# floe/backscrub

Hardware: AMD Instinct MI355X
Metric: composited frames/sec at 640×480 (batch), 1/2/4/8 MI355X + mask IoU vs CPU ref (higher is better)
Workload: dtype f32 (network) / u8 (image kernels); 1 GPU; BASELINE configs[1]: batch=256 640x480 frames, segm_lite_v681.tflite; moving scene: ring of 4 batches, a new one every step; 1 step = prep+network+decode+mask+blend, inputs resident in HBM; streams_per_gpu=256, library=bsx 0.1 (HIP gfx950, f32 NHWC)

## Files before the change

backscrub_amd/csrc/bsx_api.hip:

```cpp
#include "debug_switches.hpp"
#include <hip/hip_runtime.h>

#include <algorithm>
#include <cmath>
#include <cstdarg>
#include <cstdio>
#include <cstdlib>
#include <cstring>
#include <map>
#include <memory>
#include <string>
#include <thread>
#include <vector>

#include "../../include/bsx.h"
#include "gen_mid.hpp"
#include "kernels.hpp"
#include "roctx_ranges.hpp"
#include "plan.hpp"
#include "refusal.hpp"
#include "rtc.hpp"
#include "specialised.hpp"
#include "tflite_model.hpp"
#include "vcam_nv12_plan.hpp"
// ... 245 lines not shown
    BSX_HIP(c, hipMemcpy(c->d_geom_classes, rec.data(), G * sizeof(GeomClass), hipMemcpyHostToDevice));
  }
  if (any_edge && !c->d_geom_classes_vg) {
    BSX_HIP(c, hipMalloc(reinterpret_cast<void**>(&c->d_geom_classes_vg), G * sizeof(GeomClass)));
    BSX_HIP(c, hipMemcpy(c->d_geom_classes_vg, rec_vg.data(), G * sizeof(GeomClass), hipMemcpyHostToDevice));
  }
  if (!c->no_uniform_tiles && !c->d_geom_tile_class) {
    BSX_HIP(c, hipMalloc(&c->d_geom_tile_class, tiles + 4));
    BSX_HIP(c, hipMemset(c->d_geom_tile_class, 0, tiles + 4));
  }
  if (!c->h_geo) BSX_HIP(c, hipHostMalloc(reinterpret_cast<void**>(&c->h_geo), bsx_ctx::kIdRing * N * sizeof(GeomDesc), hipHostMallocDefault));
  BSX_HIP(c, hipMalloc(reinterpret_cast<void**>(&c->d_geo), bsx_ctx::kIdRing * N * sizeof(GeomDesc)));
  return BSX_OK;
}

int init_device_state(bsx_ctx* c) {
  BSX_HIP(c, hipStreamCreateWithFlags(&c->own_stream, hipStreamNonBlocking));
  const size_t N = (size_t)c->n_streams;
  BSX_HIP(c, hipMalloc(&c->d_arena, c->plan.arena_floats_per_stream * N * sizeof(float)));
  BSX_HIP(c, hipMalloc(&c->d_net_in, N * c->inW * c->inH * c->inC * sizeof(float)));
  BSX_HIP(c, hipMalloc(&c->d_net_in_u8, N * c->inW * c->inH * sizeof(uint32_t)));
  BSX_HIP(c, hipMalloc(&c->d_net_out, N * c->outW * c->outH * c->outC * sizeof(float)));
  BSX_HIP(c, hipMalloc(&c->d_weights, std::max<size_t>(c->plan.weights.size(), 4) * sizeof(float)));
  BSX_HIP(c, hipMemcpy(c->d_weights, c->plan.weights.data(), c->plan.weights.size() * sizeof(float), hipMemcpyHostToDevice));
  BSX_HIP(c, hipMalloc(&c->d_weights16, std::max<size_t>(c->plan.weights16.size(), 8) * sizeof(uint16_t)));
  BSX_HIP(c, hipMemcpy(c->d_weights16, c->plan.weights16.data(), c->plan.weights16.size() * sizeof(uint16_t), hipMemcpyHostToDevice));
  if (const char* m = getenv("BSX_F16_GEMM")) c->f16_terms = !strcmp(m, "off") ? 0 : (!strcmp(m, "fast") ? 1 : (!strcmp(m, "fast16") ? 17 : 3));
  c->use_program = !c->plan.program.empty() && BSX_DBG_ENV("BSX_NO_FRAME_PROGRAM") == nullptr &&
                   (c->plan.seg.on || c->plan.program_lds_tensors >= c->plan.program_global_tensors || BSX_DBG_ENV("BSX_FORCE_FRAME_PROGRAM") != nullptr);
  hipDeviceProp_t prop;
  const bool have_prop = c->use_program && !BSX_DBG_ENV("BSX_NO_RTC") && hipGetDeviceProperties(&prop, c->device) == hipSuccess;
  const KernelVariant v = kernel_variant(c->plan);
  if (c->use_program) {
    BSX_HIP(c, hipMalloc(&c->d_program, c->plan.program.size() * sizeof(MicroOp)));
    BSX_HIP(c, hipMemcpy(c->d_program, c->plan.program.data(), c->plan.program.size() * sizeof(MicroOp), hipMemcpyHostToDevice));
    BSX_HIP(c, frame_program_prepare(c->plan.program_lds_floats));
    if (c->plan.seg.on) BSX_HIP(c, seg_prepare());
    c->act16 = v.act16;
    if (BSX_DBG_ENV("BSX_NO_RTC")) no_specialised("BSX_NO_RTC", &c->kern);
    else if (!have_prop) no_specialised("no device properties", &c->kern);
    else load_specialised(build_specialised(c->plan, v, prop.gcnArchName), &c->kern);
    if (c->act16 && !c->kern.mid) {
      c->last_error = "BSX_ACT16: the specialised middle kernel is not available (" + c->kern.mid_note + ")";
      return BSX_EDEVICE;
    }
    if (c->act16) c->kern.mid_note += ", 16-bit activation storage";
  } else {
    BSX_HIP(c, nn_prepare());
  }
  if (const char* l = BSX_DBG_ENV("BSX_PIPE_WGS")) c->pipe_wgs = std::min(8, std::max(0, atoi(l)));
  if (const char* l = BSX_DBG_ENV("BSX_LANES")) c->lanes = std::min(4, std::max(1, atoi(l)));
  if (c->lanes > 1) {
    BSX_HIP(c, hipEventCreateWithFlags(&c->ev_fork, hipEventDisableTiming));
    for (int k = 1; k < c->lanes; k++) {
      BSX_HIP(c, hipStreamCreateWithFlags(&c->lane_stream[k], hipStreamNonBlocking));
      BSX_HIP(c, hipEventCreateWithFlags(&c->ev_join[k], hipEventDisableTiming));
    }
  }
  if (BSX_DBG_ENV("BSX_NO_GRAPH")) c->graph_state = -1;
  c->in_u8 = v.u8in && ((c->use_program && c->plan.seg.on) || (!c->use_program && head0_u8_ok(c->plan)));
  BSX_HIP(c, hipMalloc(&c->d_ofinal, N * c->outW * c->outH));
  BSX_HIP(c, hipMalloc(&c->d_masks, c->mask_bytes));
  BSX_HIP(c, hipMemset(c->d_ofinal, 0, N * c->outW * c->outH));
  BSX_HIP(c, hipMemset(c->d_masks, 255, c->mask_bytes));
  {
    const double sigma_color = 100.0, sigma_space = 100.0;
    const double gc = -0.5 / (sigma_color * sigma_color), gs = -0.5 / (sigma_space * sigma_space);
    const int radius = 2;
    std::vector<float> lut(768);
    for (int i = 0; i < 768; i++) lut[i] = (float)std::exp(i * i * gc);
    BSX_HIP(c, hipMalloc(&c->d_color_lut, 768 * sizeof(float)));
    BSX_HIP(c, hipMemcpy(c->d_color_lut, lut.data(), 768 * sizeof(float), hipMemcpyHostToDevice));
    int k = 0;
    for (int i = -radius; i <= radius; i++) for (int j = -radius; j <= radius; j++) {
      double r = std::sqrt((double)i * i + (double)j * j);
      if (r > radius) continue;
      c->bilateral.space_w[k] = (float)std::exp(r * r * gs);
      c->bilateral.off_y[k] = i; c->bilateral.off_x[k] = j;
      k++;
    }
    c->bilateral.color_lut = c->d_color_lut;
    c->bilateral.scale = c->norm_scale; c->bilateral.offset = c->norm_offset;
    if (k != 13 || !bilateral_taps_match(c->bilateral)) { c->last_error = "bilateral tap table does not match the kernel"; return BSX_EDEVICE; }
  }
  int rc = upload_tab(c, make_resize_tab(c->roi.w, c->roi.h, c->in_roi.w, c->in_roi.h), &c->tab_down);
  if (rc) return rc;
  rc = upload_tab(c, make_resize_tab(c->in_roi.w, c->in_roi.h, c->roi.w, c->roi.h), &c->tab_up);
  if (rc) return rc;
  c->tiles_per_frame = (size_t)((c->roi.w + mask_tile_width() - 1) / mask_tile_width()) * (size_t)((c->roi.h + mask_tile_height() - 1) / mask_tile_height());
  if (!c->no_uniform_tiles && c->tab_up.tab.mode == 0 && c->tab_up.tab.tile_ok && c->geoms.size() <= 1) {
    BSX_HIP(c, hipMalloc(&c->d_tile_class, N * c->tiles_per_frame + 4));
    BSX_HIP(c, hipMemset(c->d_tile_class, 0, N * c->tiles_per_frame + 4));
    c->tab_up.tab.tile_class = c->d_tile_class;
  }
  for (size_t g = 0; g < c->geoms.size(); g++) {
    bsx_ctx::Geom& G = c->geoms[g];
    if (g == 0) { G.tab_down = c->tab_down; G.tab_up = c->tab_up; }
    else {
      if ((rc = upload_tab(c, make_resize_tab(G.roi.w, G.roi.h, G.in_roi.w, G.in_roi.h), &G.tab_down))) return rc;
      if ((rc = upload_tab(c, make_resize_tab(G.in_roi.w, G.in_roi.h, G.roi.w, G.roi.h), &G.tab_up))) return rc;
    }
    G.tab_up.tab.tile_class = nullptr;
    G.edge = c->edge_roi && !geom_class_on_grid(G.roi);
    const size_t tile_rows = (size_t)((G.roi.h + mask_tile_height() - 1) / mask_tile_height());
    G.tiles_per_frame = (size_t)geom_tile_cols(G.roi, G.edge) * tile_rows;
    G.vg_tiles_per_frame = (size_t)geom_tile_cols(G.roi, false) * tile_rows;
    G.outside_blocks = geom_outside_blocks(G.width, G.height, G.roi);
    G.fusable = G.edge ? geom_class_edge_fusable(G.width, G.roi, G.tab_up.tab, G.shifted_tiles_fit) : geom_class_fusable(G.width, G.roi, G.tab_up.tab);
    G.xcd = geom_class_xcd(G.width, G.roi);
  }
  if (c->geoms.size() > 1) return geoms_device_state(c);
  return BSX_OK;
}

hipStream_t pick(bsx_ctx*, void* s) { return (hipStream_t)s; }

struct LaunchTimer { std::vector<hipEvent_t> ev; int k = 0; ~LaunchTimer() { for (hipEvent_t e : ev) if (e) (void)hipEventDestroy(e); } };
int timed(bsx_ctx* c, LaunchTimer* t, hipStream_t s) {
  if (t->k + 1 >= (int)t->ev.size()) { c->last_error = "error: bsx_profile_batch: the step made more launches than the profile counts\n"; return BSX_EDEVICE; }
  BSX_HIP(c, hipEventRecord(t->ev[++t->k], s));
  return BSX_OK;
}
#define BSX_LAUNCH(c, t, s, expr) do { BSX_HIP(c, (expr)); if (t) { const int trc_ = timed(c, t, s); if (trc_) return trc_; } } while (0)

int run_prep(bsx_ctx* c, const uint8_t* d_frames, int n, hipStream_t s, bool with_f32 = false, bool yuyv_in = false, LaunchTimer* t = nullptr) {
  bsx_roctx::Range range("bsx:prep");
  float* f32 = (!c->in_u8 || with_f32) ? c->tensor_ptr(c->plan.input) : nullptr;
  uint32_t* u8 = c->in_u8 ? c->d_net_in_u8 : nullptr;
  BSX_LAUNCH(c, t, s, launch_prep_fused(d_frames, c->width, c->height, c->roi, f32, u8, c->inW, c->inH, c->in_roi, c->tab_down.tab, c->bilateral, n, s, yuyv_in));
  return BSX_OK;
}
bool argmax_tail(const bsx_ctx* c) {
  return !c->use_program && !c->keep_logits && c->model_type == BSX_MODEL_DEEPLAB && !c->plan.steps.empty() && c->plan.steps.back().out == c->plan.output &&
         resize_argmax_fusable(c->plan.steps.back());
}
hipError_t launch_program(bsx_ctx* c, int n, hipStream_t s, unsigned long long* timeline = nullptr) {
  long pf = (long)c->plan.arena_floats_per_stream;
  if (c->kern.mid) {
    float* arena = c->d_arena;
    const float* weights = c->d_weights;
    void* args[] = {&arena, &pf, &weights, &timeline};
    return hipModuleLaunchKernel(c->kern.mid, (unsigned)n, 1, 1, (unsigned)c->plan.mid_lanes, 1, 1, 0, s, args, nullptr);
  }
  return launch_frame_program(c->d_program, (int)c->plan.program.size(), c->plan.program_lds_floats, c->d_arena, pf, c->d_net_in, c->d_net_out, c->d_weights, n, s,
                              timeline);
}
int state_write_fence(bsx_ctx* c, hipStream_t s) {
  if (!c->wait_before_state) return BSX_OK;
  hipEvent_t ev = c->wait_before_state;
  c->wait_before_state = nullptr;
  BSX_HIP(c, hipStreamWaitEvent(s, ev, 0));
  return BSX_OK;
}
bool program_op_elided(const bsx_ctx* c, int i) { return c->kern.mid && !BSX_DBG_ENV("BSX_RTC_FINE") && mid_pw_feeds_dw(c->plan, i); }

bool debug_tensor_half(const bsx_ctx* c, int t) {
  const Plan& p = c->plan;
  if (t == p.input || t == p.output) return false;
  if (c->use_program) {
    if (!c->act16) return false;
    if (p.seg.on && std::find(p.seg_stored.begin(), p.seg_stored.end(), t) != p.seg_stored.end()) return true;
    for (size_t i = 0; i < p.program.size() && i < p.program_out_tensor.size(); i++)
      if (p.program_out_tensor[i] == t) return p.program[i].kind != kMicroSe;
    return false;
  }
  const int n = c->last_net_n > 0 ? c->last_net_n : c->n_streams;
  for (int j = 1; j < (int)p.steps.size(); j++)
    if (p.steps[j].out == t) return p.steps[j - 1].fuse_dw == j && ir_out16(p, p.steps[j - 1], n, c->d_weights16, c->f16_terms, BSX_DBG_ENV("BSX_NO_PW_GEMM") != nullptr);
  return false;
}

bool k3_frame_runs(const bsx_ctx* c) { return c->use_program && c->plan.seg.on && c->plan.seg.k3f.on && c->kern.k3_frame != nullptr; }
bool infer_decodes(const bsx_ctx* c) { return (c->use_program && c->plan.seg.on && !c->keep_logits) || argmax_tail(c); }
int run_infer(bsx_ctx* c, int n, hipStream_t s, bool logits = true, int slot = 0, const int* ids = nullptr, LaunchTimer* t = nullptr) {
  bsx_roctx::Range range("bsx:network");
  c->last_net_n = n;
  c->last_net_logits = logits;
  if (c->arena_poison) {
    BSX_HIP(c, hipMemsetAsync(c->d_arena, 0xFF, c->plan.arena_floats_per_stream * (size_t)c->n_streams * sizeof(float), s));
    BSX_HIP(c, hipMemsetAsync(c->d_net_out, 0xFF, (size_t)c->n_streams * c->outW * c->outH * c->outC * sizeof(float), s));
  }
  if (c->use_program && c->plan.seg.on) {
    const SegPlan& sp = c->plan.seg;
    const hipFunction_t* fn = c->kern.seg;
    const long pf = (long)c->plan.arena_floats_per_stream;
    const void* in = c->in_u8 ? (const void*)c->d_net_in_u8 : (const void*)c->d_net_in;
    BSX_LAUNCH(c, t, s, launch_seg_head(fn[0], sp.head, c->d_arena, pf, in, c->d_weights, n, s, c->act16, c->in_u8, c->norm_scale, c->norm_offset));
    BSX_LAUNCH(c, t, s, launch_seg_k2(fn[1], sp.k2, c->d_arena, pf, c->d_weights, n, s, c->act16));
    BSX_LAUNCH(c, t, s, launch_program(c, n, s));
    if (k3_frame_runs(c)) {
      BSX_LAUNCH(c, t, s, launch_seg_k3_frame(c->kern.k3_frame, sp.k3f, c->d_arena, pf, c->d_weights, n, s));
    } else {
      BSX_LAUNCH(c, t, s, launch_seg_k3(fn[2], sp.k3, c->d_arena, pf, c->d_weights, n, s, c->act16));
      if (sp.tail.pre_gate_off >= 0) BSX_LAUNCH(c, t, s, launch_seg_gate(sp.tail.gate, c->d_arena, pf, c->d_weights, sp.tail.pre_gate_off, n, s));
    }
    if (!logits) { const int frc = state_write_fence(c, s); if (frc) return frc; }
    BSX_LAUNCH(c, t, s, launch_seg_tail(fn[3], sp.tail, c->d_arena, pf, c->d_net_out, c->d_ofinal + (size_t)slot * c->outW * c->outH, c->d_weights, logits, n, s,
                                        c->act16, ids));
    return BSX_OK;
  }
  if (c->use_program) {
    BSX_LAUNCH(c, t, s, launch_program(c, n, s));
    return BSX_OK;
  }
  const bool fused_tail = !logits && argmax_tail(c);
  const size_t ns = c->plan.steps.size() - (fused_tail ? 1 : 0);
  for (size_t i = 0; i < ns; i++)
    BSX_LAUNCH(c, t, s, launch_step(c->plan.steps[i], c->plan, c->d_arena, c->d_net_in, c->d_net_out, c->d_weights, n, c->n_streams, s, c->d_weights16, c->f16_terms, c->in_u8 ? c->d_net_in_u8 : nullptr, c->norm_scale, c->norm_offset));
  if (fused_tail) {
    const Step& last = c->plan.steps.back();
    { const int frc = state_write_fence(c, s); if (frc) return frc; }
    BSX_LAUNCH(c, t, s, launch_resize_argmax_iir(last, c->d_arena + (size_t)c->plan.tensor_off[last.in0] * (size_t)c->n_streams,
                                                 c->d_ofinal + (size_t)slot * c->outW * c->outH, n, s, c->tail_generic, ids));
  }
  return BSX_OK;
}
int run_decode(bsx_ctx* c, int n, hipStream_t s, int slot = 0, const int* ids = nullptr, LaunchTimer* t = nullptr) {
  bsx_roctx::Range range("bsx:decode");
  { const int frc = state_write_fence(c, s); if (frc) return frc; }
  BSX_LAUNCH(c, t, s, launch_decode(c->model_type, c->tensor_ptr(c->plan.output), c->d_ofinal + (size_t)slot * c->outW * c->outH, c->outW * c->outH, c->outC, n, s, ids));
  return BSX_OK;
}
ResizeTab tab_up_at(const bsx_ctx* c, int slot) { ResizeTab t = c->tab_up.tab; if (t.tile_class) t.tile_class += (size_t)slot * c->tiles_per_frame; return t; }
int run_mask(bsx_ctx* c, int n, hipStream_t s, int slot = 0, const int* ids = nullptr, LaunchTimer* t = nullptr, uint8_t* masks = nullptr) {
  bsx_roctx::Range range("bsx:mask");
  BSX_LAUNCH(c, t, s, launch_mask_upscale_blur(c->d_ofinal + (size_t)slot * c->outW * c->outH, c->outW, c->outH, c->in_roi, tab_up_at(c, slot),
                                      (masks ? masks : c->d_masks) + (size_t)slot * c->width * c->height, c->width, c->height, c->roi, n, s, ids));
  return BSX_OK;
}
int infer_after_prep(bsx_ctx* c, int n, hipStream_t s, int slot, const int* ids, LaunchTimer* t = nullptr) {
  if (c->onprep && !t) { BSX_HIP(c, hipStreamSynchronize(s)); c->onprep(c->caller_ctx); }
  const bool fused_decode = infer_decodes(c);
  if (const int rc = run_infer(c, n, s, !fused_decode, slot, ids, t)) return rc;
  if (c->oninfer && !t) { BSX_HIP(c, hipStreamSynchronize(s)); c->oninfer(c->caller_ctx); }
  return fused_decode ? BSX_OK : run_decode(c, n, s, slot, ids, t);
}
int enqueue_masks(bsx_ctx* c, const uint8_t* d_frames, int n, hipStream_t s, bool yuyv_in, int slot, const int* ids, LaunchTimer* t = nullptr) {
  if (const int rc = run_prep(c, d_frames, n, s, false, yuyv_in, t)) return rc;
  return infer_after_prep(c, n, s, slot, ids, t);
}
int process_impl(bsx_ctx* c, const uint8_t* d_frames, int n, int slot, hipStream_t s, bool yuyv_in = false, const int* ids = nullptr, uint8_t* masks = nullptr) {
  if (const int rc = enqueue_masks(c, d_frames, n, s, yuyv_in, slot, ids)) return rc;
  if (c->onmask) { BSX_HIP(c, hipStreamSynchronize(s)); c->onmask(c->caller_ctx); }
  return run_mask(c, n, s, slot, ids, nullptr, masks);
}


int refuse(bsx_ctx* c, const char* fn, const char* fmt, ...) {
  char buf[256];
  va_list ap;
  va_start(ap, fmt); vsnprintf(buf, sizeof buf, fmt, ap); va_end(ap);
  c->last_error = std::string("error: ") + fn + ": " + buf + "\n";
  return BSX_EINVAL;
}
}
int bsx::refuse_call(bsx_ctx* c, const char* fn, const char* fmt, ...) {
  char buf[256];
  va_list ap;
  va_start(ap, fmt); vsnprintf(buf, sizeof buf, fmt, ap); va_end(ap);
  g_last_error = std::string("error: ") + fn + ": " + buf + "\n";
  if (c) c->last_error = g_last_error;
  return BSX_EINVAL;
}
namespace {
int refuse_pending(bsx_ctx* c, const char* fn) {
  return c->pend.active ? refuse(c, fn, "a pipelined composite is pending (flush with bsx_step_batch_pipelined(ctx, NULL, ...) first)") : BSX_OK;
}

int refuse_geoms(bsx_ctx* c, const char* fn) {
  return c->geoms.size() > 1 ? refuse(c, fn, "context has %d geometries (only bsx_step_batch_geoms and bsx_step_batch_vcam_geoms step such a context)", (int)c->geoms.size()) : BSX_OK;
}

struct StepReq {
  const uint8_t* frames; const uint8_t* bg; size_t bg_stride; uint8_t* out;
  int out_w, out_h, n;
  unsigned flags; hipStream_t s;
  const int* ids;
  const MixDesc* mix = nullptr;
  const int* mix_pos = nullptr;
  bool mix_bgr = false;
  bool mix_blur_due = false;
  bool yuyv() const { return (flags & BSX_STEP_YUYV) != 0; }
  bool yin() const { return (flags & BSX_STEP_YUYV_IN) != 0; }
  unsigned flip() const { return flags & (BSX_STEP_FLIP_H | BSX_STEP_FLIP_V); }
  int bgblur() const { return (int)((flags >> 8) & 255u); }
  bool resize(const bsx_ctx* c) const { return out_w != c->width || out_h != c->height; }
  size_t out_bytes() const { return (size_t)n * out_w * out_h * (yuyv() ? 2 : 3); }
  bool out_overlaps(const uint8_t* p, size_t bytes) const { return out < p + bytes && p < out + out_bytes(); }
  bool overlap(const bsx_ctx* c) const { return out_overlaps(frames, (size_t)n * c->width * c->height * (yin() ? 2 : 3)); }
};
enum class Entry { Step, Streams, Vcam, Pipelined, Mixed, VcamMixed };

bool tile_fusable(const bsx_ctx* c, const StepReq& r) {
  return !c->onmask && !c->no_mask_blend_fusion && (!r.yuyv() || ((uintptr_t)r.out & 3) == 0) && !(r.overlap(c) && (r.yin() || r.yuyv() || r.flip())) &&
         (!r.yin() || prep_yuyv_fusable(c->width, c->roi, c->tab_down.tab)) &&
         mask_blend_fusable(c->width, c->height, c->roi, r.bg, r.bg_stride, r.frames, r.yuyv() ? r.frames : r.out);
}

int check_step(bsx_ctx* c, const char* fn, const StepReq& r, Entry kind) {
  const bool vcam = kind == Entry::Vcam, pipe = kind == Entry::Pipelined, blur = r.bgblur() != 0;
  if (kind == Entry::Mixed) {
    if (!r.frames || !r.out || r.n <= 0 || r.n > c->n_streams) return refuse(c, fn, "null buffer or batch size out of range");
    if (r.flags & ~(BSX_STEP_YUYV | BSX_STEP_NO_MASK | BSX_STEP_YUYV_IN)) return refuse(c, fn, "flags 0x%x has bits outside yuyv / no-mask / yuyv-in", r.flags);
    if (const int rc = refuse_pending(c, fn)) return rc;
    if (r.yuyv() && (c->width & 1)) return refuse(c, fn, "YUYV output needs an even width");
    if (r.yin() && (c->width & 1)) return refuse(c, fn, "YUYV input needs an even capture width");
    if (r.overlap(c)) return refuse(c, fn, "output overlaps the frames (the mixed step has no in-place form)");
// ... 823 lines not shown
  char line[256];
  snprintf(line, sizeof line, "specialised middle kernel: %zu micro-ops, %zu workgroup barriers per launch (%zu between ops + %zu inside ops)\n", p.program.size(), ob + sy, ob, sy);
  return line;
}
}

extern "C" {

const char* bsx_version(void) { return "bsx 0.1 (HIP gfx950, f32 NHWC)"; }

int bsx_device_count(void) {
  int n = 0;
  if (hipGetDeviceCount(&n) != hipSuccess) return 0;
  return n;
}

const char* bsx_last_error(const bsx_ctx* ctx) { return ctx ? ctx->last_error.c_str() : g_last_error.c_str(); }

static bool capture_rois(const bsx_ctx* c, size_t width, size_t height, Rect4* roi, Rect4* in_roi) {
  float ratio = (float)c->inH / (float)c->inW;
  float frameratio = (float)height / (float)width;
  if (frameratio < ratio) {
    *roi = Rect4{(int)((width - height / ratio) / 2), 0, (int)(height / ratio), (int)height};
    *in_roi = Rect4{0, 0, c->inW, c->inH};
  } else {
    *roi = Rect4{0, 0, (int)width, (int)height};
    *in_roi = Rect4{(int)((c->inW - c->inH / frameratio) / 2), 0, (int)(c->inH / frameratio), c->inH};
  }
  return !(roi->w <= 0 || roi->h <= 0 || roi->x < 0 || roi->x + roi->w > (int)width || in_roi->w <= 0 || in_roi->x < 0 || in_roi->x + in_roi->w > c->inW ||
           in_roi->x + in_roi->w > c->outW || in_roi->h > c->outH);
}

static bsx_ctx* new_ctx(const char* model_path, size_t threads, const bsx_geometry* geoms, int n_geoms, int device, bsx_debug_fn ondebug, bsx_stage_fn onprep,
                        bsx_stage_fn oninfer, bsx_stage_fn onmask, void* caller_ctx, unsigned geom_flags = 0) {
  const size_t width = (size_t)geoms[0].width, height = (size_t)geoms[0].height;
  int n_streams = 0;
  for (int g = 0; g < n_geoms; g++) n_streams += geoms[g].n_streams;
  try {
  std::unique_ptr<bsx_ctx> c(new bsx_ctx);
  c->ondebug = ondebug; c->onprep = onprep; c->oninfer = oninfer; c->onmask = onmask; c->caller_ctx = caller_ctx;
  c->threads = threads; c->width = (int)width; c->height = (int)height; c->n_streams = n_streams; c->device = device;
  c->edge_roi = (geom_flags & BSX_GEOMS_EDGE_ROI) != 0;
  std::string err;
  if (!load_tflite(model_path, &c->graph, &err)) { report(nullptr, ondebug, caller_ctx, "error: %s\n", err.c_str()); return nullptr; }
  c->model_type = model_type_from_name(model_path);
  if (c->model_type == BSX_MODEL_UNKNOWN) { report(nullptr, ondebug, caller_ctx, "error: unknown model type '%s'.\n", model_path); return nullptr; }
  if (c->model_type == BSX_MODEL_DEEPLAB) { c->norm_scale = (float)(1 / 127.5); c->norm_offset = -1.f; }
  else { c->norm_scale = (float)(1 / 255.0); c->norm_offset = 0.f; }
  const TensorInfo& ti = c->graph.tensors[c->graph.input];
  const TensorInfo& to = c->graph.tensors[c->graph.output];
  if (ti.shape.size() != 4 || to.shape.size() != 4 || ti.dims[0] != 1) {
    report(nullptr, ondebug, caller_ctx, "error: model input/output is not a single 4-D float tensor\n");
    return nullptr;
  }
  c->inH = ti.dims[1]; c->inW = ti.dims[2]; c->inC = ti.dims[3];
  c->outH = to.dims[1]; c->outW = to.dims[2]; c->outC = to.dims[3];
  if (c->inC != 3) { report(nullptr, ondebug, caller_ctx, "error: model input must have 3 channels\n"); return nullptr; }
  if ((c->model_type == BSX_MODEL_MEET && c->outC != 2) || (c->model_type == BSX_MODEL_DEEPLAB && c->outC < 16)) {
    report(nullptr, ondebug, caller_ctx, "error: model output has %d channels, unexpected for this model type\n", c->outC);
    return nullptr;
  }
  bool no_reuse = BSX_DBG_ENV("BSX_ARENA_NO_REUSE") != nullptr;
  const bool segments = BSX_DBG_ENV("BSX_NO_SEGMENTS") == nullptr && BSX_DBG_ENV("BSX_NO_FRAME_PROGRAM") == nullptr;
  if (!build_plan(c->graph, &c->plan, &err, !no_reuse, segments)) { report(nullptr, ondebug, caller_ctx, "error: unable to build GPU plan: %s\n", err.c_str()); return nullptr; }
  if (!capture_rois(c.get(), width, height, &c->roi, &c->in_roi)) {
    report(nullptr, ondebug, caller_ctx, "error: frame/model geometry yields an empty or out-of-range ROI\n");
    return nullptr;
  }
  c->no_mask_tile = BSX_DBG_ENV("BSX_NO_MASK_TILE") != nullptr;
  for (int g = 0; g < n_geoms; g++) {
    bsx_ctx::Geom G;
    G.width = geoms[g].width; G.height = geoms[g].height; G.n_streams = geoms[g].n_streams;
    G.first = g ? c->geoms[g - 1].first + c->geoms[g - 1].n_streams : 0;
    G.mask_offset = c->mask_bytes;
    c->mask_bytes += (size_t)G.n_streams * G.width * G.height;
    if (!capture_rois(c.get(), (size_t)G.width, (size_t)G.height, &G.roi, &G.in_roi)) {
      report(nullptr, ondebug, caller_ctx, "error: bsx_new_geoms: geoms[%d] (%d x %d): frame/model geometry yields an empty or out-of-range ROI\n", g, G.width, G.height);
      return nullptr;
    }
    if (c->edge_roi) {
      const HostResizeTab up = make_resize_tab(G.in_roi.w, G.in_roi.h, G.roi.w, G.roi.h);
      G.shifted_tiles_fit = up.mode == 0 && mask_tile_fits(up.xofs.data(), up.yofs.data(), up.sw, up.sh, up.dw, up.dh, geom_edge_shift(G.roi));
      const bool tiles = up.mode == 0 && !c->no_mask_tile && G.roi.w >= 8 && G.shifted_tiles_fit && mask_tile_fits(up.xofs.data(), up.yofs.data(), up.sw, up.sh, up.dw, up.dh);
      if (G.width & 3) {
        report(nullptr, ondebug, caller_ctx, "error: bsx_new_geoms_ex: geoms[%d] (%d x %d): width %d is not a multiple of 4 (the edge-ROI flag frees roi.x and roi.w; a row "
               "must still be whole dwords)\n", g, G.width, G.height, G.width);
        return nullptr;
      }
      if (!tiles) {
        report(nullptr, ondebug, caller_ctx, "error: bsx_new_geoms_ex: geoms[%d] (%d x %d) is off the fused tile route: the mask up-scale %d x %d -> %d x %d must be a tiled "
               "linear one\n", g, G.width, G.height, G.in_roi.w, G.in_roi.h, G.roi.w, G.roi.h);
        return nullptr;
      }
    } else if (n_geoms > 1) {
      const HostResizeTab up = make_resize_tab(G.in_roi.w, G.in_roi.h, G.roi.w, G.roi.h);
      const bool tiles = up.mode == 0 && !c->no_mask_tile && mask_tile_fits(up.xofs.data(), up.yofs.data(), up.sw, up.sh, up.dw, up.dh);
      if ((G.width & 3) || (G.roi.x & 3) || (G.roi.w & 3) || !tiles) {
        report(nullptr, ondebug, caller_ctx, "error: bsx_new_geoms: geoms[%d] (%d x %d) is off the fused tile route: width %d, roi.x %d and roi.w %d must be multiples of 4 and "
               "the mask up-scale %d x %d -> %d x %d a tiled linear one\n", g, G.width, G.height, G.width, G.roi.x, G.roi.w, G.in_roi.w, G.in_roi.h, G.roi.w, G.roi.h);
        return nullptr;
      }
    }
    c->geoms.push_back(G);
  }
  c->no_mask_blend_fusion = BSX_DBG_ENV("BSX_NO_MASK_BLEND_FUSION") != nullptr;
  c->no_bgblur_fusion = BSX_DBG_ENV("BSX_NO_BGBLUR_FUSION") != nullptr;
  c->vcam_direct = BSX_DBG_ENV("BSX_VCAM_DIRECT") != nullptr;
  c->no_uniform_tiles = getenv("BSX_NO_UNIFORM_TILES") != nullptr;
  c->tail_generic = BSX_DBG_ENV("BSX_TAIL_GENERIC") != nullptr;
  c->keep_logits = BSX_DBG_ENV("BSX_KEEP_LOGITS") != nullptr;
  c->arena_poison = BSX_DBG_ENV("BSX_ARENA_POISON") != nullptr;
  int ndev = 0;
  if (hipGetDeviceCount(&ndev) != hipSuccess || device < 0 || device >= ndev) {
    report(nullptr, ondebug, caller_ctx, "error: HIP device %d not available (%d visible)\n", device, ndev); return nullptr; }
  DeviceGuard guard(device);
  if (init_device_state(c.get()) != BSX_OK) { bsx_ctx* raw = c.release(); bsx_delete(raw); return nullptr; }
  c->plan_text = c->plan.describe();
  {
    char line[256];
    for (size_t i = 0; i < c->plan.steps.size(); i++) {
      if (c->use_program || !c->d_weights16 || !ir_out16_planned(c->plan, c->plan.steps[i], c->f16_terms)) continue;
      const Step& dd = c->plan.steps[c->plan.steps[i].fuse_dw];
      snprintf(line, sizeof line, "f16 storage: steps %zu and %d (expand + depthwise) store t%d (%dx%dx%d per frame) as f16 at %ld pixels and more, step %d reads it as f16\n", i,
               c->plan.steps[i].fuse_dw, dd.out, dd.OH, dd.OW, dd.Cout, kOut16MinRows, c->plan.steps[i].fuse_dw + 1);
      c->plan_text += line;
    }
    snprintf(line, sizeof line, "frame program: %s, %zu micro-ops, LDS %d floats (%.1f KiB), %d tensors in LDS, %d in HBM\n",
             c->use_program ? "ON" : "off", c->plan.program.size(), c->plan.program_lds_floats, c->plan.program_lds_floats / 256.0,
             c->plan.program_lds_tensors, c->plan.program_global_tensors);
    c->plan_text += line;
    if (no_reuse) c->plan_text += "arena: every tensor in a slot of its own (debug switch)\n";
    if (c->arena_poison) c->plan_text += "arena: filled with NaN bytes in front of every network stage (debug switch)\n";
    if (c->use_program) c->plan_text += "program execution: " + c->kern.mid_note + "\n";
    if (c->use_program && c->plan.seg.on) {
      std::string seg = c->plan.seg_text;
      if (c->act16)
        for (size_t at = seg.find(" stores t"); at != std::string::npos; at = seg.find(" stores t", at)) {
          for (at += 7; at + 2 < seg.size() && seg[at] == ' ' && seg[at + 1] == 't' && isdigit((unsigned char)seg[at + 2]); ) {
            for (at += 2; at < seg.size() && isdigit((unsigned char)seg[at]); at++) {}
            seg.insert(at, ":f16");
            at += 4;
          }
        }
      c->plan_text += seg;
    }
    if (c->use_program && c->plan.seg.on) c->plan_text += "segment execution: " + c->kern.seg_note + "\n";
    if (c->use_program && c->plan.seg.on && c->plan.seg.k3f.on && !c->kern.k3_frame)
      c->plan_text += "segment k3 execution: tiles and the gate launch (the per-frame form is part of the specialised module only)\n";
    if (c->use_program && c->kern.mid) c->plan_text += mid_barrier_line(c->plan, c->act16);
    for (size_t i = 0; i < c->plan.program_labels.size(); i++) {
      c->plan_text += "P" + std::to_string(i) + " " + c->plan.program_labels[i];
      if (i < c->plan.program_out_tensor.size()) {
        const int sp = c->plan.program[i].out.space;
        c->plan_text += " -> t" + std::to_string(c->plan.program_out_tensor[i]) + (sp == kLocLds ? " lds" : (program_op_elided(c.get(), (int)i) ? " elided" : (sp == kLocOutput ? " output" : " hbm")));
        if (sp == kLocGlobal && !program_op_elided(c.get(), (int)i) && debug_tensor_half(c.get(), c->plan.program_out_tensor[i])) c->plan_text += " f16";
      }
      c->plan_text += "\n";
    }
  }
  return c.release();
  } catch (const std::exception& e) {
    report(nullptr, ondebug, caller_ctx, "error: %s while creating the context\n", e.what());
    return nullptr;
  } catch (...) {
    report(nullptr, ondebug, caller_ctx, "error: unknown exception while creating the context\n");
    return nullptr;
  }
}

bsx_ctx* bsx_new(const char* model_path, size_t threads, size_t width, size_t height, int n_streams, int device, bsx_debug_fn ondebug,
                 bsx_stage_fn onprep, bsx_stage_fn oninfer, bsx_stage_fn onmask, void* caller_ctx) {
  if (!model_path || !width || !height || width > 0x7fffffffu || height > 0x7fffffffu || n_streams <= 0 || n_streams > 65535) {
    report(nullptr, ondebug, caller_ctx, "error: bad arguments to bsx_new\n"); return nullptr; }
  const bsx_geometry one{(int)width, (int)height, n_streams};
  return new_ctx(model_path, threads, &one, 1, device, ondebug, onprep, oninfer, onmask, caller_ctx);
}

static bsx_ctx* new_geoms_checked(const char* fn, const char* model_path, size_t threads, const bsx_geometry* geoms, int n_geoms, int device, unsigned geom_flags,
                                  bsx_debug_fn ondebug, bsx_stage_fn onprep, bsx_stage_fn oninfer, bsx_stage_fn onmask, void* caller_ctx) {
  if (!model_path || !geoms) { report(nullptr, ondebug, caller_ctx, "%s model_path or geoms is NULL\n", fn); return nullptr; }
  if (n_geoms < 1 || n_geoms > BSX_MAX_GEOMS) { report(nullptr, ondebug, caller_ctx, "%s n_geoms = %d is outside [1, %d]\n", fn, n_geoms, BSX_MAX_GEOMS); return nullptr; }
  long total = 0;
  for (int g = 0; g < n_geoms; g++) {
    if (geoms[g].width <= 0 || geoms[g].height <= 0) { report(nullptr, ondebug, caller_ctx, "%s geoms[%d]: size %d x %d is not positive\n", fn, g, geoms[g].width, geoms[g].height); return nullptr; }
    if (geoms[g].n_streams <= 0) { report(nullptr, ondebug, caller_ctx, "%s geoms[%d] (%d x %d): n_streams = %d is not positive\n", fn, g, geoms[g].width, geoms[g].height, geoms[g].n_streams); return nullptr; }
    for (int k = 0; k < g; k++)
      if (geoms[k].width == geoms[g].width && geoms[k].height == geoms[g].height) {
        report(nullptr, ondebug, caller_ctx, "%s geoms[%d] (%d x %d) repeats the size of geoms[%d]\n", fn, g, geoms[g].width, geoms[g].height, k); return nullptr; }
    total += geoms[g].n_streams;
    if (total > 65535) { report(nullptr, ondebug, caller_ctx, "%s geoms[%d] (%d x %d) brings the total to %ld streams, above 65535\n", fn, g, geoms[g].width, geoms[g].height, total); return nullptr; }
  }
  if (n_geoms > 1 && onmask) { report(nullptr, ondebug, caller_ctx, "%s an onmask callback needs a context of one geometry (%d given)\n", fn, n_geoms); return nullptr; }
  return new_ctx(model_path, threads, geoms, n_geoms, device, ondebug, onprep, oninfer, onmask, caller_ctx, geom_flags);
}

bsx_ctx* bsx_new_geoms(const char* model_path, size_t threads, const bsx_geometry* geoms, int n_geoms, int device, bsx_debug_fn ondebug, bsx_stage_fn onprep,
                       bsx_stage_fn oninfer, bsx_stage_fn onmask, void* caller_ctx) {
  return new_geoms_checked("error: bsx_new_geoms:", model_path, threads, geoms, n_geoms, device, 0, ondebug, onprep, oninfer, onmask, caller_ctx);
}

bsx_ctx* bsx_new_geoms_ex(const char* model_path, size_t threads, const bsx_geometry* geoms, int n_geoms, int device, unsigned flags, bsx_debug_fn ondebug,
                          bsx_stage_fn onprep, bsx_stage_fn oninfer, bsx_stage_fn onmask, void* caller_ctx) {
  if (flags == 0) return bsx_new_geoms(model_path, threads, geoms, n_geoms, device, ondebug, onprep, oninfer, onmask, caller_ctx);
  if (const unsigned unknown = flags & ~BSX_GEOMS_EDGE_ROI) {
    report(nullptr, ondebug, caller_ctx, "error: bsx_new_geoms_ex: flags 0x%x has the unknown bit 0x%x (known: 0x%x, the edge-ROI flag)\n", flags, unknown & (0u - unknown),
           BSX_GEOMS_EDGE_ROI);
    return nullptr;
  }
  return new_geoms_checked("error: bsx_new_geoms_ex:", model_path, threads, geoms, n_geoms, device, flags, ondebug, onprep, oninfer, onmask, caller_ctx);
}

void bsx_delete(bsx_ctx* c) {
  if (!c) return;
  DeviceGuard guard(c->device);
  if (c->own_stream) (void)hipStreamSynchronize(c->own_stream);
  for (auto& kv : c->host_graphs) if (kv.second) (void)hipGraphExecDestroy(kv.second);
  unload_specialised(&c->kern);
  void* ptrs[] = {c->d_arena, c->d_net_in, c->d_net_in_u8, c->d_net_out, c->d_weights, c->d_ofinal, c->d_masks, c->d_host_frame, c->d_bgr_scratch, c->d_bgr_scratch2, c->d_mask_scratch, c->d_bgblur_scratch, c->d_bgr_in_scratch, c->d_color_lut, c->tab_down.mem, c->tab_up.mem, c->d_program, c->d_weights16, c->d_tile_class};
  for (void* p : ptrs) if (p) (void)hipFree(p);
  for (auto& kv : c->bg_tabs) if (kv.second.mem) (void)hipFree(kv.second.mem);
  for (auto& kv : c->vcam_tabs) if (kv.second.d.mem) (void)hipFree(kv.second.d.mem);
  for (auto& kv : c->vg_geoms) { for (void* m : kv.second.mem) if (m) (void)hipFree(m); if (kv.second.d_rec) (void)hipFree(kv.second.d_rec); }
  if (c->own_stream) (void)hipStreamDestroy(c->own_stream);
  for (int k = 1; k < 4; k++) { if (c->lane_stream[k]) (void)hipStreamDestroy(c->lane_stream[k]); if (c->ev_join[k]) (void)hipEventDestroy(c->ev_join[k]); }
  if (c->ev_fork) (void)hipEventDestroy(c->ev_fork);
  if (c->comp_stream) { (void)hipStreamSynchronize(c->comp_stream); (void)hipStreamDestroy(c->comp_stream); }
  if (c->ev_pdone) (void)hipEventDestroy(c->ev_pdone);
  if (c->ev_pcomp) (void)hipEventDestroy(c->ev_pcomp);
  for (hipEvent_t& e : c->ev_ids) if (e) (void)hipEventDestroy(e);
  if (c->d_ids) (void)hipFree(c->d_ids);
  if (c->h_ids) (void)hipHostFree(c->h_ids);
  if (c->d_mix) (void)hipFree(c->d_mix);
  if (c->h_mix) (void)hipHostFree(c->h_mix);
  if (c->d_rsz) (void)hipFree(c->d_rsz);
  if (c->h_rsz) (void)hipHostFree(c->h_rsz);
  if (c->d_blur) (void)hipFree(c->d_blur);
  if (c->h_blur) (void)hipHostFree(c->h_blur);
  if (c->d_blur_coef) (void)hipFree(c->d_blur_coef);
  for (size_t g = 1; g < c->geoms.size(); g++) { if (c->geoms[g].tab_down.mem) (void)hipFree(c->geoms[g].tab_down.mem); if (c->geoms[g].tab_up.mem) (void)hipFree(c->geoms[g].tab_up.mem); }
  if (c->d_geom_classes) (void)hipFree(c->d_geom_classes);
  if (c->d_geom_classes_vg) (void)hipFree(c->d_geom_classes_vg);
  if (c->d_geom_tile_class) (void)hipFree(c->d_geom_tile_class);
  if (c->d_geo) (void)hipFree(c->d_geo);
  if (c->d_vo) (void)hipFree(c->d_vo);
  if (c->h_vo) (void)hipHostFree(c->h_vo);
  if (c->h_geo) (void)hipHostFree(c->h_geo);
  delete c;
}

int bsx_get_info(const bsx_ctx* c, bsx_info* o) {
  if (!c || !o) return BSX_EINVAL;
  memset(o, 0, sizeof *o);
  o->model_type = c->model_type; o->width = c->width; o->height = c->height; o->n_streams = c->n_streams;
  o->in_w = c->inW; o->in_h = c->inH; o->in_c = c->inC; o->out_w = c->outW; o->out_h = c->outH; o->out_c = c->outC;
  int r[4] = {c->roi.x, c->roi.y, c->roi.w, c->roi.h}, q[4] = {c->in_roi.x, c->in_roi.y, c->in_roi.w, c->in_roi.h};
  memcpy(o->roi, r, sizeof r); memcpy(o->in_roi, q, sizeof q);
  o->n_ops = c->graph.n_file_ops; o->n_steps = c->use_program ? (c->plan.seg.on ? 5 : 1) : (int)c->plan.steps.size(); o->device = c->device;
  o->norm_scale = c->norm_scale; o->norm_offset = c->norm_offset;
  o->nn_flops_per_frame = 2.0 * c->plan.macs_per_frame;
  o->act_bytes_per_stream = c->plan.arena_floats_per_stream * sizeof(float);
  return BSX_OK;
}

int bsx_reset(bsx_ctx* c, void* stream) {
  if (!c) return BSX_EINVAL;
  DeviceGuard guard(c->device);
  hipStream_t s = pick(c, stream);
  const size_t N = (size_t)c->n_streams;
  c->pend.active = false;
  BSX_HIP(c, hipMemsetAsync(c->d_ofinal, 0, N * c->outW * c->outH, s));
  BSX_HIP(c, hipMemsetAsync(c->d_masks, 255, c->mask_bytes, s));
  return BSX_OK;
}

uint8_t* bsx_masks_device(bsx_ctx* c) { return c ? c->d_masks : nullptr; }

int bsx_process_batch(bsx_ctx* c, const uint8_t* d_frames, int n, uint8_t* d_masks, void* stream) {
  if (!c || !d_frames || n <= 0 || n > c->n_streams) return BSX_EINVAL;
  if (const int rc = refuse_geoms(c, "bsx_process_batch")) return rc;
  if (const int rc = refuse_pending(c, "bsx_process_batch")) return rc;
  DeviceGuard guard(c->device);
  hipStream_t s = pick(c, stream);
  if (const int rc = process_impl(c, d_frames, n, 0, s)) return rc;
  if (d_masks) BSX_HIP(c, hipMemcpyAsync(d_masks, c->d_masks, (size_t)n * c->width * c->height, hipMemcpyDeviceToDevice, s));
  return BSX_OK;
}

int bsx_process_host(bsx_ctx* c, int stream_idx, const uint8_t* h_bgr, size_t bgr_stride, uint8_t* h_mask, size_t mask_stride) {
  if (!c || !h_bgr || !h_mask || stream_idx < 0 || stream_idx >= c->n_streams) return BSX_EINVAL;
  if (const int rc = refuse_geoms(c, "bsx_process_host")) return rc;
  if (bgr_stride < (size_t)c->width * 3 || mask_stride < (size_t)c->width) return BSX_ESIZE;
  if (const int rc = refuse_pending(c, "bsx_process_host")) return rc;
  DeviceGuard guard(c->device);
  hipStream_t s = c->own_stream;
  const size_t fbytes = (size_t)c->width * c->height * 3;
  if (!c->d_host_frame) BSX_HIP(c, hipMalloc(&c->d_host_frame, fbytes));
  BSX_HIP(c, hipMemcpy2DAsync(c->d_host_frame, (size_t)c->width * 3, h_bgr, bgr_stride, (size_t)c->width * 3, c->height, hipMemcpyHostToDevice, s));
  int rc = BSX_OK;
  hipGraphExec_t exec = nullptr;
  if (c->graph_state >= 0 && !c->onprep && !c->oninfer && !c->onmask) {
    auto it = c->host_graphs.find(stream_idx);
    if (it != c->host_graphs.end()) exec = it->second;
    else if (c->host_graphs.size() < 64) {
      hipGraph_t g = nullptr;
      bool ok = hipStreamBeginCapture(s, hipStreamCaptureModeThreadLocal) == hipSuccess;
      if (ok) {
        rc = process_impl(c, c->d_host_frame, 1, stream_idx, s);
// ... 327 lines not shown
  DeviceGuard guard(c->device);
  hipStream_t s = pick(c, stream);
  const bool seg = c->use_program && c->plan.seg.on;
  const bool fused_decode = infer_decodes(c);
  const bool atail = argmax_tail(c);
  const int n_net = c->use_program ? (seg ? (c->plan.seg.tail.pre_gate_off >= 0 && !k3_frame_runs(c) ? 6 : 5) : 1) : (int)c->plan.steps.size();
  const bool fuse_tail = tile_fusable(c, StepReq{d_frames, d_bg, bg_stride, d_out, c->width, c->height, n, 0u, s, nullptr});
  const int L = 1 + n_net + (fused_decode ? 0 : 1) + (fuse_tail ? 1 : 2) + (fuse_tail ? 1 : 0);
  if (cap < L) return BSX_EINVAL;
  LaunchTimer t{std::vector<hipEvent_t>((size_t)L + 1, nullptr)};
  for (auto& e : t.ev) BSX_HIP(c, hipEventCreate(&e));
  std::vector<double> sum(L, 0.0);
  const double N = n, px = (double)c->width * c->height;
  for (int it = 0; it < iters; it++) {
    t.k = 0;
    BSX_HIP(c, hipEventRecord(t.ev[0], s));
    if (const int rc = enqueue_masks(c, d_frames, n, s, false, 0, nullptr, &t)) return rc;
    if (fuse_tail) {
      BSX_LAUNCH(c, &t, s, launch_mask_blend(c->d_ofinal, c->outW, c->outH, c->in_roi, c->tab_up.tab, c->d_masks, c->width, c->height, c->roi, d_bg, bg_stride,
                                             d_frames, d_out, n, s));
    } else if (const int rc = run_mask(c, n, s, 0, nullptr, &t)) return rc;
    BSX_LAUNCH(c, &t, s, launch_blend(d_bg, bg_stride, d_frames, c->d_masks, d_out, (size_t)c->width * c->height, n, s));
    BSX_HIP(c, hipStreamSynchronize(s));
    if (t.k != L) { c->last_error = "error: bsx_profile_batch: the step made fewer launches than the profile counts\n"; return BSX_EDEVICE; }
    for (int j = 0; j < L; j++) { float ms = 0; BSX_HIP(c, hipEventElapsedTime(&ms, t.ev[j], t.ev[j + 1])); sum[j] += ms; }
  }
  auto put = [&](int j, const std::string& name, double bytes, double flops) {
    memset(&out[j], 0, sizeof out[j]);
    snprintf(out[j].name, sizeof out[j].name, "%s", name.c_str());
    out[j].avg_ms = sum[j] / iters; out[j].bytes = bytes; out[j].flops = flops;
  };
  int j = 0;
  const double canvas = (double)c->inW * c->inH;
  const double touched = (double)std::min(c->roi.w, 2 * c->in_roi.w) * (double)std::min(c->roi.h, 2 * c->in_roi.h);
  put(j++, "prep", N * (3.0 * touched + (c->in_u8 ? 4.0 : 12.0) * canvas), 0);
  if (seg) {
    const std::vector<Step>& S = c->plan.steps;
    const int NS = (int)S.size();
    auto macs = [&](int a, int b) { double m = 0; for (int i = a; i <= b; i++) m += S[i].macs; return m; };
    const SegPlan& sp = c->plan.seg;
    const double eA = 16.0 * sp.head.H1 * sp.head.W1, eb0 = 16.0 * sp.head.H2 * sp.head.W2, ec0 = (double)sp.k2.dw.C * sp.k2.H3 * sp.k2.W3;
    const double elo2 = 16.0 * sp.k3.HL * sp.k3.WL, elo = 16.0 * sp.k3.H2 * sp.k3.W2;
    const double ein = (double)c->inW * c->inH * c->inC, eout = (double)c->outW * c->outH * c->outC;
    put(j++, "seg_head", N * ((c->in_u8 ? 4.0 * c->inW * c->inH : 4.0 * ein) + 4.0 * (eA + eb0)), N * 2.0 * macs(0, 2));
    put(j++, "seg_k2", N * 4.0 * (eb0 + eb0 + ec0), N * 2.0 * macs(3, 8));
    put(j++, "frame_program", N * 4.0 * (ec0 + elo2) + 4.0 * c->plan.weights.size(), N * 2.0 * macs(9, NS - 11));
    const double egate = 16.0 * (sp.tail.gate.part[0].n + sp.tail.gate.part[1].n) + 16.0, fgate = 2.0 * macs(NS - 5, NS - 4);
    if (k3_frame_runs(c)) put(j++, "seg_k3", N * 4.0 * (eb0 + elo2 + elo + egate), N * (2.0 * macs(NS - 10, NS - 8) + fgate));
    else {
      put(j++, "seg_k3", N * 4.0 * (eb0 + elo2 + elo), N * 2.0 * macs(NS - 10, NS - 8));
      if (sp.tail.pre_gate_off >= 0) put(j++, "seg_gate", N * 4.0 * egate, 0);
    }
    put(j++, fused_decode ? "seg_tail+decode" : "seg_tail", N * (4.0 * (eA + elo) + (fused_decode ? 2.0 * c->outW * c->outH : 4.0 * eout)), N * 2.0 * macs(NS - 7, NS - 1));
  } else if (c->use_program) {
    double io = (double)c->inW * c->inH * c->inC + (double)c->outW * c->outH * c->outC;
    put(j++, "frame_program", N * io * 4.0 + 4.0 * c->plan.weights.size(), N * 2.0 * c->plan.macs_per_frame);
  } else
  for (const Step& st : c->plan.steps) {
    double in = (double)st.H * st.W * st.Cin, o = (double)st.OH * st.OW * st.Cout, b = 0;
    switch (st.kind) {
      case StepKind::Eltwise: b = in + o + (st.elt == kEltUnary ? 0 : (st.bcast1 ? st.Cin : in)) + (st.elt == kEltMulAdd ? in : 0); break;
      case StepKind::Concat: b = 2 * o; break;
      case StepKind::Gap: b = in + st.Cin; break;
      default: b = in + o + (st.residual >= 0 ? o : 0) + (st.in_scale >= 0 ? st.Cin : 0); break;
    }
    const bool is_tail = atail && &st == &c->plan.steps.back();
    const bool ir_on = c->d_weights16 && c->f16_terms > 0;
    const bool h0 = c->plan.steps[0].fuse_head0;
    const bool h0_member = h0 && (&st == &c->plan.steps[1] || &st == &c->plan.steps[2]);
    if (h0_member || (st.fused_away && !(h0 && &st <= &c->plan.steps[2]) && ir_on)) { put(j++, st.label + " (inside the launch before)", 0, 0); continue; }
    if (st.chain_mid >= 0 && chain3_on(c->plan, st.chain_mid, n, c->d_weights16, c->f16_terms)) { put(j++, st.label + " (inside the chained launch)", 0, 0); continue; }
    if (st.chain_first >= 0 && chain3_on(c->plan, (int)(&st - c->plan.steps.data()), n, c->d_weights16, c->f16_terms)) {
      const Step& ca = c->plan.steps[st.chain_first];
      const Step& cc = c->plan.steps[st.chain_last];
      put(j++, ca.label + "+" + st.label + "+" + cc.label, N * 4.0 * ((double)ca.H * ca.W * ca.Cin + (double)cc.OH * cc.OW * cc.Cout), N * 2.0 * (ca.macs + st.macs + cc.macs));
      continue;
    }
    if (st.fuse_head0 && h0) {
      const Step& d1 = c->plan.steps[1];
      const Step& p2 = c->plan.steps[2];
      put(j++, st.label + "+" + d1.label + "+" + p2.label, N * ((c->in_u8 ? 4.0 * st.H * st.W : 4.0 * in) + 4.0 * (double)p2.OH * p2.OW * p2.Cout), N * 2.0 * (st.macs + d1.macs + p2.macs));
      continue;
    }
    if (st.fuse_dw >= 0 && ir_on) {
      const Step& dd = c->plan.steps[st.fuse_dw];
      put(j++, st.label + "+" + dd.label, N * 4.0 * (in + (double)dd.OH * dd.OW * dd.Cout), N * 2.0 * (st.macs + dd.macs));
      continue;
    }
    put(j++, is_tail ? st.label + "+argmax" : st.label, is_tail ? N * (4.0 * in + 2.0 * st.OH * st.OW) : N * b * 4.0, N * 2.0 * st.macs);
  }
  if (!fused_decode) put(j++, "decode_iir", N * ((double)c->outW * c->outH * c->outC * 4.0 + 2.0 * c->outW * c->outH), 0);
  if (fuse_tail) {
    put(j++, "mask_blend", N * ((double)c->in_roi.w * c->in_roi.h + 10.0 * px), 0);
    put(j++, "blend(standalone)", N * 10.0 * px, 0);
  } else {
    put(j++, "mask_upscale_blur", N * ((double)c->in_roi.w * c->in_roi.h + (double)c->roi.w * c->roi.h), 0);
    put(j++, "blend", N * 10.0 * px, 0);
  }
  return j;
}

int bsx_debug_mask_tile_stats(bsx_ctx* c, int n, long* out4) {
  if (!c || !out4 || n <= 0 || n > c->n_streams) return BSX_EINVAL;
  if (const int rc = refuse_geoms(c, "bsx_debug_mask_tile_stats")) return rc;
  DeviceGuard guard(c->device);
  out4[0] = (long)c->tiles_per_frame * n; out4[1] = out4[2] = 0; out4[3] = out4[0];
  if (!c->d_tile_class) return BSX_OK;
  BSX_HIP(c, launch_tile_class(c->d_ofinal, c->outW, c->outH, c->in_roi, c->tab_up.tab, c->roi, n, nullptr));
  std::vector<uint8_t> cls((size_t)out4[0]);
  if (hipDeviceSynchronize() != hipSuccess || hipMemcpy(cls.data(), c->d_tile_class, cls.size(), hipMemcpyDeviceToHost) != hipSuccess) return BSX_EDEVICE;
  out4[3] = 0;
  for (uint8_t v : cls) out4[v == 1 ? 1 : (v == 2 ? 2 : 3)]++;
  return BSX_OK;
}

int bsx_debug_gauss_coeffs(int ksize, int shift, uint32_t* c4, uint32_t* c2) {
  return (c4 && c2 && gauss_coeff_words(ksize, shift, c4, c2)) ? BSX_OK : BSX_EINVAL;
}

int bsx_debug_program_timeline(bsx_ctx* c, int n, unsigned long long* ticks, int cap, void* stream) {
  if (!c || !ticks || n <= 0 || n > c->n_streams) return BSX_EINVAL;
  DeviceGuard guard(c->device);
  if (!c->use_program) return 0;
  const int L = (int)c->plan.program.size();
  if (cap < L + 1 || L + 1 > 256) return BSX_EINVAL;
  unsigned long long* d = nullptr;
  const size_t kTl = 1024 + 64 * 16 * 4;
  BSX_HIP(c, hipMalloc(&d, kTl * sizeof(unsigned long long)));
  BSX_HIP(c, hipMemset(d, 0, kTl * sizeof(unsigned long long)));
  hipStream_t s = pick(c, stream);
  BSX_HIP(c, launch_program(c, n, s, d));
  BSX_HIP(c, hipStreamSynchronize(s));
  BSX_HIP(c, hipMemcpy(ticks, d, std::min((size_t)cap, kTl) * sizeof(unsigned long long), hipMemcpyDeviceToHost));
  (void)hipFree(d);
  return L;
}

int bsx_model_describe(const char* model_path, char* buf, size_t cap) {
  if (!model_path || !buf || !cap) return BSX_EINVAL;
  std::string err, out;
  int rc = BSX_OK;
  try {
  Graph g; Plan p;
  if (!load_tflite(model_path, &g, &err) || !build_plan(g, &p, &err)) { out = err; rc = BSX_EMODEL; }
  else {
    char head[256];
    snprintf(head, sizeof head, "ops=%d nodes=%d steps=%d macs=%.0f arena_floats=%zu\n", g.n_file_ops, (int)g.nodes.size(), (int)p.steps.size(),
             p.macs_per_frame, p.arena_floats_per_stream);
    out = head + p.describe();
    snprintf(head, sizeof head, "program micro-ops=%zu lds_floats=%d lds_tensors=%d hbm_tensors=%d arena_bytes_per_frame=%ld placement_policy=%u lds_blocks=%zu lds_check=%s\n", p.program.size(),
             p.program_lds_floats, p.program_lds_tensors, p.program_global_tensors, p.program_arena_bytes, p.program_policy, p.program_blocks.size(), p.program_check.c_str());
    out += head;
    for (size_t i = 0; i < p.program_labels.size(); i++)
      out += "P" + std::to_string(i) + " " + p.program_labels[i] + (i < p.program_out_tensor.size() ? " -> t" + std::to_string(p.program_out_tensor[i]) : std::string()) + "\n";
    if (p.seg.on) out += p.seg_text;
    if (!p.program.empty()) out += mid_barrier_line(p, false);
    if (BSX_DBG_ENV("BSX_PLAN_BLOCKS"))
      for (const auto& b : p.program_blocks) { snprintf(head, sizeof head, "block off=%d len=%d steps=[%d,%d] %s\n", b.off, b.len, b.from, b.until, b.what.c_str()); out += head; }
  }
  } catch (const std::exception& e) { out = std::string("exception while reading the model: ") + e.what(); rc = BSX_EMODEL; }
  catch (...) { out = "unknown exception while reading the model"; rc = BSX_EMODEL; }
  snprintf(buf, cap, "%s", out.c_str());
  return rc;
}

long bsx_model_kernel_source(const char* model_path, char* buf, size_t cap) {
  if (!model_path || !buf || !cap) return BSX_EINVAL;
  try {
    Graph g; Plan p;
    std::string err;
    if (!load_tflite(model_path, &g, &err) || !build_plan(g, &p, &err)) { snprintf(buf, cap, "%s", err.c_str()); return BSX_EMODEL; }
    if (p.program.empty()) { snprintf(buf, cap, "no program"); return 0; }
    const SpecialisedCode m = build_specialised(p, kernel_variant(p), "gfx950", kBuildMid).mid;
    snprintf(buf, cap, "%s", (m.source.empty() ? m.why : m.source).c_str());
    return (long)m.source.size();
  } catch (...) { snprintf(buf, cap, "exception while reading the model"); return BSX_EMODEL; }
}

long bsx_model_seg_source(const char* model_path, char* buf, size_t cap) {
  if (!model_path || !buf || !cap) return BSX_EINVAL;
  try {
    Graph g; Plan p;
    std::string err;
    if (!load_tflite(model_path, &g, &err) || !build_plan(g, &p, &err)) { snprintf(buf, cap, "%s", err.c_str()); return BSX_EMODEL; }
    const SpecialisedCode sc = build_specialised(p, kernel_variant(p), "gfx950", kBuildSeg).seg;
    snprintf(buf, cap, "%s", (sc.source.empty() ? sc.why : sc.source).c_str());
    return (long)sc.source.size();
  } catch (...) { snprintf(buf, cap, "exception while reading the model"); return BSX_EMODEL; }
}

int bsx_model_precompile(const char* model_path, const char* arch, char* msg, size_t cap) {
  if (!model_path || !msg || !cap) return BSX_EINVAL;
  try {
    Graph g; Plan p;
    std::string err;
    if (!load_tflite(model_path, &g, &err) || !build_plan(g, &p, &err)) { snprintf(msg, cap, "%s", err.c_str()); return BSX_EMODEL; }
    if (p.program.empty()) { snprintf(msg, cap, "interpreted (no program)"); return BSX_OK; }
    const SpecialisedBuild b = build_specialised(p, kernel_variant(p), arch ? arch : "gfx950");
    const std::string& e = b.mid.fallback;
    if (b.mid.code.empty()) { snprintf(msg, cap, "%s", e.c_str()); return e.compare(0, 19, "interpreted (hipRTC") == 0 ? BSX_EMODEL : BSX_OK; }
    std::string seg_msg;
    if (p.seg.on) {
      if (!b.seg.code.empty()) {
        long worst = 0;
        for (const char* k : {"bsx_seg_head", "bsx_seg_k2", "bsx_seg_k3", "bsx_seg_tail"}) worst = std::max(worst, code_object_scratch_bytes(b.seg.code, k));
        if (b.seg_k3_frame) worst = std::max(worst, code_object_scratch_bytes(b.seg.code, "bsx_seg_k3f"));
        char sm[256];
        snprintf(sm, sizeof sm, "; segment kernels %s (%zu bytes of source, %zu bytes of code object, %ld B of scratch)", b.seg.cached ? "cached" : "compiled", b.seg.source.size(),
                 b.seg.code.size(), worst);
        seg_msg = sm;
      } else {
        seg_msg = "; segment kernels: " + b.seg.fallback;
        if (b.seg.fallback.find("hipRTC:") != std::string::npos) { snprintf(msg, cap, "%s", seg_msg.c_str()); return BSX_EMODEL; }
      }
    }
    snprintf(msg, cap, "%s (%zu bytes of source, %zu bytes of code object, %ld B of scratch%s, cache %s)%s", b.mid.cached ? "cached" : "compiled", b.mid.source.size(),
             b.mid.code.size(), b.scratch, b.opaque_tid ? ", lane indices re-derived per op" : "", rtc_cache_dir().c_str(), seg_msg.c_str());
    return BSX_OK;
  } catch (...) { snprintf(msg, cap, "exception while reading the model"); return BSX_EMODEL; }
}

const char* bsx_plan_describe(bsx_ctx* c) { return c ? c->plan_text.c_str() : ""; }

static const char* debug_tensor_unstored(const bsx_ctx* c, int t) {
  const Plan& p = c->plan;
  if (t == p.input) return nullptr;
  if (t == p.output) return c->last_net_logits ? nullptr : "the last network stage decoded inside its final kernel and wrote no logits";
  if (c->use_program) {
    if (p.seg.on && std::find(p.seg_stored.begin(), p.seg_stored.end(), t) != p.seg_stored.end()) return nullptr;
    if (p.seg.on && std::find(p.seg_partials.begin(), p.seg_partials.end(), t) != p.seg_partials.end()) return nullptr;
    for (size_t i = 0; i < p.program.size() && i < p.program_out_tensor.size(); i++) {
      if (p.program_out_tensor[i] != t) continue;
      if (p.program[i].out.space == kLocLds) return "the frame program keeps it in LDS";
      if (p.program[i].out.space != kLocGlobal) return "the frame program writes it to a buffer of its own";
      if (program_op_elided(c, (int)i)) return "the specialised middle kernel computes it chunk by chunk inside the depthwise that reads it";
      return nullptr;
    }
    return p.seg.on ? "it lives inside a segment kernel or a fused micro-op (LDS / registers only)" : "it lives inside a fused micro-op (LDS / registers only)";
  }
  const int NS = (int)p.steps.size();
  const int n = c->last_net_n > 0 ? c->last_net_n : c->n_streams;
  const bool ir_on = c->d_weights16 && c->f16_terms > 0;
  for (int j = 0; j < NS; j++) {
    const Step& st = p.steps[j];
    if (st.out != t) continue;
    if (p.steps[0].fuse_head0 && j < 2) return "the fused head kernel (stem + depthwise + 1x1) keeps it in LDS";
    if (st.fuse_dw >= 0 && ir_on) return "the fused expand + depthwise kernel keeps it in LDS";
    if (st.chain_first >= 0 && chain3_on(p, j, n, c->d_weights16, c->f16_terms)) return "the chained 1x1 kernel keeps it in registers";
    if (st.chain_mid >= 0 && j < st.chain_mid && chain3_on(p, st.chain_mid, n, c->d_weights16, c->f16_terms)) return "the chained 1x1 kernel keeps it in registers";
    return nullptr;
  }
  return "no step of this plan writes it";
}

static long debug_tensor_at(bsx_ctx* c, int t, int stream_idx, float* h_out, long cap) {
  if (!c) return BSX_EINVAL;
  if (t < 0 || t >= (int)c->plan.tensor_off.size() || t >= (int)c->plan.tensor_elems.size() || stream_idx < 0 || stream_idx >= c->n_streams || (h_out && cap < 0)) { c->last_error = "bsx_debug_tensor: tensor or stream index out of range"; return BSX_EINVAL; }
  if (c->plan.tensor_off[t] < 0) { c->last_error = "bsx_debug_tensor: tensor " + std::to_string(t) + " has no place in the arena (a constant, or fused away by the planner)"; return BSX_EINVAL; }
  if (const char* why = debug_tensor_unstored(c, t)) { c->last_error = "bsx_debug_tensor: tensor " + std::to_string(t) + " is never written to the arena on this path: " + why; return BSX_EINVAL; }
  DeviceGuard guard(c->device);
  const long n = c->plan.tensor_elems[t];
  if (!h_out) return n;
  const float* p = (t == c->plan.input || t == c->plan.output || !c->use_program) ? c->tensor_ptr(t) + (size_t)stream_idx * (size_t)n
                                                                                 : c->tensor_ptr(t) + (size_t)stream_idx * c->plan.arena_floats_per_stream;
  if (hipDeviceSynchronize() != hipSuccess) return BSX_EDEVICE;
  const size_t take = (size_t)std::min(n, cap);
  if (debug_tensor_half(c, t)) {
    const bool batch_major = !c->use_program;
    const _Float16* ph = reinterpret_cast<const _Float16*>(batch_major ? c->tensor_ptr(t) : p) + (batch_major ? (size_t)stream_idx * (size_t)n : 0);
    std::vector<_Float16> h(take);
    if (take && hipMemcpy(h.data(), ph, sizeof(_Float16) * take, hipMemcpyDeviceToHost) != hipSuccess) return BSX_EDEVICE;
    for (size_t i = 0; i < take; i++) h_out[i] = (float)h[i];
    return n;
  }
  if (hipMemcpy(h_out, p, sizeof(float) * take, hipMemcpyDeviceToHost) != hipSuccess) return BSX_EDEVICE;
  return n;
}

long bsx_debug_tensor_of(bsx_ctx* c, int t, int stream_idx, float* h_out, long cap) { return debug_tensor_at(c, t, stream_idx, h_out, cap); }
long bsx_debug_tensor(bsx_ctx* c, int t, float* h_out, long cap) { return debug_tensor_at(c, t, 0, h_out, cap); }

}
```

backscrub_amd/csrc/gen_mid.cpp:

```cpp
#include "debug_switches.hpp"
#include "gen_mid.hpp"

#include <algorithm>
#include <cstdarg>
#include <cstdio>
#include <cstdlib>
#include <utility>
#include <vector>

namespace bsx {
namespace {

const char kPrelude[] =
#include "mid_prelude_str.inc"
    ;

struct Out {
  std::string s;
  void f(const char* fmt, ...) __attribute__((format(printf, 2, 3))) {
    char buf[2048];
    va_list ap, ap2;
    va_start(ap, fmt);
    va_copy(ap2, ap);
    const int need = vsnprintf(buf, sizeof buf, fmt, ap);
    va_end(ap);
    if (need >= 0 && (size_t)need < sizeof buf) s.append(buf, (size_t)need);
    else if (need >= 0) { std::string big((size_t)need + 1, '\0'); vsnprintf(&big[0], big.size(), fmt, ap2); big.resize((size_t)need); s += big; }
    va_end(ap2);
  }
};

std::string comment_safe(const std::string& in) {
  std::string o;
  for (char ch : in.substr(0, 200)) o += (ch == '\n' || ch == '\r' || ch == '\\' || (unsigned char)ch < 32) ? ' ' : ch;
  return o;
}

int sp_of(const Loc& l) { return l.space == kLocNone ? 0 : (l.space == kLocLds ? 1 : 2); }
bool plain(const Loc& l) { return l.space == kLocNone || l.space == kLocLds || l.space == kLocGlobal; }


}


static bool dw_geom_ok(const MicroOp& d) { return d.strip && d.dh == 1 && d.dw == 1 && d.kh == d.kw && (d.kh == 3 || d.kh == 5) && d.sh == d.sw && (d.sh == 1 || d.sh == 2) && d.Cin % 4 == 0; }
bool mid_dw_chunked(const MicroOp& d) {
  return d.kind == (int)StepKind::DwConv && dw_geom_ok(d) && d.in0.space == kLocGlobal && d.band_rows > 0 && (d.Cin % d.band_rows) % 8 == 0 && d.res.space == kLocNone &&
         !BSX_DBG_ENV("BSX_RTC_NO_DW_STAGE");
}
bool mid_pw_feeds_dw(const Plan& plan, int j) {
  const std::vector<MicroOp>& P = plan.program;
  const int n = (int)P.size();
  auto disjoint = [](long a0, long a1, long b0, long b1) { return a1 <= b0 || b1 <= a0; };
  if (BSX_DBG_ENV("BSX_RTC_NO_PWDW") || j < 0 || j + 1 >= n) return false;
  const MicroOp& a = P[j];
  const MicroOp& d = P[j + 1];
  if (!(a.kind == (int)StepKind::PwConv && a.mfma && !a.gemv && a.stage_floats > 0 && a.out.space == kLocGlobal && a.res.space == kLocNone) || !mid_dw_chunked(d)) return false;
  if (d.in0.off != a.out.off || d.Cin != a.Cout || d.band_rows % 16 || a.cout_pad < a.Cout) return false;
  for (long e : plan.program_ext_offs) if (e == a.out.off) return false;
  for (int q = j + 2; q < n; q++) {
    for (const Loc* l : {&P[q].in0, &P[q].in1, &P[q].in2, &P[q].res, &P[q].scale}) if (l->space == kLocGlobal && l->off == a.out.off) return false;
    for (int c = 0; c < P[q].n_cat; c++) if (P[q].cat[c].space == kLocGlobal && P[q].cat[c].off == a.out.off) return false;
    if (P[q].out.space == kLocGlobal && P[q].out.off == a.out.off) break;
  }
  const long pin = (long)a.H * a.W, ws0 = d.ws_off, ws1 = ws0 + (long)d.H * d.W * (d.band_rows + 4);
  std::vector<std::pair<long, long>> keep, placed;
  keep.push_back({a.w_lds, a.w_lds + a.stage_floats});
  if (a.in0.space == kLocLds) keep.push_back({a.in0.off, a.in0.off + pin * a.in0.stride});
  if (a.in2.space == kLocLds) keep.push_back({a.in2.off, a.in2.off + pin * a.in2.stride});
  if (a.scale.space == kLocLds) keep.push_back({a.scale.off, a.scale.off + a.Cin});
  placed.push_back({ws0, ws1});
  if (d.stage_floats > 0) placed.push_back({d.w_lds, d.w_lds + d.stage_floats});
  if (d.out.space == kLocLds) placed.push_back({d.out.off, d.out.off + (long)d.OH * d.OW * d.out.stride});
  for (auto& kq : keep) for (auto& pq : placed) if (!disjoint(kq.first, kq.second, pq.first, pq.second)) return false;
  return true;
}

std::string generate_mid_source(const Plan& plan, std::string* why, bool act16, bool opaque_tid) {
  auto asp = [&](const Loc& l) { const int sp = sp_of(l); return (sp == 2 && act16) ? 3 : sp; };
  auto loc = [&](Out& o, const char* p, const Loc& l) { o.f("  static constexpr int %s_SP = %d, %s_OFF = %d, %s_ST = %d;\n", p, asp(l), p, l.off, p, l.stride); };
  auto fail = [&](const std::string& m) { if (why) *why = m; return std::string(); };
  const std::vector<MicroOp>& P = plan.program;
  if (P.empty()) return fail("no program");
  const bool fine = BSX_DBG_ENV("BSX_RTC_FINE") != nullptr;
  Out o;
  o.s.reserve(sizeof kPrelude + 64 * 1024);
  if (BSX_DBG_ENV("BSX_RTC_EXP_MFMA")) o.s += "#define BSXM_EXP_MFMA_QUARTER 1   // timing experiment: WRONG RESULTS (mid_prelude.hip op_pw)\n";
  o.f("#define BSXM_LANES %d\n#define BSXM_ZERO_OFF %d\n", plan.mid_lanes, plan.lds_zero_off());
  if (opaque_tid) o.s += "#define BSXM_OPAQUE_TID 1\n";
  o.s += kPrelude;
  o.f("\nnamespace bsxm {\n");
  std::string body;
  Out k;
  const int n = (int)P.size();
  auto stage_of = [&](int i, Out& dst) {
    const MicroOp& m = P[i];
    if (m.stage_floats > 0) dst.f("  stage<%d>(W + %lld, L + %d);\n", m.stage_floats, m.w_off, m.w_lds);
    else {
      if (m.fc_stage[0] > 0) dst.f("  stage<%d>(W + %lld, L + %d);\n", m.fc_stage[0], m.b_off, m.fc_lds[0]);
      if (m.fc_stage[1] > 0) dst.f("  stage<%d>(W + %lld, L + %d);\n", m.fc_stage[1], m.b3_off, m.fc_lds[1]);
    }
  };
  stage_of(0, k);
  auto dw_chunked = [&](const MicroOp& d) { return mid_dw_chunked(d); };
  (void)dw_chunked;
  auto pw_feeds_dw = [&](int j) { return !fine && mid_pw_feeds_dw(plan, j); };
  for (int i = 0; i < n; i++) {
    const MicroOp& m = P[i];
    for (const Loc* l : {&m.in0, &m.in1, &m.in2, &m.res, &m.scale, &m.out}) if (!plain(*l)) return fail("operand in the network input / output buffer");
    if (fine && i > 0 && i <= 64) k.f("  FINE_END(%d);\n", i - 1);
    if (fine) k.f("  f_a = __builtin_readcyclecounter();\n");
    k.f("  op_barrier();\n  if (tl && blockIdx.x == 0 && threadIdx.x == 0) tl[%d] = __builtin_amdgcn_s_memrealtime();\n", i);
    k.f("  // ---- P%d %s\n", i, i < (int)plan.program_labels.size() ? comment_safe(plan.program_labels[i]).c_str() : "");
    if (fine) k.f("  f_b = __builtin_readcyclecounter();\n");
    const bool fed_by_prev = i > 0 && pw_feeds_dw(i - 1);
    if (i + 1 < n && !fed_by_prev) stage_of(i + 1, k);
    auto fc_loads = [&](int j) {
      const MicroOp& q = P[j];
      auto fcl = [&](int which, int cin, int cout, int stage, int lds, long long w2, long long b) {
        k.f("  FcRegs<%d, %d> fc%d_%d;\n", cin, cout, j, which);
        if (stage > 0) k.f("  fc_load<%d, %d, SP_LDS, %d, %d>(L, W, fc%d_%d);\n", cin, cout, lds + (int)(w2 - b), lds, j, which);
        else k.f("  fc_load<%d, %d, SP_GLB, %lld, %lld>(L, W, fc%d_%d);\n", cin, cout, w2, b, j, which);
      };
      fcl(1, q.Cin, q.C1, q.fc_stage[0], q.fc_lds[0], q.w2_off, q.b_off);
      if (q.n_fc == 2) fcl(2, q.C1, q.C2, q.fc_stage[1], q.fc_lds[1], q.w3_off, q.b3_off);
    };
    auto early = [&](int j) {
      if (j <= 0 || j >= n || P[j].kind != kMicroSe || P[j].fc_stage[0] > 0 || P[j].fc_stage[1] > 0) return false;
      if (BSX_DBG_ENV("BSX_RTC_NO_EARLY_FC")) return false;
      const MicroOp& pv = P[j - 1];
      if (pv.kind == (int)StepKind::PwConv && pv.mfma && !pv.gemv) return true;
      if (pv.kind != (int)StepKind::DwConv || pv.in0.space != kLocLds) return false;
      const int K = pv.kh, S = pv.sh, V = K == 5 ? 2 : 4, TX = (S == 1 && !(pv.OW % 5 != 0 && pv.OW % 4 == 0)) ? 5 : 4, NIN = (TX - 1) * S + K;
      return K * (NIN + K) * V <= 144;
    };
    if (early(i + 1)) fc_loads(i + 1);
    if (m.kind == (int)StepKind::PwConv && m.mfma && !m.gemv) {
      if (m.Cin % 4 || m.Cout % 4 || m.cout_pad % 16 || m.stage_floats <= 0) return fail("pw: channel counts / unstaged weights");
      if (m.scale.space != kLocNone && m.scale.space != kLocLds) return fail("pw: scale vector outside LDS");
      o.f("struct Op%d {\n  static constexpr int P = %d, CIN = %d, COUT = %d, CPAD = %d, ACT = %d;\n", i, m.OH * m.OW, m.Cin, m.Cout, m.cout_pad, m.act);
      loc(o, "X", m.in0); loc(o, "Y", m.out); loc(o, "R", m.res); loc(o, "D", m.in2);
      o.f("  static constexpr int S_OFF = %d, W_LDS = %d, B_LDS = %d;\n", m.scale.space == kLocLds ? m.scale.off : -1, m.w_lds, m.w_lds + (int)(m.b_off - m.w_off));
      o.f("  static constexpr int N0 = 0, NCOLS = %d, YSUB = 0;\n", m.cout_pad);
      o.f("  static constexpr bool NFAST = %s;\n};\n", ((m.out.space == kLocGlobal && !BSX_DBG_ENV("BSX_RTC_NO_NFAST")) || (m.in0.space == kLocGlobal && m.cout_pad > 16 && !BSX_DBG_ENV("BSX_RTC_NO_NFAST_IN"))) ? "true" : "false");
      if (pw_feeds_dw(i)) k.f("  // (computed chunk by chunk inside P%d: the tensor between them is never written)\n", i + 1);
      else k.f("  op_pw<Op%d>(L, A);\n", i);
    } else if (m.kind == (int)StepKind::DwConv) {
      const bool ok = m.strip && m.dh == 1 && m.dw == 1 && m.kh == m.kw && (m.kh == 3 || m.kh == 5) && m.sh == m.sw && (m.sh == 1 || m.sh == 2) && m.Cin % 4 == 0;
      if (!ok) return fail("dw: geometry outside the strip form");
      const int K = m.kh, S = m.sh, V = K == 5 ? 2 : 4;
      int TX = S == 1 ? 5 : 4;
      if (S == 1 && m.OW % 5 != 0 && m.OW % 4 == 0) TX = 4;
      const bool staged = m.stage_floats > 0;
      if (!staged && (m.w_off > 0x7fffffffll || m.b_off > 0x7fffffffll)) return fail("dw: weight offset");
      const bool chunked = mid_dw_chunked(m);
      const int CK = chunked ? m.band_rows : m.Cin, nch = (m.Cin + CK - 1) / CK;
      for (int c = 0; c < nch; c++) {
        const int CKc = std::min(CK, m.Cin - c * CK);
        char name[32];
        if (chunked) snprintf(name, sizeof name, "Op%d_%d", i, c); else snprintf(name, sizeof name, "Op%d", i);
        o.f("struct %s {\n  static constexpr int K = %d, S = %d, H = %d, W = %d, OH = %d, OW = %d, PT = %d, PL = %d, C = %d, CW = %d, YC0 = %d, ACT = %d, V = %d, TX = %d;\n", name, K, S,
            m.H, m.W, m.OH, m.OW, m.pt, m.pl, CKc, m.Cin, c * CK, m.act, V, TX);
        o.f("  static constexpr bool ZC = %s;\n", ((chunked && BSX_DBG_ENV("BSX_RTC_NO_ZC_CHUNK")) || BSX_DBG_ENV("BSX_RTC_NO_ZERO_CELL")) ? "false" : "true");
        if (chunked) o.f("  static constexpr int X_SP = 1, X_OFF = %d, X_ST = %d;\n", m.ws_off, CK + 4); else loc(o, "X", m.in0);
        loc(o, "Y", m.out); loc(o, "R", m.res);
        if (staged) o.f("  static constexpr int W_SP = SP_LDS, W_OFF = %d, B_OFF = %d;\n};\n", m.w_lds + c * CK, m.w_lds + (int)(m.b_off - m.w_off) + c * CK);
        else o.f("  static constexpr int W_SP = SP_GLB, W_OFF = %lld, B_OFF = %lld;\n};\n", m.w_off + c * CK, m.b_off + c * CK);
        if (chunked) {
          if (c > 0) k.f("  __syncthreads();\n");
          if (fed_by_prev) {
            const MicroOp& a = P[i - 1];
            o.f("struct Op%d_%d {\n  static constexpr int P = %d, CIN = %d, COUT = %d, CPAD = %d, ACT = %d;\n", i - 1, c, a.OH * a.OW, a.Cin, a.Cout, a.cout_pad, a.act);
            loc(o, "X", a.in0); loc(o, "R", a.res); loc(o, "D", a.in2);
            o.f("  static constexpr int Y_SP = 1, Y_OFF = %d, Y_ST = %d;\n", m.ws_off, CK + 4);
            o.f("  static constexpr int S_OFF = %d, W_LDS = %d, B_LDS = %d;\n", a.scale.space == kLocLds ? a.scale.off : -1, a.w_lds, a.w_lds + (int)(a.b_off - a.w_off));
            o.f("  static constexpr int N0 = %d, NCOLS = %d, YSUB = %d;\n  static constexpr bool NFAST = true;\n};\n", c * CK, (CKc + 15) / 16 * 16, c * CK);
            k.f("  op_pw<Op%d_%d>(L, A);\n  __syncthreads();\n", i - 1, c);
            if (c == nch - 1 && i + 1 < n) stage_of(i + 1, k);
          } else
            k.f("  load_chunk<%d, %d, %d, %d, %d, %d, %d, %d>(L, A);\n  __syncthreads();\n", asp(m.in0), m.in0.off, m.H * m.W, m.in0.stride, CKc, c * CK, m.ws_off, CK + 4);
        }
        k.f("  op_dw<%s>(L, A, W);\n", name);
      }
    } else if (m.kind == kMicroSe) {
      if (m.in1.space != kLocLds || (m.n_fc == 2 && m.in2.space != kLocLds) || m.Cin % 4 || m.C1 % 1) return fail("se: mean / hidden vectors outside LDS");
      if (m.w2_off > 0x7fffffffll || m.w3_off > 0x7fffffffll) return fail("se: weight offset");
      if (!early(i)) fc_loads(i);
      const int mean = m.in1.off;
      auto part = [&](const Loc& l, int rows, int C, int hw, int coff, bool accum, bool partials) {
        const int st = partials ? C : l.stride;
        k.f("  gap_part<%d, %d, %d, %d, %d, %d, %d, %s, %d>(L, A);\n", partials ? 2 : asp(l), l.off, st, rows, C, hw, coff, accum ? "true" : "false", mean);
      };
      if (m.n_cat == 0) part(m.in0, m.H * m.W, m.Cin, m.H * m.W, 0, false, false);
      else {
        int coff = 0;
        for (int c = 0; c < m.n_cat; c++) {
          if (!plain(m.cat[c]) || m.cat_c[c] % 4) return fail("se: pooled part");
          const bool partials = m.cat_parts[c] > 0;
          if (partials && m.cat[c].space != kLocGlobal) return fail("se: partial sums outside the arena");
          part(m.cat[c], partials ? m.cat_parts[c] : m.cat_hw[c], m.cat_c[c], m.cat_hw[c], coff, m.gap_sum && c > 0, partials);
          if (!m.gap_sum) coff += m.cat_c[c];
        }
      }
      k.f("  __syncthreads();\n");
      const Loc& y1 = m.n_fc == 1 ? m.out : m.in2;
      k.f("  fc_apply<%d, %d, %d, %d, %d, %d>(L, A, fc%d_1);\n", m.Cin, m.C1, m.act, mean, sp_of(y1), y1.off, i);
      if (m.n_fc == 2) {
        k.f("  __syncthreads();\n");
        k.f("  fc_apply<%d, %d, %d, %d, %d, %d>(L, A, fc%d_2);\n", m.C1, m.C2, m.act2, m.in2.off, sp_of(m.out), m.out.off, i);
      }
    } else if (m.kind == (int)StepKind::Resize) {
      if (m.Cin % 4) return fail("resize: channels");
      o.f("struct Op%d {\n  static constexpr int H = %d, W = %d, OH = %d, OW = %d, C = %d;\n  static constexpr bool HALF_PIXEL = %s, ALIGN = %s;\n", i, m.H, m.W, m.OH, m.OW, m.Cin,
          m.half_pixel ? "true" : "false", m.align_corners ? "true" : "false");
      loc(o, "X", m.in0); loc(o, "Y", m.out);
      o.f("};\n");
      k.f("  op_resize<Op%d>(L, A);\n", i);
    } else {
      return fail("micro-op kind " + std::to_string(m.kind) + " has no specialised body");
    }
  }
  o.f("}  // namespace bsxm\n\nusing namespace bsxm;\n");
  const bool two_per_cu = plan.mid_lanes <= 512 && plan.lds_total_floats <= kLdsTotalFloats / 2;
  o.f("extern \"C\" __global__ void __launch_bounds__(%d)%s bsx_mid(float* __restrict__ arena, long per_frame, const float* __restrict__ weights, unsigned long long* tl) {\n", plan.mid_lanes,
      two_per_cu ? " __attribute__((amdgpu_waves_per_eu(4, 4)))" : "");
  if (plan.program_lds_floats > plan.lds_zero_off()) return fail("LDS plan reaches into the zero cell");
  o.f("  static_assert(kZeroOff == %d && kThreads == %d, \"geometry macros\");\n", plan.lds_zero_off(), plan.mid_lanes);
  o.f("  __shared__ __attribute__((aligned(16))) float smem[%d];\n", plan.lds_total_floats);
  o.f("  lds_f* L = (lds_f*)smem;\n  glb_f* A = (glb_f*)(arena + (size_t)blockIdx.x * (size_t)per_frame);\n  const glb_f* W = (const glb_f*)weights;\n");
  o.f("  if (threadIdx.x < %d) L[kZeroOff + threadIdx.x] = 0.f;      // visible to every wave behind the first op's barrier\n", kLdsZeroFloats);
  if (fine) o.f("  unsigned long long f_a = 0, f_b = 0;\n"
                "#define FINE_END(i) do { const unsigned long long f_d = __builtin_readcyclecounter(); if (tl && blockIdx.x == 0 && (threadIdx.x & 63) == 0) { "
                "unsigned long long* f4 = tl + 1024 + ((i) * 16 + (threadIdx.x >> 6)) * 4; f4[0] = f_b - f_a; f4[1] = 0; f4[2] = f_d - f_b; f4[3] = f_a; } } while (0)\n");
  o.s += k.s;
  if (fine && n <= 64) o.f("  FINE_END(%d);\n", n - 1);
  o.f("  op_barrier();\n  if (tl && blockIdx.x == 0 && threadIdx.x == 0) tl[%d] = __builtin_amdgcn_s_memrealtime();\n}\n", n);
  return o.s;
}

}
```

backscrub_amd/csrc/gen_mid.hpp:

```cpp
#pragma once
#include <string>

#include "plan.hpp"

namespace bsx {

std::string generate_mid_source(const Plan& plan, std::string* why, bool act16 = false, bool opaque_tid = false);

bool mid_dw_chunked(const MicroOp& d);
bool mid_pw_feeds_dw(const Plan& plan, int j);

}
```

backscrub_amd/csrc/mid_prelude.hip:

```cpp
#if !defined(__HIPCC_RTC__)
#include <hip/hip_runtime.h>
#endif

namespace bsxm {

enum { SP_NONE = 0, SP_LDS = 1, SP_GLB = 2, SP_GLB16 = 3 };
enum { ACT_NONE = 0, ACT_RELU = 1, ACT_RELU6 = 3, ACT_HSWISH = 100, ACT_SIGMOID = 101 };
#ifndef BSXM_LANES
#define BSXM_LANES 1024
#endif
#ifndef BSXM_ZERO_OFF
#define BSXM_ZERO_OFF (160 * 256 - 4)
#endif
constexpr int kThreads = BSXM_LANES, kWaves = kThreads / 64;
constexpr int kZeroOff = BSXM_ZERO_OFF;

typedef __attribute__((address_space(3))) float lds_f;
typedef __attribute__((address_space(1))) float glb_f;
typedef float f4v __attribute__((ext_vector_type(4)));
typedef float f2v __attribute__((ext_vector_type(2)));
typedef __attribute__((address_space(3))) f4v lds_v4;
typedef __attribute__((address_space(1))) f4v glb_v4;
typedef __attribute__((address_space(3))) f2v lds_v2;
typedef __attribute__((address_space(1))) f2v glb_v2;
// ... 123 lines not shown
      if constexpr (TM > 0) {
#pragma unroll
        for (int r = 0; r < TM; r++) ta[r] = __fmul_rn(ta[r], L[T::S_OFF + 16 * NJ + TM * g + r]);
      }
    }
    if constexpr (T::D_SP != SP_NONE) {
#pragma unroll
      for (int j = 0; j < NJ; j++) { const f4v dv = ld4<T::D_SP>(L + T::D_OFF, A + T::D_OFF, arow * T::D_ST + 16 * j + 4 * g); a[j].x = __fadd_rn(a[j].x, dv.x); a[j].y = __fadd_rn(a[j].y, dv.y); a[j].z = __fadd_rn(a[j].z, dv.z); a[j].w = __fadd_rn(a[j].w, dv.w); }
      if constexpr (TM > 0) {
#pragma unroll
        for (int r = 0; r < TM; r++) ta[r] = __fadd_rn(ta[r], ld1<T::D_SP>(L + T::D_OFF, A + T::D_OFF, arow * T::D_ST + 16 * NJ + TM * g + r));
      }
    }
    f4v acc0 = {0.f, 0.f, 0.f, 0.f}, acc1 = {0.f, 0.f, 0.f, 0.f};
#if defined(BSXM_EXP_MFMA_QUARTER)
#pragma unroll
    for (int j = 0; j < NJ; j += 2) {
      acc0 = __builtin_amdgcn_mfma_f32_16x16x4f32(b[j][0] + b[j][1] + b[j][2] + b[j][3], a[j].x + a[j].y + a[j].z + a[j].w, acc0, 0, 0, 0);
      if (j + 1 < NJ) acc1 = __builtin_amdgcn_mfma_f32_16x16x4f32(b[j + 1 < NJ ? j + 1 : j][0] + b[j + 1 < NJ ? j + 1 : j][1] + b[j + 1 < NJ ? j + 1 : j][2] + b[j + 1 < NJ ? j + 1 : j][3],
                                                                  a[j + 1 < NJ ? j + 1 : j].x + a[j + 1 < NJ ? j + 1 : j].y + a[j + 1 < NJ ? j + 1 : j].z + a[j + 1 < NJ ? j + 1 : j].w, acc1, 0, 0, 0);
    }
#else
#pragma unroll
    for (int j = 0; j < NJ; j += 2) {
      acc0 = __builtin_amdgcn_mfma_f32_16x16x4f32(b[j][0], a[j].x, acc0, 0, 0, 0);
      if (j + 1 < NJ) acc1 = __builtin_amdgcn_mfma_f32_16x16x4f32(b[j + 1 < NJ ? j + 1 : j][0], a[j + 1 < NJ ? j + 1 : j].x, acc1, 0, 0, 0);
      acc0 = __builtin_amdgcn_mfma_f32_16x16x4f32(b[j][1], a[j].y, acc0, 0, 0, 0);
      if (j + 1 < NJ) acc1 = __builtin_amdgcn_mfma_f32_16x16x4f32(b[j + 1 < NJ ? j + 1 : j][1], a[j + 1 < NJ ? j + 1 : j].y, acc1, 0, 0, 0);
      acc0 = __builtin_amdgcn_mfma_f32_16x16x4f32(b[j][2], a[j].z, acc0, 0, 0, 0);
      if (j + 1 < NJ) acc1 = __builtin_amdgcn_mfma_f32_16x16x4f32(b[j + 1 < NJ ? j + 1 : j][2], a[j + 1 < NJ ? j + 1 : j].z, acc1, 0, 0, 0);
      acc0 = __builtin_amdgcn_mfma_f32_16x16x4f32(b[j][3], a[j].w, acc0, 0, 0, 0);
      if (j + 1 < NJ) acc1 = __builtin_amdgcn_mfma_f32_16x16x4f32(b[j + 1 < NJ ? j + 1 : j][3], a[j + 1 < NJ ? j + 1 : j].w, acc1, 0, 0, 0);
    }
#endif
    if constexpr (TM > 0) {
#pragma unroll
      for (int r = 0; r < TM; r++) acc1 = __builtin_amdgcn_mfma_f32_16x16x4f32(tb[r], ta[r], acc1, 0, 0, 0);
    }
    const f4v acc = acc0 + acc1;
    const int c0 = n0 + 4 * g, pix = m0 + li;
    f4v v = acc;
    if ((T::COUT % 16 == 0 || c0 < T::COUT) && (P % 16 == 0 || pix < P)) {
      v = act4<T::ACT>(v + *(const lds_v4*)(bl + c0));
      if constexpr (T::R_SP != SP_NONE) v += ld4<T::R_SP>(L + T::R_OFF, A + T::R_OFF, pix * T::R_ST + c0);
      st4<T::Y_SP>(L + T::Y_OFF, A + T::Y_OFF, pix * T::Y_ST + c0 - T::YSUB, v);
    }
  }
}

template <int SP, int X_OFF, int P, int CFULL, int CK, int C0, int WS, int WST = CK + 4>
__device__ __forceinline__ void load_chunk(lds_f* L, const glb_f* A) {
  constexpr int Q = CK / 4, TOTAL = P * Q, IT = (TOTAL + kThreads - 1) / kThreads;
  f4v v[IT];
#pragma unroll
  for (int it = 0; it < IT; it++) {
    const int i = min(tid_now() + it * kThreads, TOTAL - 1), px = i / Q, q = i - px * Q;
    v[it] = ld4<SP>(L, A + X_OFF, px * CFULL + C0 + 4 * q);
  }
#pragma unroll
  for (int it = 0; it < IT; it++) {
    const int i = tid_now() + it * kThreads, px = i / Q, q = i - px * Q;
    if (i < TOTAL) *(lds_v4*)(L + WS + px * WST + 4 * q) = v[it];
  }
}

template <class T> __device__ __forceinline__ void op_dw(lds_f* L, glb_f* A, const glb_f* Wg) {
  constexpr int K = T::K, S = T::S, TX = T::TX, V = T::V, C = T::C, CV = C / V, NIN = (TX - 1) * S + K;
  constexpr int NSTRIPS = (T::OW + TX - 1) / TX, TOTAL = CV * NSTRIPS * T::OH;
  typedef float vec_t __attribute__((ext_vector_type(V)));
  constexpr bool ZC = T::ZC && T::X_SP == SP_LDS;
  auto ldx = [&](int off) -> vec_t { if constexpr (V == 4) return ld4<T::X_SP>(L + T::X_OFF, A + T::X_OFF, off); else return ld2<T::X_SP>(L + T::X_OFF, A + T::X_OFF, off); };
  auto ldw = [&](int off) -> vec_t { if constexpr (V == 4) return ld4<T::W_SP>(L, Wg, off); else return ld2<T::W_SP>(L, Wg, off); };
#pragma unroll
  for (int it = 0; it < (TOTAL + kThreads - 1) / kThreads; it++) {
    const int item = tid_now() + it * kThreads;
    if (item >= TOTAL) break;
    const int t = item / CV, cq = item - t * CV, oy = t / NSTRIPS, sx = t - oy * NSTRIPS;
    const int ch = cq * V, ox0 = sx * TX, ix0 = ox0 * S - T::PL;
    vec_t acc[TX];
#pragma unroll
    for (int k = 0; k < TX; k++) acc[k] = (vec_t)(0.f);
    auto load_row = [&](int fy, vec_t (&xin)[NIN], vec_t (&wv)[K]) {
      const int iy = oy * S - T::PT + fy;
      const bool vy = iy >= 0 && iy < T::H;
      if constexpr (ZC) {
        const int rowo = (iy * T::W + ix0) * T::X_ST + ch;
#pragma unroll
        for (int j = 0; j < NIN; j++) { const int ix = ix0 + j; xin[j] = ldx(((vy && ix >= 0 && ix < T::W) ? rowo : kZeroOff - T::X_OFF - j * T::X_ST) + j * T::X_ST); }
#pragma unroll
        for (int fx = 0; fx < K; fx++) wv[fx] = ldw(T::W_OFF + (fy * K + fx) * T::CW + ch);
      } else {
        const int rowo = min(max(iy, 0), T::H - 1) * T::W * T::X_ST + ch;
#pragma unroll
        for (int j = 0; j < NIN; j++) xin[j] = ldx(rowo + min(max(ix0 + j, 0), T::W - 1) * T::X_ST);
#pragma unroll
        for (int fx = 0; fx < K; fx++) { wv[fx] = ldw(T::W_OFF + (fy * K + fx) * T::CW + ch); if (!vy) wv[fx] = (vec_t)(0.f); }
      }
    };
    auto fma_row = [&](vec_t (&xin)[NIN], const vec_t (&wv)[K]) {
      if constexpr (!ZC) {
#pragma unroll
        for (int j = 0; j < NIN; j++) { const int ix = ix0 + j; if (ix < 0 || ix >= T::W) xin[j] = (vec_t)(0.f); }
      }
#pragma unroll
      for (int k = 0; k < TX; k++) {
#pragma unroll
        for (int fx = 0; fx < K; fx++) acc[k] = __builtin_elementwise_fma(xin[k * S + fx], wv[fx], acc[k]);
      }
    };
    if constexpr (T::X_SP == SP_GLB || T::X_SP == SP_GLB16) {
      vec_t xa[NIN], wa[K];
      load_row(0, xa, wa);
#pragma unroll 1
      for (int fy = 0; fy < K; fy++) {
        vec_t xb[NIN], wb[K];
        load_row(fy + 1 < K ? fy + 1 : fy, xb, wb);
        fma_row(xa, wa);
#pragma unroll
        for (int j = 0; j < NIN; j++) xa[j] = xb[j];
#pragma unroll
        for (int fx = 0; fx < K; fx++) wa[fx] = wb[fx];
      }
    } else if constexpr (K * (NIN + K) * V <= 144) {
#pragma unroll
      for (int fy = 0; fy < K; fy++) { vec_t xin[NIN], wv[K]; load_row(fy, xin, wv); fma_row(xin, wv); }
    } else {
      vec_t x0[NIN], w0[K], x1[NIN], w1[K];
      static_assert(K % 2 == 1, "op_dw: odd filter sizes");
      load_row(0, x0, w0);
#pragma unroll 1
      for (int fy = 0; fy + 1 < K; fy += 2) {
        load_row(fy + 1, x1, w1);
        fma_row(x0, w0);
        load_row(fy + 2, x0, w0);
        fma_row(x1, w1);
      }
      fma_row(x0, w0);
    }
    const vec_t bq = ldw(T::B_OFF + ch);
#pragma unroll
    for (int k = 0; k < TX; k++) {
      const int ox = ox0 + k;
      if (T::OW % TX == 0 || ox < T::OW) {
        const int pix = oy * T::OW + ox, cho = ch + T::YC0;
        vec_t v = acc[k] + bq;
        if constexpr (V == 4) v = act4<T::ACT>(v); else v = act2<T::ACT>(v);
        if constexpr (T::R_SP != SP_NONE) { if constexpr (V == 4) v += ld4<T::R_SP>(L + T::R_OFF, A + T::R_OFF, pix * T::R_ST + ch); else v += ld2<T::R_SP>(L + T::R_OFF, A + T::R_OFF, pix * T::R_ST + ch); }
        if constexpr (V == 4) st4<T::Y_SP>(L + T::Y_OFF, A + T::Y_OFF, pix * T::Y_ST + cho, v); else st2<T::Y_SP>(L + T::Y_OFF, A + T::Y_OFF, pix * T::Y_ST + cho, v);
      }
    }
  }
}

template <int SP, int OFF, int ST, int ROWS, int C, int HW, int COFF, bool ACCUM, int MEAN_OFF>
__device__ __forceinline__ void gap_part(lds_f* L, glb_f* A) {
  constexpr int C4 = C / 4;
  const int lane = tid_now() & 63, wave = wave_id();
#pragma unroll
  for (int it = 0; it < (C4 + kWaves - 1) / kWaves; it++) {
    const int cq = wave + it * kWaves;
    if (cq >= C4) break;
    f4v a0 = {0.f, 0.f, 0.f, 0.f}, a1 = a0;
#pragma unroll
    for (int r0 = 0; r0 < ROWS; r0 += 128) {
      const int r = r0 + lane;
      if (r < ROWS) a0 += ld4<SP>(L + OFF, A + OFF, r * ST + cq * 4);
      if (r0 + 64 < ROWS && r + 64 < ROWS) a1 += ld4<SP>(L + OFF, A + OFF, (r + 64) * ST + cq * 4);
    }
    a0 += a1;
    float t = wave_total_scatter(a0, lane);
    if (lane < 4) {
      t /= (float)HW;
      if (ACCUM) t += L[MEAN_OFF + COFF + cq * 4 + lane];
      L[MEAN_OFF + COFF + cq * 4 + lane] = t;
    }
  }
}

template <int CIN, int COUT> struct FcGeom {
  static constexpr int K8 = 4 * ((CIN + 31) / 32);
  static constexpr bool EIGHT = CIN % K8 == 0;
  static constexpr int LK = EIGHT ? 8 : ((CIN % 16 == 0) ? 4 : ((CIN % 8 == 0) ? 2 : 1)), KLEN = EIGHT ? K8 : CIN / LK, NSUB = CIN / KLEN;
  static constexpr int PER = kThreads / LK, IT = (COUT + PER - 1) / PER, Q = KLEN / 4;
};
template <int CIN, int COUT> struct FcRegs { f4v w[FcGeom<CIN, COUT>::IT][FcGeom<CIN, COUT>::Q]; float b[FcGeom<CIN, COUT>::IT]; };
template <int CIN, int COUT, int W_SP, int W_OFF, int B_OFF>
__device__ __forceinline__ void fc_load(const lds_f* L, const glb_f* Wg, FcRegs<CIN, COUT>& r) {
  typedef FcGeom<CIN, COUT> G;
  const int sub = tid_now() & (G::LK - 1), co0 = tid_now() / G::LK;
  asm volatile("" : "+s"(Wg));
#pragma unroll
  for (int it = 0; it < G::IT; it++) {
    const int co = min(co0 + it * G::PER, COUT - 1);
    const int ks = min(sub, G::NSUB - 1) * G::KLEN;
#pragma unroll
    for (int q = 0; q < G::Q; q++) r.w[it][q] = ld4<W_SP>(L, Wg, W_OFF + co * CIN + ks + 4 * q);
    r.b[it] = ld1<W_SP>(L, Wg, B_OFF + co);
  }
}
template <int CIN, int COUT, int ACT, int X_OFF, int Y_SP, int Y_OFF>
__device__ __forceinline__ void fc_apply(lds_f* L, glb_f* A, const FcRegs<CIN, COUT>& r) {
  typedef FcGeom<CIN, COUT> G;
  const int sub = tid_now() & (G::LK - 1), co0 = tid_now() / G::LK;
  f4v xv[G::Q];
#pragma unroll
  for (int q = 0; q < G::Q; q++) {
    xv[q] = *(const lds_v4*)(L + X_OFF + min(sub, G::NSUB - 1) * G::KLEN + 4 * q);
    if (G::NSUB < G::LK && sub >= G::NSUB) xv[q] = (f4v)(0.f);
  }
#pragma unroll
  for (int it = 0; it < G::IT; it++) {
    const int co = co0 + it * G::PER;
    float a0 = 0.f, a1 = 0.f;
#pragma unroll
    for (int q = 0; q < G::Q; q++) {
      a0 = fmaf(xv[q].x, r.w[it][q].x, a0); a1 = fmaf(xv[q].y, r.w[it][q].y, a1); a0 = fmaf(xv[q].z, r.w[it][q].z, a0); a1 = fmaf(xv[q].w, r.w[it][q].w, a1);
    }
    float acc = a0 + a1;
    if constexpr (G::LK >= 2) acc += dpp<kQuadXor1>(acc);
    if constexpr (G::LK >= 4) acc += dpp<kQuadXor2>(acc);
    if constexpr (G::LK >= 8) acc += dpp<kHalfMirror>(acc);
    if (sub == 0 && co < COUT) st1<Y_SP>(L + Y_OFF, A + Y_OFF, co, act1<ACT>(acc + r.b[it]));
  }
}

__device__ __forceinline__ void interp(int o, float scale, bool half_pixel, int in_size, float* frac, int* lo, int* hi) {
  const float v = half_pixel ? __fadd_rn(__fmul_rn((float)o + 0.5f, scale), -0.5f) : __fmul_rn((float)o, scale);
  const float fl = __builtin_floorf(v);
  *lo = max((int)fl, 0);
  *hi = min((int)__builtin_ceilf(v), in_size - 1);
  *frac = v - (float)*lo;
}
__device__ __forceinline__ float bilerp(float x00, float x10, float x01, float x11, float dy, float dx) {
  const float a = __fmul_rn(__fmul_rn(x00, 1.f - dy), 1.f - dx), b = __fmul_rn(__fmul_rn(x10, dy), 1.f - dx);
  const float c = __fmul_rn(__fmul_rn(x01, 1.f - dy), dx), d = __fmul_rn(__fmul_rn(x11, dy), dx);
  return __fadd_rn(__fadd_rn(__fadd_rn(a, b), c), d);
}
template <class T> __device__ __forceinline__ void op_resize(lds_f* L, glb_f* A) {
  constexpr int CV = T::C / 4, TOTAL = T::OH * T::OW * CV;
  const float hs = (T::ALIGN && T::OH > 1) ? (float)(T::H - 1) / (float)(T::OH - 1) : (float)T::H / (float)T::OH;
  const float ws = (T::ALIGN && T::OW > 1) ? (float)(T::W - 1) / (float)(T::OW - 1) : (float)T::W / (float)T::OW;
#pragma unroll
  for (int it = 0; it < (TOTAL + kThreads - 1) / kThreads; it++) {
    const int item = tid_now() + it * kThreads;
    if (item >= TOTAL) break;
    const int p = item / CV, ch = (item - p * CV) * 4, oy = p / T::OW, ox = p - oy * T::OW;
    float dy, dx; int y0, y1, x0, x1;
    interp(oy, hs, T::HALF_PIXEL, T::H, &dy, &y0, &y1);
    interp(ox, ws, T::HALF_PIXEL, T::W, &dx, &x0, &x1);
    const f4v a = ld4<T::X_SP>(L + T::X_OFF, A + T::X_OFF, (y0 * T::W + x0) * T::X_ST + ch), b = ld4<T::X_SP>(L + T::X_OFF, A + T::X_OFF, (y1 * T::W + x0) * T::X_ST + ch);
    const f4v c = ld4<T::X_SP>(L + T::X_OFF, A + T::X_OFF, (y0 * T::W + x1) * T::X_ST + ch), d = ld4<T::X_SP>(L + T::X_OFF, A + T::X_OFF, (y1 * T::W + x1) * T::X_ST + ch);
    const f4v v = {bilerp(a.x, b.x, c.x, d.x, dy, dx), bilerp(a.y, b.y, c.y, d.y, dy, dx), bilerp(a.z, b.z, c.z, d.z, dy, dx), bilerp(a.w, b.w, c.w, d.w, dy, dx)};
    st4<T::Y_SP>(L + T::Y_OFF, A + T::Y_OFF, p * T::Y_ST + ch, v);
  }
}

}
```

backscrub_amd/csrc/plan.cpp:

```cpp
#include "debug_switches.hpp"
#include "plan.hpp"
#include "gen_seg.hpp"
#include "gen_mid.hpp"

#include <algorithm>
#include <cmath>
#include <cstdio>
#include <cstdlib>
#include <cstring>
#include <map>

namespace bsx {
namespace {

void conv_geometry(int in, int k, int s, int d, bool same, int* out, int* pad) {
  int eff = (k - 1) * d + 1;
  *out = same ? (in + s - 1) / s : (in + s - eff) / s;
  int total = (*out - 1) * s + eff - in;
  *pad = total > 0 ? total / 2 : 0;
}

uint16_t f32_to_f16_rn(float f) {
  uint32_t x; memcpy(&x, &f, 4);
  const uint32_t sign = (x >> 16) & 0x8000u;
  x &= 0x7fffffffu;
  if (x >= 0x7f800000u) return (uint16_t)(sign | 0x7c00u | ((x > 0x7f800000u) ? 0x200u : 0));
  if (x >= 0x477ff000u) return (uint16_t)(sign | 0x7bffu);
  if (x < 0x33000001u) return (uint16_t)sign;
  if (x < 0x38800000u) {
    const int e = (int)(x >> 23);
    const uint32_t m = (x & 0x7fffffu) | 0x800000u;
    const int shift = 126 - e;
    uint32_t h = m >> shift;
    const uint32_t rem = m & ((1u << shift) - 1), half = 1u << (shift - 1);
    if (rem > half || (rem == half && (h & 1))) h++;
    return (uint16_t)(sign | h);
  }
  uint32_t h = ((x - 0x38000000u) >> 13);
  const uint32_t rem = x & 0x1fffu;
  if (rem > 0x1000u || (rem == 0x1000u && (h & 1))) h++;
  return (uint16_t)(sign | h);
}
float f16_to_f32(uint16_t h) {
  const uint32_t sign = (uint32_t)(h & 0x8000u) << 16, e = (h >> 10) & 31, m = h & 1023;
  uint32_t bits;
  if (e == 31) bits = sign | 0x7f800000u | (m << 13);
  else if (e) bits = sign | ((e + 112) << 23) | (m << 13);
  else if (!m) bits = sign;
  else { int sh = 0; uint32_t mm = m; while (!(mm & 1024)) { mm <<= 1; sh++; } bits = sign | ((uint32_t)(113 - sh) << 23) | ((mm & 1023) << 13); }
  float f; memcpy(&f, &bits, 4); return f;
}

bool is_unary(OpType t) { return t == OpType::Relu || t == OpType::Relu6 || t == OpType::HardSwish || t == OpType::Logistic; }
int unary_act(OpType t) {
  switch (t) {
    case OpType::Relu: return kActRelu;
    case OpType::Relu6: return kActRelu6;
    case OpType::HardSwish: return kActHswish;
    case OpType::Logistic: return kActSigmoid;
    default: return kActNone;
  }
}
const char* act_name(int a) {
  switch (a) { case kActRelu: return "relu"; case kActRelu6: return "relu6"; case kActHswish: return "hswish"; case kActSigmoid: return "sigmoid"; default: return "-"; }
}
bool same_dims(const TensorInfo& a, const TensorInfo& b) { for (int i = 0; i < 4; i++) if (a.dims[i] != b.dims[i]) return false; return true; }
bool is_chan_vec(const TensorInfo& v, const TensorInfo& full) { return v.dims[1] == 1 && v.dims[2] == 1 && v.dims[3] == full.dims[3] && (full.dims[1] * full.dims[2] > 1); }

int round_up(int v, int m) { return (v + m - 1) / m * m; }

}

std::string Plan::describe() const {
  static const char* kn[] = {"conv", "pwconv", "dwconv", "gap", "eltwise", "resize", "concat", "tconv"};
  std::string s;
  char line[512];
  int i = 0;
  for (const Step& st : steps) {
    snprintf(line, sizeof line, "%3d %-7s %-26s in %dx%dx%d -> out %dx%dx%d k%dx%d s%d d%d act=%s res=%d scale=%d macs=%.0f t%d->t%d\n", i++,
             kn[(int)st.kind], st.label.c_str(), st.H, st.W, st.Cin, st.OH, st.OW, st.Cout, st.kh, st.kw, st.sh, st.dh, act_name(st.act),
             st.residual, st.in_scale, st.macs, st.in0, st.out);
    s += line;
    if (st.fuse_head0) { s += "      ^ fused with steps 1 and 2 (stem + depthwise + 1x1 in one tiled kernel)\n"; }
    if (st.chain_first >= 0) {
      snprintf(line, sizeof line, "      ^ chained with steps %d and %d at 8192 pixels and more (three 1x1 convolutions in one kernel: the tensors between them stay in registers)\n", st.chain_first, st.chain_last);
      s += line;
    }
    if (st.fuse_dw >= 0) {
      const Step& dd = steps[st.fuse_dw];
      const IrGeom ig = ir_geometry(st.OH, st.OW, st.Cout, dd.OH, dd.sh, dd.dh);
      snprintf(line, sizeof line, "      ^ fused with step %d (expand + depthwise in one kernel: %d channels x %d rows per workgroup, %d band(s))\n", st.fuse_dw, ig.CH, ig.BH, ig.nbands);
      s.insert(s.size() - 1, "");
      s += line;
    }
  }
  return s;
}

static void lower_frame_program(const Graph& g, Plan* plan, const std::vector<Step>& steps, const std::vector<int>& ext, const std::map<int, int>& part_n,
                                const std::map<int, int>& part_hw, const int scratch, const unsigned policy = 0) {
  const bool long_to_hbm = (policy & 1u) != 0, elide_expand = (policy & 2u) != 0, small_top = (policy & 4u) != 0;
  const int kLdsTotal = plan->lds_total_floats, kLdsZero = plan->lds_zero_off();
  plan->program.clear();
  plan->program_scratch_floats = scratch;
  plan->program_labels.clear();
  plan->program_out_tensor.clear();
  plan->program_blocks.clear();
  plan->program_check.clear();
  plan->program_ext_offs.clear();
  for (int t : ext) if (t >= 0 && plan->tensor_off[t] >= 0) plan->program_ext_offs.push_back(plan->tensor_off[t]);
  const int NS = (int)steps.size();
  const int NT = (int)g.tensors.size();
  std::vector<int> last(NT, -1);
  for (int s = 0; s < NS; s++) {
    const Step& st = steps[s];
    if ((st.kind == StepKind::PwConv || st.kind == StepKind::Eltwise || st.kind == StepKind::DwConv || st.kind == StepKind::Gap ||
         st.kind == StepKind::TConv) && (st.Cin % 4)) return;
    if (st.out_bias >= 0) return;
    for (int t : {st.in0, st.in1, st.in2, st.residual, st.in_scale, st.out}) if (t >= 0) last[t] = s;
    for (int t : st.concat_in) last[t] = s;
  }
  last[g.output] = NS + 1;
  for (int t : ext) if (t >= 0) last[t] = NS + 1;
  auto padded = [&](int t) { const TensorInfo& ti = g.tensors[t]; const int C = ti.dims[3], P = ti.dims[1] * ti.dims[2]; return (P * (C + (((C / 4) % 2 == 0) ? 4 : 8)) + 3) / 4 * 4; };
  std::vector<char> elide(NS, 0);
  if (elide_expand)
    for (int s = 0; s + 1 < NS; s++) {
      const Step& a = steps[s];
      const Step& d = steps[s + 1];
      if (!(a.kind == StepKind::PwConv && a.residual < 0 && a.out >= 0 && last[a.out] == s + 1 && d.kind == StepKind::DwConv && d.in0 == a.out && d.residual < 0 && d.dh == 1 && d.dw == 1)) continue;
      if (a.out == g.output || std::find(ext.begin(), ext.end(), a.out) != ext.end() || g.tensors[a.out].dims[3] % 8 || a.cout_pad < (g.tensors[a.out].dims[3] + 15) / 16 * 16) continue;
      const int P = g.tensors[a.out].dims[1] * g.tensors[a.out].dims[2], need = padded(a.out), need_o = padded(d.out), ws = (P * 20 + 3) / 4 * 4 , room = kLdsTotal - scratch - 2 * kLdsMaxStageFloats;
      if (need + need_o > room && (need_o > room ? ws : need_o + ws) <= room) {
        elide[s] = 1;
        for (int t : {a.in0, a.in2, a.in_scale}) if (t >= 0) last[t] = std::max(last[t], s + 1);
      }
    }
  const bool no_lds = BSX_DBG_ENV("BSX_PROGRAM_NO_LDS") != nullptr;
  std::vector<Loc> loc(NT);
  struct Blk { int off, len, until; };
  std::vector<Blk> live;
  std::map<int, int> reserved_at;
  int reserved = 0;
  std::vector<int> firstdef(NT, -1);
  for (int s = 0; s < NS; s++) if (steps[s].out >= 0 && firstdef[steps[s].out] < 0) firstdef[steps[s].out] = s;
  if (!BSX_DBG_ENV("BSX_PLAN_NO_TOPDOWN")) {
    for (int t = 0; t < NT; t++) {
      if (firstdef[t] < 0 || last[t] - firstdef[t] <= 8 || t == g.input || t == g.output) continue;
      if (std::find(ext.begin(), ext.end(), t) != ext.end()) continue;
      const TensorInfo& ti = g.tensors[t];
      const int C = ti.dims[3], P = ti.dims[1] * ti.dims[2];
      if (C % 4 || P <= 1) continue;
      const int pad = ((C / 4) % 2 == 0) ? 4 : 8, need = (P * (C + pad) + 3) / 4 * 4;
      if (reserved + need > kLdsTotal / 4) continue;
      reserved += need;
      reserved_at[t] = kLdsZero - reserved;
    }
  }
  const int cap = kLdsZero - reserved;
  int high = scratch;
  auto place = [&](int t, int s) {
    if (t < 0 || loc[t].space != kLocNone) return;
    const TensorInfo& ti = g.tensors[t];
    int C = ti.dims[3], P = ti.dims[1] * ti.dims[2];
    Loc l;
    l.elems = (int)ti.elems();
    bool lds_ok = (C % 4 == 0) && t != g.input && t != g.output && !no_lds;
    int pad = ((C / 4) % 2 == 0) ? 4 : 8;
    int stride = P > 1 ? C + pad : C;
    int need = (P * stride + 3) / 4 * 4;
    if (need > kLdsTotal - scratch - 2 * kLdsMaxStageFloats && !BSX_DBG_ENV("BSX_PLAN_NO_SLOT_RESERVE")) lds_ok = false;
    if (long_to_hbm && lds_ok && reserved_at.find(t) == reserved_at.end() && firstdef[t] >= 0 && last[t] - firstdef[t] > 8 && P > 1 &&
        std::find(ext.begin(), ext.end(), t) == ext.end()) lds_ok = false;
    if (lds_ok && s >= 0 && s < NS && elide[s] && steps[s].out == t) lds_ok = false;
    if (lds_ok) {
      live.erase(std::remove_if(live.begin(), live.end(), [&](const Blk& b) { return b.until < s; }), live.end());
      std::sort(live.begin(), live.end(), [](const Blk& a, const Blk& b) { return a.off < b.off; });
      int pos = scratch;
      auto rz = reserved_at.find(t);
      if (rz != reserved_at.end()) pos = rz->second;
      else if (small_top && need <= kLdsTotal / 6) {
        pos = cap + 1;
        int hi = cap;
        for (int k = (int)live.size() - 1; k >= -1; k--) {
          const int lo = k >= 0 ? live[k].off + live[k].len : scratch;
          if (hi - lo >= need) { pos = hi - need; break; }
          if (k >= 0) hi = std::min(hi, live[k].off);
        }
      } else
      for (const Blk& b : live) { if (pos + need <= b.off) break; pos = std::max(pos, b.off + b.len); }
      if (rz != reserved_at.end() || pos + need <= cap) {
        l.space = kLocLds; l.off = pos; l.stride = stride;
        if (rz == reserved_at.end()) live.push_back({pos, need, last[t]});
        plan->program_blocks.push_back({pos, need, s, last[t], "tensor " + std::to_string(t)});
        high = std::max(high, pos + need);
        plan->program_lds_tensors++;
        loc[t] = l;
        return;
      }
    }
    l.space = t == g.input ? kLocInput : (t == g.output ? kLocOutput : kLocGlobal);
    l.off = (int)plan->tensor_off[t]; l.stride = C;
    plan->program_global_tensors++;
    loc[t] = l;
  };
  plan->program_lds_tensors = plan->program_global_tensors = 0;
  place(g.input, -1);
  for (int t : ext) {
    if (t < 0 || loc[t].space != kLocNone) continue;
    const TensorInfo& ti = g.tensors[t];
    Loc l;
    l.elems = (int)ti.elems(); l.space = kLocGlobal; l.off = (int)plan->tensor_off[t]; l.stride = ti.dims[3];
    loc[t] = l;
    plan->program_global_tensors++;
  }
  auto gemv_form = [&](const Step& st) { return st.kind == StepKind::PwConv && st.in2 < 0 && st.OH * st.OW <= 4 && st.OH * st.OW * st.Cout * 16 <= kLdsScratchFloats; };
  std::vector<int> stage(NS, 0), slot(NS, 0);
  std::vector<std::vector<int>> slots_from(NS);
  for (int s = 0; s < NS; s++) {
    const Step& st = steps[s];
    long nb = st.kind == StepKind::DwConv ? st.Cout : (st.kind == StepKind::TConv ? st.Cout : st.cout_pad);
    long range = ((long)st.b_off - (long)st.w_off) + ((nb + 3) / 4) * 4;
    if (st.kind == StepKind::PwConv && st.OH * st.OW == 1 && st.w2_off > st.b_off && !BSX_DBG_ENV("BSX_NO_FC_STAGE")) {
      auto fc1px = [&](int k) { const Step& f = steps[k]; return f.kind == StepKind::PwConv && f.OH * f.OW == 1; };
      int q0 = s;
      while (q0 > 0 && fc1px(q0 - 1)) q0--;
      const long frange = ((long)st.w2_off - (long)st.b_off) + (long)st.Cout * st.Cin;
      if (q0 > 0 && s - q0 <= 1 && steps[q0 - 1].kind == StepKind::Gap && frange <= kLdsMaxStageFloats) {
        stage[s] = (int)((frange + 3) / 4 * 4);
        slots_from[std::max(q0 - 2, 0)].push_back(s);
      }
      continue;
    }
    bool uses = (st.kind == StepKind::PwConv && !gemv_form(st)) || st.kind == StepKind::Conv || st.kind == StepKind::DwConv || st.kind == StepKind::TConv;
    if (st.kind == StepKind::PwConv && st.cout_pad % 16 != 0) uses = false;
    if (!(uses && st.b_off > st.w_off && range <= kLdsMaxStageFloats)) continue;
    stage[s] = (int)range;
    int q = s > 0 ? s - 1 : 0;
    auto fc_like = [&](int k) { const Step& f = steps[k]; return f.kind == StepKind::PwConv && f.OH * f.OW == 1; };
    if (s > 0 && fc_like(q)) {
      while (q > 0 && fc_like(q - 1)) q--;
      if (q > 0 && steps[q - 1].kind == StepKind::Gap) q--;
    }
    if (s > 2 && steps[s - 1].kind == StepKind::TConv && steps[s - 2].kind == StepKind::DwConv) q = std::min(q, s - 3);
    slots_from[q].push_back(s);
  }
  std::vector<MicroOp> prog;
  std::vector<std::string> labels;
  std::vector<int> out_t;
  std::vector<int> tail_ws(NS, -1), tail_rows(NS, 0);
  auto tail_pattern = [&](int s) {
    if (s + 2 >= NS || BSX_DBG_ENV("BSX_PROGRAM_NO_TAIL")) return false;
    const Step& a = steps[s];
    const Step& b = steps[s + 1];
    const Step& c2 = steps[s + 2];
    return a.kind == StepKind::PwConv && a.residual < 0 && a.Cin == 16 && a.cout_pad == 16 && a.Cout == 16 &&
           a.OH * a.OW > 1024 && last[a.out] == s + 1 &&
           b.kind == StepKind::DwConv && b.in0 == a.out && b.residual == a.out && b.kh == 3 && b.kw == 3 && b.sh == 1 && b.sw == 1 && b.dh == 1 &&
           b.dw == 1 && b.pad_t == 1 && b.pad_l == 1 && last[b.out] == s + 2 &&
           c2.kind == StepKind::TConv && c2.in0 == b.out && c2.kh == 2 && c2.kw == 2 && c2.Cout <= 4 &&
           c2.OH == 2 * c2.H && c2.OW == 2 * c2.W;
  };
  for (int s = 0; s < NS; s++) {
    const Step& st = steps[s];
    for (int s2 : slots_from[s]) {
      const int need = (stage[s2] + 3) / 4 * 4;
      live.erase(std::remove_if(live.begin(), live.end(), [&](const Blk& b) { return b.until < s; }), live.end());
      std::sort(live.begin(), live.end(), [](const Blk& a, const Blk& b) { return a.off < b.off; });
      int pos = -1, hi = cap;
      if (!BSX_DBG_ENV("BSX_PLAN_NO_TOPDOWN")) {
        for (int k = (int)live.size() - 1; k >= -1; k--) {
          const int lo = k >= 0 ? live[k].off + live[k].len : scratch;
          if (hi - lo >= need) { pos = hi - need; break; }
          if (k >= 0) hi = std::min(hi, live[k].off);
        }
        if (pos < 0) pos = cap;
      } else {
        pos = scratch;
        for (const Blk& b : live) { if (pos + need <= b.off) break; pos = std::max(pos, b.off + b.len); }
      }
      if (pos + need <= cap) {
        const int until = elide[s2] ? s2 + 1 : s2;
        slot[s2] = pos; live.push_back({pos, need, until}); high = std::max(high, pos + need);
        plan->program_blocks.push_back({pos, need, s, until, "weights of step " + std::to_string(s2)});
      }
      else stage[s2] = 0;
    }
    if (tail_pattern(s)) {
      auto need_for = [&](int r) { return (r + 2) * st.W * (st.Cout + 4); };
      live.erase(std::remove_if(live.begin(), live.end(), [&](const Blk& b) { return b.until < s; }), live.end());
      std::sort(live.begin(), live.end(), [](const Blk& a, const Blk& b) { return a.off < b.off; });
      const int rmax = BSX_DBG_ENV("BSX_TAIL_ROWS") ? atoi(BSX_DBG_ENV("BSX_TAIL_ROWS")) : 16;
      for (int R = rmax; R >= 1 && tail_ws[s] < 0; R = R > 4 ? R - 2 : R - 1) {
        const int need = need_for(R);
        if ((R + 2) * st.W > 64 * 16 * 4) continue;
        int pos = scratch;
        for (const Blk& b : live) { if (pos + need <= b.off) break; pos = std::max(pos, b.off + b.len); }
        if (pos + need <= cap) {
          tail_ws[s] = pos; tail_rows[s] = R; live.push_back({pos, need, s + 2}); high = std::max(high, pos + need);
          plan->program_blocks.push_back({pos, need, s, s + 2, "tail band of step " + std::to_string(s)});
        }
      }
    }
    place(st.out, s);
    MicroOp m;
    m.kind = (int)st.kind;
    m.H = st.H; m.W = st.W; m.Cin = st.Cin; m.OH = st.OH; m.OW = st.OW; m.Cout = st.Cout;
    m.kh = st.kh; m.kw = st.kw; m.sh = st.sh; m.sw = st.sw; m.dh = st.dh; m.dw = st.dw; m.pt = st.pad_t; m.pl = st.pad_l;
    m.act = st.act; m.elt = st.elt; m.bcast1 = st.bcast1; m.align_corners = st.align_corners; m.half_pixel = st.half_pixel;
    m.cout_pad = st.cout_pad; m.cout_tile = st.cout_tile;
    m.w_off = (long long)st.w_off; m.b_off = (long long)st.b_off; m.w2_off = (long long)st.w2_off;
    m.gemv = gemv_form(st) ? 1 : 0;
    m.strip = (st.kind == StepKind::DwConv && !BSX_DBG_ENV("BSX_NO_DW_STRIP")) ? 1 : 0;
    auto L = [&](int t) { return t >= 0 ? loc[t] : Loc(); };
    m.in0 = L(st.in0); m.in1 = L(st.in1); m.in2 = L(st.in2); m.res = L(st.residual); m.scale = L(st.in_scale); m.out = L(st.out);
    if (st.concat_in.size() > 4) return;
    m.n_cat = (int)st.concat_in.size();
    m.gap_sum = st.gap_sum ? 1 : 0;
    for (int k = 0; k < m.n_cat; k++) {
      const int ct = st.concat_in[k];
      m.cat[k] = L(ct); m.cat_c[k] = st.concat_c[k];
      m.cat_hw[k] = g.tensors[ct].dims[1] * g.tensors[ct].dims[2];
      auto pn = part_n.find(ct);
      if (pn != part_n.end()) { m.cat_parts[k] = pn->second; m.cat_hw[k] = part_hw.at(ct); }
    }
    if (st.kind == StepKind::DwConv && !((st.kh == 3 && st.kw == 3) || (st.kh == 5 && st.kw == 5))) return;
    m.stage_floats = stage[s]; m.w_lds = slot[s];
    if (st.kind == StepKind::PwConv && st.OH * st.OW == 1 && st.w2_off > st.b_off) {
      m.fc_stage[0] = stage[s]; m.fc_lds[0] = slot[s]; m.stage_floats = 0; m.w_lds = 0;
    }
    if (st.kind == StepKind::PwConv && !m.gemv) {
      m.cout_tile = 16;
      m.mfma = (st.cout_pad % 16 == 0 && m.stage_floats > 0) ? 1 : 0;
      if (!m.mfma) m.stage_floats = 0;
    }
    if (st.kind == StepKind::Conv && m.stage_floats > 0 && st.cout_pad % 16 == 0 && m.in0.space != kLocLds && st.residual < 0 &&
        st.dh == 1 && st.dw == 1 && st.kh * st.kw * st.Cin <= 256) {
      const int rowf = st.W * st.Cin;
      int band = 16;
      auto need_for = [&](int b) { return ((b - 1) * st.sh + st.kh) * rowf + 3 * (((st.kh * st.kw * st.Cin + 3) / 4) * 4) + 8; };
      auto band_floats = [&](int b) { return ((b - 1) * st.sh + st.kh) * rowf; };
      while (band > 1 && band_floats(band) > 8192) band /= 2;
      const int need = (need_for(band) + 3) / 4 * 4;
      live.erase(std::remove_if(live.begin(), live.end(), [&](const Blk& b) { return b.until < s; }), live.end());
      std::sort(live.begin(), live.end(), [](const Blk& a, const Blk& b) { return a.off < b.off; });
      int pos = scratch;
      for (const Blk& b : live) { if (pos + need <= b.off) break; pos = std::max(pos, b.off + b.len); }
      if (pos + need <= cap && band_floats(band) <= 8192) {
        m.mfma = 1; m.ws_off = pos; m.band_rows = band;
        live.push_back({pos, need, s});
        plan->program_blocks.push_back({pos, need, s, s, "stem band of step " + std::to_string(s)});
        high = std::max(high, pos + need);
      }
    }
    if (st.kind == StepKind::DwConv && m.strip && m.in0.space == kLocGlobal && st.dh == 1 && st.dw == 1 && st.residual < 0 && !BSX_DBG_ENV("BSX_PLAN_NO_DW_STAGE")) {
      live.erase(std::remove_if(live.begin(), live.end(), [&](const Blk& b) { return b.until < s; }), live.end());
      std::sort(live.begin(), live.end(), [](const Blk& a, const Blk& b) { return a.off < b.off; });
      for (int CK : {32, 16}) {
        if (m.band_rows || (st.Cin % CK) % 8) continue;
        const int need = (st.H * st.W * (CK + 4) + 3) / 4 * 4;
        int pos = scratch;
        for (const Blk& b : live) { if (pos + need <= b.off) break; pos = std::max(pos, b.off + b.len); }
        if (pos + need <= cap) {
          m.ws_off = pos; m.band_rows = CK;
          live.push_back({pos, need, s});
          plan->program_blocks.push_back({pos, need, s, s, "depthwise input chunk of step " + std::to_string(s)});
          high = std::max(high, pos + need);
        }
      }
    }
    if (m.scale.space != kLocNone && m.scale.space != kLocLds) return;
    if (BSX_DBG_ENV("BSX_PROGRAM_NOP")) m.kind = 99;
    if (const char* only = BSX_DBG_ENV("BSX_PROGRAM_ONLY")) { if (atoi(only) != s) m.kind = 99; }
    prog.push_back(m);
    out_t.push_back(st.out);
    {
      char buf[200];
      snprintf(buf, sizeof buf, "%-12s %dx%dx%d->%dx%dx%d%s%s in:%s out:%s", st.label.c_str(), st.H, st.W, st.Cin, st.OH, st.OW, st.Cout,
               m.mfma ? " mfma" : "", m.gemv ? " gemv" : "", m.in0.space == kLocLds ? "lds" : "hbm", m.out.space == kLocLds ? "lds" : "hbm");
      labels.push_back(buf);
    }
  }
  if (!BSX_DBG_ENV("BSX_PROGRAM_NO_SE")) {
    std::vector<MicroOp> fusedp;
    std::vector<std::string> flabels;
    std::vector<int> fout;
    for (size_t i = 0; i < prog.size(); i++) {
      const MicroOp& g0 = prog[i];
      auto is_fc = [&](size_t k, const Loc& in) {
        if (k >= prog.size()) return false;
        const MicroOp& f = prog[k];
        const Step& st = steps[k];
        return f.kind == (int)StepKind::PwConv && f.OH * f.OW == 1 && st.w2_off != 0 && f.res.space == kLocNone && f.scale.space == kLocNone &&
               f.in0.space == kLocLds && f.in0.off == in.off && (f.out.space == kLocLds || f.out.space == kLocGlobal) && f.Cin % 4 == 0;
      };
      auto single_use = [&](size_t k) { const Step& st = steps[k]; return last[st.out] == (int)k + 1; };
      if (tail_ws[i] >= 0 && prog[i].mfma && prog[i].out.space == kLocGlobal && prog[i].scale.space != kLocGlobal) {
        MicroOp m = prog[i];
        const MicroOp& d = prog[i + 1];
        const MicroOp& t = prog[i + 2];
        m.kind = kMicroTail; m.mfma = 0; m.stage_floats = 0;
        m.w3_off = d.w_off; m.b3_off = d.b_off; m.act2 = d.act;
        m.w4_off = t.w_off; m.b4_off = t.b_off; m.act3 = t.act; m.C2 = t.Cout;
        m.OH = t.OH; m.OW = t.OW; m.out = t.out;
        m.ws_off = tail_ws[i]; m.band_rows = tail_rows[i];
        m.magic_w = (unsigned)((0x100000000ull + (unsigned long long)m.W - 1) / (unsigned long long)m.W);
        fusedp.push_back(m);
        flabels.push_back("tail[pw+dw+tconv] " + labels[i]);
        fout.push_back(out_t[i + 2]);
        i += 2;
        continue;
      }
      if (g0.kind == (int)StepKind::Gap && g0.out.space == kLocLds && is_fc(i + 1, g0.out) && single_use(i)) {
        MicroOp m = g0;
        const MicroOp& f1 = prog[i + 1];
        m.kind = kMicroSe; m.in1 = g0.out; m.in2 = f1.out; m.n_fc = 1;
        m.w2_off = (long long)steps[i + 1].w2_off; m.b_off = f1.b_off; m.act = f1.act; m.C1 = f1.Cout; m.out = f1.out;
        m.fc_stage[0] = f1.fc_stage[0]; m.fc_lds[0] = f1.fc_lds[0]; m.fc_stage[1] = 0;
        size_t used = 2;
        if (is_fc(i + 2, f1.out) && single_use(i + 1)) {
          const MicroOp& f2 = prog[i + 2];
          m.n_fc = 2; m.w3_off = (long long)steps[i + 2].w2_off; m.b3_off = f2.b_off; m.act2 = f2.act; m.C2 = f2.Cout; m.out = f2.out;
          m.fc_stage[1] = f2.fc_stage[0]; m.fc_lds[1] = f2.fc_lds[0];
          used = 3;
        }
        fusedp.push_back(m);
        flabels.push_back("se[" + std::to_string(m.n_fc) + "fc" + (m.fc_stage[0] ? "+w1" : "") + (m.fc_stage[1] ? "+w2" : "") + "] " + labels[i]);
        fout.push_back(out_t[i + used - 1]);
        i += used - 1;
      } else {
        fusedp.push_back(g0);
        flabels.push_back(labels[i]);
        fout.push_back(out_t[i]);
      }
    }
    prog.swap(fusedp);
    labels.swap(flabels);
    out_t.swap(fout);
  }
  plan->program = std::move(prog);
  plan->program_labels = std::move(labels);
  plan->program_out_tensor = std::move(out_t);
  plan->program_lds_floats = high;
  if (BSX_DBG_ENV("BSX_PLAN_DEBUG"))
    for (const auto& b : plan->program_blocks) fprintf(stderr, "lds block [%6d, %6d) steps [%2d, %2d] %s\n", b.off, b.off + b.len, b.from, b.until, b.what.c_str());
  plan->program_check = verify_program_lds(*plan);
  if (plan->program_check != "ok") plan->program.clear();
}

static long program_arena_bytes(const Plan& plan) {
  long b = 0;
  const int n = (int)plan.program.size();
  for (int i = 0; i < n; i++) {
    const MicroOp& m = plan.program[i];
    const bool out_elided = mid_pw_feeds_dw(plan, i), in_elided = i > 0 && mid_pw_feeds_dw(plan, i - 1);
    const long reps = out_elided ? (plan.program[i + 1].Cin + plan.program[i + 1].band_rows - 1) / plan.program[i + 1].band_rows : 1;
    for (const Loc* l : {&m.in0, &m.in1, &m.in2, &m.res, &m.out}) {
      if (l->space != kLocGlobal || (l == &m.out && out_elided) || (l == &m.in0 && in_elided)) continue;
      b += 4L * l->elems * (l == &m.out ? 1 : reps);
    }
    for (int c = 0; c < m.n_cat; c++) if (m.cat[c].space == kLocGlobal && m.cat_parts[c] == 0) b += 4L * m.cat[c].elems;
  }
  return b;
}
static void build_frame_program(const Graph& g, Plan* plan, const std::vector<Step>& steps, const std::vector<int>& ext = {},
                                const std::map<int, int>& part_n = {}, const std::map<int, int>& part_hw = {}) {
  auto lower = [&](unsigned policy) {
    lower_frame_program(g, plan, steps, ext, part_n, part_hw, kLdsScratchFloats, policy);
    if (plan->program.empty() || BSX_DBG_ENV("BSX_PLAN_FULL_SCRATCH")) return;
    for (const MicroOp& m : plan->program)
      if ((m.kind == (int)StepKind::PwConv && m.gemv) || m.kind == kMicroTail || m.kind == (int)StepKind::Conv) return;
    lower_frame_program(g, plan, steps, ext, part_n, part_hw, 64, policy);
    if (plan->program.empty()) lower_frame_program(g, plan, steps, ext, part_n, part_hw, kLdsScratchFloats, policy);
  };
  if (const char* force = BSX_DBG_ENV("BSX_PLAN_POLICY")) { plan->program_policy = (unsigned)atoi(force) & 7u; lower(plan->program_policy); plan->program_arena_bytes = program_arena_bytes(*plan); return; }
  unsigned best = 0;
  long best_b = -1;
  for (unsigned pol = 0; pol < 8; pol++) {
    lower(pol);
    if (plan->program.empty()) continue;
    const long b = program_arena_bytes(*plan);
    if (best_b < 0 || b < best_b) { best_b = b; best = pol; }
  }
  lower(best);
  plan->program_policy = best;
  plan->program_arena_bytes = program_arena_bytes(*plan);
}

std::string verify_program_lds(const Plan& plan) {
  const auto& b = plan.program_blocks;
  for (size_t i = 0; i < b.size(); i++) {
    if (b[i].off < plan.program_scratch_floats || b[i].off + b[i].len > plan.lds_zero_off() || b[i].len <= 0 || b[i].from > b[i].until)
      return "block out of range: " + b[i].what;
    for (size_t j = i + 1; j < b.size(); j++) {
      const bool time = b[i].from <= b[j].until && b[j].from <= b[i].until;
      const bool mem = b[i].off < b[j].off + b[j].len && b[j].off < b[i].off + b[i].len;
      if (time && mem) return "overlap: " + b[i].what + " [" + std::to_string(b[i].from) + "," + std::to_string(b[i].until) + "] and " + b[j].what + " [" +
                              std::to_string(b[j].from) + "," + std::to_string(b[j].until) + "]";
    }
  }
  for (const MicroOp& m : plan.program) {
    for (const Loc* l : {&m.in0, &m.in1, &m.in2, &m.res, &m.scale, &m.out})
      if (l->space == kLocLds && (l->off < plan.program_scratch_floats || l->off >= plan.program_lds_floats)) return "operand outside the LDS block area";
    if (m.stage_floats > 0 && (m.w_lds < plan.program_scratch_floats || m.w_lds + m.stage_floats > plan.program_lds_floats)) return "weight slot outside the LDS block area";
  }
  return "ok";
}


namespace {

bool resize_weights_uniform(int in, int out, bool align, bool half_pixel) {
  std::vector<double> wsum(in, 0.0);
  const float scale = (align && out > 1) ? (float)(in - 1) / (float)(out - 1) : (float)in / (float)out;
  for (int o = 0; o < out; o++) {
    const float v = half_pixel ? ((float)o + 0.5f) * scale - 0.5f : (float)o * scale;
    const float fl = std::floor(v);
    const int lo = std::max((int)fl, 0), hi = std::min((int)std::ceil(v), in - 1);
    const float frac = v - (float)lo;
    wsum[lo] += 1.0 - frac; wsum[hi] += frac;
  }
  const double want = (double)out / (double)in;
  for (double x : wsum) if (std::fabs(x - want) > 1e-5) return false;
  return true;
}

SegConvW conv_w(const Step& st) { SegConvW c; c.w_off = (long long)st.w_off; c.b_off = (long long)st.b_off; c.Cin = st.kh * st.kw * st.Cin; c.Cout = st.Cout; c.cout_pad = st.cout_pad; c.act = st.act; return c; }
SegDwW dw_w(const Step& st) { SegDwW c; c.w_off = (long long)st.w_off; c.b_off = (long long)st.b_off; c.C = st.Cout; c.act = st.act; return c; }
SegFc fc_w(const Step& st) { SegFc c; c.w_off = (long long)st.w2_off; c.b_off = (long long)st.b_off; c.Cin = st.Cin; c.Cout = st.Cout; c.act = st.act; return c; }

bool is_pw16(const Step& st) { return st.kind == StepKind::PwConv && st.Cin == 16 && st.Cout == 16 && st.cout_pad == 16 && st.OH * st.OW > 4; }
bool is_fc_step(const Step& st) { return st.kind == StepKind::PwConv && st.OH * st.OW == 1 && st.w2_off != 0 && st.residual < 0 && st.in_scale < 0 && st.in2 < 0 && st.Cin <= 32 && st.Cin % 8 == 0 && st.Cout <= 32; }
bool is_dw3(const Step& st, int stride) {
  return st.kind == StepKind::DwConv && st.kh == 3 && st.kw == 3 && st.sh == stride && st.sw == stride && st.dh == 1 && st.dw == 1;
}
int tiles_for(int extent, int target) { return (extent + target - 1) / target; }

}

static bool seg_fail(int where) { if (BSX_DBG_ENV("BSX_SEG_DEBUG")) fprintf(stderr, "segmentation: check %d failed\n", where); return false; }
static bool build_segments(Graph& g, Plan* plan) {
  const std::vector<Step>& S = plan->steps;
  const int NS = (int)S.size();
  if (NS < 9 + 15) return seg_fail(1);
  auto uses_of = [&](int t) {
    int n = 0;
    for (const Step& q : S) {
      for (int u : {q.concat_in.empty() ? q.in0 : -1, q.in1, q.in2, q.residual, q.in_scale}) n += (u == t);
      for (int u : q.concat_in) n += (u == t);
    }
    return n + (t == g.output);
  };
  auto dims = [&](int t, int k) { return g.tensors[t].dims[k]; };

  const Step &stem = S[0], &hpw = S[1], &hdw = S[2];
  if (!(stem.kind == StepKind::Conv && stem.in0 == g.input && stem.kh == 3 && stem.kw == 3 && stem.sh == 2 && stem.sw == 2 && stem.dh == 1 && stem.dw == 1 &&
        stem.Cin == 3 && stem.Cout == 16 && stem.cout_pad == 16 && stem.residual < 0)) return seg_fail(2);
  const int A = stem.out;
  if (!(is_pw16(hpw) && hpw.in0 == A && hpw.residual < 0 && hpw.in_scale < 0 && hpw.in2 < 0 && uses_of(hpw.out) == 1)) return seg_fail(3);
  if (!(is_dw3(hdw, 2) && hdw.in0 == hpw.out && hdw.Cout == 16 && hdw.residual < 0)) return seg_fail(4);
  const int b0 = hdw.out;
  const Step &g1 = S[3], &f1a = S[4], &f1b = S[5], &pwa = S[6], &pwb = S[7], &kdw = S[8];
  if (!(g1.kind == StepKind::Gap && g1.concat_in.empty() && g1.in0 == b0 && is_fc_step(f1a) && f1a.in0 == g1.out && is_fc_step(f1b) && f1b.in0 == f1a.out &&
        f1a.Cin == 16 && f1b.Cout == 16 && uses_of(b0) == 2)) return seg_fail(5);
  if (!(is_pw16(pwa) && pwa.in0 == b0 && pwa.in_scale == f1b.out && pwa.residual < 0 && pwa.in2 < 0 && uses_of(f1b.out) == 1)) return seg_fail(6);
  const int B = pwa.out;
  if (!(pwb.kind == StepKind::PwConv && pwb.in0 == B && pwb.Cin == 16 && pwb.cout_pad % 16 == 0 && pwb.residual < 0 && pwb.in_scale < 0 && pwb.in2 < 0 &&
        uses_of(pwb.out) == 1 && pwb.Cout % 4 == 0)) return seg_fail(7);
  if (!(is_dw3(kdw, 2) && kdw.in0 == pwb.out && kdw.residual < 0)) return seg_fail(8);
  const int c0 = kdw.out;
  const Step &tr = S[NS - 7], &tg = S[NS - 6], &tf1 = S[NS - 5], &tf2 = S[NS - 4], &tpw = S[NS - 3], &tdw = S[NS - 2], &ttc = S[NS - 1];
  if (!(tr.kind == StepKind::Resize && tr.Cin == 16 && tr.OH == dims(A, 1) && tr.OW == dims(A, 2))) return seg_fail(9);
  const int lo = tr.in0, up = tr.out;
  auto pools = [](const Step& q, int a, int b) { return q.kind == StepKind::Gap && q.concat_in.size() == 2 && ((q.concat_in[0] == a && q.concat_in[1] == b) || (q.gap_sum && q.concat_in[0] == b && q.concat_in[1] == a)); };
  if (!(pools(tg, A, up) && is_fc_step(tf1) && tf1.in0 == tg.out &&
        is_fc_step(tf2) && tf2.in0 == tf1.out && tf2.Cout == 16)) return seg_fail(10);
  if (!(is_pw16(tpw) && tpw.in0 == A && tpw.in_scale == tf2.out && tpw.in2 == up && tpw.residual < 0)) return seg_fail(11);
  if (!(is_dw3(tdw, 1) && tdw.in0 == tpw.out && tdw.residual == tpw.out && tdw.Cout == 16 && tdw.pad_t == 1 && tdw.pad_l == 1)) return seg_fail(12);
  if (!(ttc.kind == StepKind::TConv && ttc.in0 == tdw.out && ttc.kh == 2 && ttc.kw == 2 && ttc.Cin == 16 && (ttc.Cout == 1 || ttc.Cout == 2) && ttc.out == g.output)) return seg_fail(13);
  if (uses_of(A) != 3 || uses_of(up) != 2 || uses_of(tpw.out) != 2 || uses_of(tdw.out) != 1 || uses_of(tf2.out) != 1) return seg_fail(14);
  if (!resize_weights_uniform(tr.H, tr.OH, tr.align_corners, tr.half_pixel) || !resize_weights_uniform(tr.W, tr.OW, tr.align_corners, tr.half_pixel)) return seg_fail(15);
  const Step &kr = S[NS - 14], &kg = S[NS - 13], &kf1 = S[NS - 12], &kf2 = S[NS - 11], &kp1 = S[NS - 10], &kd = S[NS - 9], &kp2 = S[NS - 8];
  if (!(kr.kind == StepKind::Resize && kr.Cin == 16 && kr.OH == dims(B, 1) && kr.OW == dims(B, 2))) return seg_fail(16);
  const int lo2 = kr.in0, up2 = kr.out;
  if (!(pools(kg, B, up2) && is_fc_step(kf1) && kf1.in0 == kg.out &&
        is_fc_step(kf2) && kf2.in0 == kf1.out && kf2.Cout == 16)) return seg_fail(17);
  if (!(is_pw16(kp1) && kp1.in0 == B && kp1.in_scale == kf2.out && kp1.in2 == up2 && kp1.residual < 0)) return seg_fail(18);
  if (!(is_dw3(kd, 1) && kd.in0 == kp1.out && kd.residual == kp1.out && kd.Cout == 16 && kd.pad_t == 1 && kd.pad_l == 1)) return seg_fail(19);
  if (!(is_pw16(kp2) && kp2.in0 == kd.out && kp2.out == lo && kp2.residual < 0 && kp2.in_scale < 0 && kp2.in2 < 0)) return seg_fail(20);
  if (uses_of(B) != 3 || uses_of(up2) != 2 || uses_of(kp1.out) != 2 || uses_of(kd.out) != 1 || uses_of(kf2.out) != 1 || uses_of(lo) != 1 || uses_of(lo2) != 1) return seg_fail(21);
  if (!resize_weights_uniform(kr.H, kr.OH, kr.align_corners, kr.half_pixel) || !resize_weights_uniform(kr.W, kr.OW, kr.align_corners, kr.half_pixel)) return seg_fail(22);
  if (uses_of(c0) != 1) return seg_fail(23);
  auto clampish = [](int a) { return a == kActNone || a == kActRelu || a == kActRelu6; };
  if (!(clampish(stem.act) || stem.act == kActHswish) || !(ttc.act == kActNone || ttc.act == kActSigmoid) || (ttc.act == kActSigmoid && ttc.Cout != 1)) return seg_fail(34);
  for (const Step* q : {&hpw, &hdw, &pwa, &pwb, &kdw, &kp1, &kd, &kp2, &tpw, &tdw}) if (!clampish(q->act)) return seg_fail(35);

  size_t top = plan->arena_floats_per_stream;
  auto reserve = [&](size_t floats) { size_t at = top; top += (floats + 63) / 64 * 64; return (long long)at; };
  auto synth = [&](const char* name, int n, int C) {
    TensorInfo t; t.dims[0] = 1; t.dims[1] = n; t.dims[2] = 1; t.dims[3] = C; t.shape = {1, n, 1, C}; t.name = name;
    g.tensors.push_back(t);
    plan->tensor_off.push_back(-1);
    return (int)g.tensors.size() - 1;
  };
  SegPlan sp;
  int tgt[8] = {4, 14, 4, 7, 16, 14, 18, 14};
  if (const char* e = BSX_DBG_ENV("BSX_SEG_TILES")) sscanf(e, "%d,%d,%d,%d,%d,%d,%d,%d", &tgt[0], &tgt[1], &tgt[2], &tgt[3], &tgt[4], &tgt[5], &tgt[6], &tgt[7]);
  auto split = [&](int extent, int target, int* tile, int* n) { *n = tiles_for(extent, std::max(1, target)); *tile = (extent + *n - 1) / *n; };

  SegHead& h = sp.head;
  h.H0 = stem.H; h.W0 = stem.W; h.H1 = stem.OH; h.W1 = stem.OW; h.H2 = hdw.OH; h.W2 = hdw.OW;
  h.stem_pt = stem.pad_t; h.stem_pl = stem.pad_l; h.dw_pt = hdw.pad_t; h.dw_pl = hdw.pad_l;
  h.stem = conv_w(stem); h.pw = conv_w(hpw); h.dw = dw_w(hdw);
  split(h.H2, tgt[0], &h.TR, &h.tiles_y); split(h.W2, tgt[1], &h.TC, &h.tiles_x);
  h.lds_floats = seg_head_lds_floats(h);
  h.rw = seg_row_width(2 * h.TC + 1); h.m_ct = (65536u + (unsigned)(h.rw / 16) - 1) / (unsigned)(h.rw / 16);
  if (h.TR > 4 || h.TC > 15 || (4 * h.TC + 3) * 3 > 192) return seg_fail(30);
  SegK2& k2 = sp.k2;
  k2.H2 = hdw.OH; k2.W2 = hdw.OW; k2.H3 = kdw.OH; k2.W3 = kdw.OW; k2.dw_pt = kdw.pad_t; k2.dw_pl = kdw.pad_l;
  k2.pw_a = conv_w(pwa); k2.pw_b = conv_w(pwb); k2.dw = dw_w(kdw);
  split(k2.H3, tgt[2], &k2.TR, &k2.tiles_y); split(k2.W3, tgt[3], &k2.TC, &k2.tiles_x);
  k2.lds_floats = seg_k2_lds_floats(k2);
  k2.wst = seg_k2_stage(k2, k2.lds_floats, dbg_env_int(BSX_DBG_ENV("BSX_K2_LDS_CAP"), 160 * 1024), BSX_DBG_ENV("BSX_K2_GLOBAL_W") ? 0 : 2);
  k2.lds_floats += k2.wst.floats;
  k2.rw = seg_row_width(2 * k2.TC + 1); k2.m_ct = (65536u + (unsigned)(k2.rw / 16) - 1) / (unsigned)(k2.rw / 16);
  if (k2.TC > 15 || ((2 * k2.TR + 1) * (k2.rw / 16) + 3) / 4 > 6) return seg_fail(31);
// ... 640 lines not shown
```

backscrub_amd/csrc/plan.hpp:

```cpp
#pragma once
#include "debug_switches.hpp"
#include <cstdio>
#include <cstdlib>
#include <cstddef>
#include <string>
#include <vector>

#include "frame_program.hpp"
#include "segments.hpp"
#include "tflite_model.hpp"

namespace bsx {

enum class StepKind : int { Conv = 0, PwConv, DwConv, Gap, Eltwise, Resize, Concat, TConv };
enum EltOp : int { kEltAdd = 0, kEltMul = 1, kEltUnary = 2, kEltMulAdd = 3 };

struct Step {
  StepKind kind = StepKind::Conv;
  std::string label;
  int in0 = -1, in1 = -1, in2 = -1;
  int out = -1;
  int residual = -1;
  int in_scale = -1;
  int out_bias = -1;
  int H = 1, W = 1, Cin = 1, OH = 1, OW = 1, Cout = 1;
  int kh = 1, kw = 1, sh = 1, sw = 1, dh = 1, dw = 1, pad_t = 0, pad_l = 0;
  int act = kActNone;
  int elt = kEltAdd;
  bool bcast1 = false;
  bool align_corners = false, half_pixel = false;
  int cout_pad = 0;
  int cout_tile = 16;
  size_t w_off = 0, b_off = 0;
  size_t w2_off = 0;
  size_t w16_off = 0;
  int k16_pad = 0;
  std::vector<int> concat_in;
  std::vector<int> concat_c;
  bool gap_sum = false;
  double macs = 0;
  int last_node = -1;
  int fuse_dw = -1;
  bool in_from_fused_dw = false;
  bool fused_away = false;
  bool fuse_head0 = false;
  int chain_first = -1, chain_last = -1;
  int chain_mid = -1;
  size_t chain_w16_off = 0;
};
constexpr int kChainS0 = 5, kChainP1 = 8, kChainP2 = 8;
inline size_t chain3_stream_halves() { return (size_t)(kChainS0 * 4 * kChainP1 + kChainP2 * (4 * kChainP1 + 4)) * 512; }

struct IrGeom { int CH = 0, BH = 0, nbands = 0, rows = 0; };
inline long ir_stage_floats(int CH) { return CH == 32 ? 8 * 512 : 0; }
inline long ir_lds_bytes(int rows, int W, int CH) { return ((long)rows * W * CH + 10 * CH + 4 + ir_stage_floats(CH)) * 4; }
inline IrGeom ir_geometry(int H, int W, int Cexp, int OH, int S, int d) {
  if (const char* e = BSX_DBG_ENV("BSX_IR_GEOM")) {
    int w = 0, ch = 0, bh = 0;
    if (sscanf(e, "%d:%d,%d", &w, &ch, &bh) == 3 && w == W && ch > 0 && Cexp % ch == 0 && bh > 0) {
      IrGeom g; g.CH = ch; g.BH = bh < OH ? bh : OH; g.nbands = (OH + g.BH - 1) / g.BH;
      const int r = S * (g.BH - 1) + 2 * d + 1; g.rows = r < H ? r : H;
      if (ir_lds_bytes(g.rows, W, ch) <= 160 * 1024) return g;
    }
  }
  auto rows_for = [&](int bh) { const int r = S * (bh - 1) + 2 * d + 1; return r < H ? r : H; };
  for (int CH : {32, 24, 16}) {
    if (Cexp % CH) continue;
    if (ir_lds_bytes(rows_for(OH), W, CH) <= 160 * 1024) { IrGeom g; g.CH = CH; g.BH = OH; g.nbands = 1; g.rows = rows_for(OH); return g; }
  }
  IrGeom best;
  double best_score = 0;
  for (int CH : {32, 24, 16}) {
    if (Cexp % CH) continue;
    int BH = OH;
    while (BH > 1 && ir_lds_bytes(rows_for(BH), W, CH) > 80 * 1024) BH--;
    if (ir_lds_bytes(rows_for(BH), W, CH) > 80 * 1024 || BH < 2) continue;
    const int nb = (OH + BH - 1) / BH;
    BH = (OH + nb - 1) / nb;
    const double score = (double)(S * BH) / rows_for(BH) * CH / ((CH + 15) / 16 * 16);
    if (score > best_score) { best_score = score; best.CH = CH; best.BH = BH; best.nbands = nb; best.rows = rows_for(BH); }
  }
  return best;
}

inline long head0_lds_floats(int W0, int W1, int bh) {
  const long in_t = (((2l * (bh + 2) + 1) * (W0 + 2) * 3 + 3) & ~3l), dband = (long)bh * W1 * 16;
  return (in_t > dband ? in_t : dband) + (long)(bh + 2) * W1 * 16 + 1024;
}
inline int head0_band_rows(int W0, int W1) {
  if (const char* e = BSX_DBG_ENV("BSX_H0_BH")) { const int bh = atoi(e); if (bh >= 1 && bh <= 8 && head0_lds_floats(W0, W1, bh) * 4 <= 156 * 1024) return bh; }
  for (int bh = 8; bh >= 2; bh--)
    if (head0_lds_floats(W0, W1, bh) * 4 <= 80 * 1024) return bh;
  for (int bh = 8; bh >= 2; bh--)
    if (head0_lds_floats(W0, W1, bh) * 4 <= 156 * 1024) return bh;
  return 0;
}

struct Plan {
  std::vector<Step> steps;
  std::vector<float> weights;
  std::vector<uint16_t> weights16;
  std::vector<long> tensor_off;
  std::vector<long> tensor_elems;
  size_t arena_floats_per_stream = 0;
  int input = -1, output = -1;
  double macs_per_frame = 0;
  std::vector<MicroOp> program;
  std::vector<std::string> program_labels;
  std::vector<int> program_out_tensor;
  int mid_lanes = kFrameThreads;
  int lds_total_floats = kLdsTotalFloats;
  int lds_zero_off() const { return lds_total_floats - kLdsZeroFloats; }
  int program_lds_floats = 0;
  int program_scratch_floats = 0;
  int program_lds_tensors = 0, program_global_tensors = 0;
  std::vector<long> program_ext_offs;
  struct LdsBlock { int off, len, from, until; std::string what; };
  std::vector<LdsBlock> program_blocks;
  std::string program_check;
  SegPlan seg;
  unsigned program_policy = 0;
  long program_arena_bytes = 0;
  std::string seg_text;
  std::vector<int> seg_stored;
  std::vector<int> seg_partials;
  std::string describe() const;
};

struct MidGeometry { int lanes, lds_floats; };
MidGeometry mid_geometry_default();

std::string verify_program_lds(const Plan& plan);

bool build_plan(const Graph& g, Plan* plan, std::string* err, bool reuse_arena = true, bool segments = true);

}
```

backscrub_amd/csrc/specialised.cpp:

```cpp
#include "specialised.hpp"

#include "debug_switches.hpp"

#include <algorithm>
#include <cstdio>
#include <cstdlib>

#include "gen_mid.hpp"
#include "gen_seg.hpp"
#include "rtc.hpp"

namespace bsx {

KernelVariant kernel_variant(const Plan& plan) {
  const char* a16 = getenv("BSX_ACT16");
  KernelVariant v;
  v.act16 = a16 && atoi(a16) != 0 && plan.seg.on;
  v.u8in = BSX_DBG_ENV("BSX_F32_INPUT") == nullptr;
  return v;
}

namespace {

bool compile(SpecialisedCode* part, const std::string& arch, const char* what, size_t cut) {
  std::string log;
  if (rtc_build(part->source, arch, &part->code, &log, &part->cached)) return true;
  if (BSX_DBG_ENV("BSX_RTC_DEBUG")) fprintf(stderr, "%s\n", log.c_str());
  part->code.clear();
  part->fallback = std::string(what) + " (hipRTC: " + log.substr(0, cut) + ")";
  return false;
}

void build_mid(const Plan& plan, bool act16, const std::string& arch, SpecialisedBuild* b) {
  int force = -1;
  if (const char* e = BSX_DBG_ENV("BSX_RTC_TID")) force = atoi(e) != 0;
  auto form = [&](bool opaque, SpecialisedCode* m, long* scratch) {
    m->source = generate_mid_source(plan, &m->why, act16, opaque);
    if (m->source.empty()) { m->fallback = "interpreted (" + m->why + ")"; return false; }
    if (!compile(m, arch, "interpreted", 400)) return false;
    *scratch = code_object_scratch_bytes(m->code, "bsx_mid");
    return true;
  };
  if (!form(force == 1, &b->mid, &b->scratch)) return;
  b->opaque_tid = force == 1;
  if (force >= 0 || b->scratch <= 0) return;
  SpecialisedCode alt;
  long alt_scratch = -1;
  if (form(true, &alt, &alt_scratch) && alt_scratch >= 0 && alt_scratch < b->scratch) { b->mid = std::move(alt); b->scratch = alt_scratch; b->opaque_tid = true; }
}

void build_seg(const Plan& plan, KernelVariant v, const std::string& arch, SpecialisedCode* s) {
  s->source = generate_seg_source(plan, v.act16, v.u8in, &s->why);
  if (BSX_DBG_ENV("BSX_NO_SEG_RTC")) s->fallback = "ahead-of-time kernels (BSX_NO_SEG_RTC)";
  else if (s->source.empty()) s->fallback = "ahead-of-time kernels (" + s->why + ")";
  else compile(s, arch, "ahead-of-time kernels", 600);
}

bool load_module(const std::vector<char>& code, const char* const* names, int n, hipModule_t* mod, hipFunction_t* fn) {
  hipModule_t m = nullptr;
  if (hipModuleLoadData(&m, code.data()) != hipSuccess) { (void)hipGetLastError(); return false; }
  hipFunction_t f[5] = {};
  for (int i = 0; i < n; i++) {
    if (hipModuleGetFunction(&f[i], m, names[i]) != hipSuccess) { (void)hipModuleUnload(m); (void)hipGetLastError(); return false; }
  }
  *mod = m;
  std::copy(f, f + n, fn);
  return true;
}

}

SpecialisedBuild build_specialised(const Plan& plan, KernelVariant v, const std::string& arch, unsigned parts) {
  SpecialisedBuild b;
  if (parts & kBuildMid) build_mid(plan, v.act16, arch, &b);
  if (parts & kBuildSeg) build_seg(plan, v, arch, &b.seg);
  b.seg_k3_frame = plan.seg.on && plan.seg.k3f.on;
  return b;
}

void no_specialised(const char* why, SpecialisedKernels* k) {
  k->mid_note = std::string("interpreted (") + why + ")";
  k->seg_note = std::string("ahead-of-time kernels (") + why + ")";
}

void load_specialised(const SpecialisedBuild& b, SpecialisedKernels* k) {
  static const char* const kMid[] = {"bsx_mid"};
  static const char* const kSeg[] = {"bsx_seg_head", "bsx_seg_k2", "bsx_seg_k3", "bsx_seg_tail", "bsx_seg_k3f"};
  k->mid_note = b.mid.fallback;
  if (!b.mid.code.empty()) {
    if (!load_module(b.mid.code, kMid, 1, &k->mid_mod, &k->mid)) k->mid_note = "interpreted (code object did not load)";
    else k->mid_note = std::string("specialised kernel (hipRTC") + (b.mid.cached ? ", from the cache" : ", compiled now") + (b.opaque_tid ? ", lane indices re-derived per op" : "") +
                       (b.scratch > 0 ? ", " + std::to_string(b.scratch) + " B of scratch" : "") + ")";
  }
  k->seg_note = b.seg.fallback;
  if (!b.seg.code.empty()) {
    hipFunction_t fn[5] = {};
    if (!load_module(b.seg.code, kSeg, b.seg_k3_frame ? 5 : 4, &k->seg_mod, fn)) k->seg_note = "ahead-of-time kernels (code object did not load)";
    else {
      std::copy(fn, fn + 4, k->seg);
      k->k3_frame = fn[4];
    }
    if (k->seg_mod) k->seg_note = std::string("specialised kernels (hipRTC") + (b.seg.cached ? ", from the cache)" : ", compiled now)");
  }
}

void unload_specialised(SpecialisedKernels* k) {
  if (k->mid_mod) (void)hipModuleUnload(k->mid_mod);
  if (k->seg_mod) (void)hipModuleUnload(k->seg_mod);
  *k = SpecialisedKernels{};
}

}
```

backscrub_amd/csrc/specialised.hpp:

```cpp
#pragma once
#include <hip/hip_runtime.h>

#include <string>
#include <vector>

#include "plan.hpp"

namespace bsx {

struct KernelVariant {
  bool act16 = false;
  bool u8in = false;
};
KernelVariant kernel_variant(const Plan& plan);

struct SpecialisedCode {
  std::string source;
  std::string why;
  std::vector<char> code;
  std::string fallback;
  bool cached = false;
};

struct SpecialisedBuild {
  SpecialisedCode mid, seg;
  bool opaque_tid = false;
  bool seg_k3_frame = false;
  long scratch = -1;
};
enum : unsigned { kBuildMid = 1, kBuildSeg = 2 };
SpecialisedBuild build_specialised(const Plan& plan, KernelVariant v, const std::string& arch, unsigned parts = kBuildMid | kBuildSeg);

struct SpecialisedKernels {
  hipModule_t mid_mod = nullptr, seg_mod = nullptr;
  hipFunction_t mid = nullptr;
  hipFunction_t seg[4] = {};
  hipFunction_t k3_frame = nullptr;
  std::string mid_note, seg_note;
};
void no_specialised(const char* why, SpecialisedKernels* k);
void load_specialised(const SpecialisedBuild& b, SpecialisedKernels* k);
void unload_specialised(SpecialisedKernels* k);

}
```

Before: 741,600 frames/s.

## Fuse stride-1 depthwise into following 1x1 MFMA conv via registers

Adds an op_dw_pw device body that computes each stride-1 depthwise output chunk in registers and feeds it straight into the 1x1 convolution's MFMA accumulation. The intermediate tensor is never written to LDS or HBM. The planner marks candidate pairs, lowers the program with and without early weight staging, and keeps whichever needs less arena. The build falls back to the unfused kernel if the fused form needs scratch or fails to compile. This removes a store/load round trip and a barrier per pair, but raises register pressure and recomputes the depthwise for each output tile row.

```diff
diff --git a/backscrub_amd/csrc/bsx_api.hip b/backscrub_amd/csrc/bsx_api.hip
--- a/backscrub_amd/csrc/bsx_api.hip
+++ b/backscrub_amd/csrc/bsx_api.hip
@@ -421,7 +421,8 @@
   BSX_HIP(c, hipStreamWaitEvent(s, ev, 0));
   return BSX_OK;
 }
-bool program_op_elided(const bsx_ctx* c, int i) { return c->kern.mid && !BSX_DBG_ENV("BSX_RTC_FINE") && mid_pw_feeds_dw(c->plan, i); }
+static bool program_op_in_registers(const bsx_ctx* c, int i) { return c->kern.mid && c->kern.dwpw && mid_dw_feeds_pw(c->plan, i); }
+bool program_op_elided(const bsx_ctx* c, int i) { return (c->kern.mid && !BSX_DBG_ENV("BSX_RTC_FINE") && mid_pw_feeds_dw(c->plan, i)) || program_op_in_registers(c, i); }
 
 bool debug_tensor_half(const bsx_ctx* c, int t) {
   const Plan& p = c->plan;
@@ -1551,7 +1552,7 @@
       c->plan_text += "P" + std::to_string(i) + " " + c->plan.program_labels[i];
       if (i < c->plan.program_out_tensor.size()) {
         const int sp = c->plan.program[i].out.space;
-        c->plan_text += " -> t" + std::to_string(c->plan.program_out_tensor[i]) + (sp == kLocLds ? " lds" : (program_op_elided(c.get(), (int)i) ? " elided" : (sp == kLocOutput ? " output" : " hbm")));
+        c->plan_text += " -> t" + std::to_string(c->plan.program_out_tensor[i]) + (program_op_in_registers(c.get(), (int)i) ? " elided" : sp == kLocLds ? " lds" : (program_op_elided(c.get(), (int)i) ? " elided" : (sp == kLocOutput ? " output" : " hbm")));
         if (sp == kLocGlobal && !program_op_elided(c.get(), (int)i) && debug_tensor_half(c.get(), c->plan.program_out_tensor[i])) c->plan_text += " f16";
       }
       c->plan_text += "\n";
@@ -2185,7 +2186,8 @@
              p.program_lds_floats, p.program_lds_tensors, p.program_global_tensors, p.program_arena_bytes, p.program_policy, p.program_blocks.size(), p.program_check.c_str());
     out += head;
     for (size_t i = 0; i < p.program_labels.size(); i++)
-      out += "P" + std::to_string(i) + " " + p.program_labels[i] + (i < p.program_out_tensor.size() ? " -> t" + std::to_string(p.program_out_tensor[i]) : std::string()) + "\n";
+      out += "P" + std::to_string(i) + " " + p.program_labels[i] + (i < p.program_out_tensor.size() ? " -> t" + std::to_string(p.program_out_tensor[i]) : std::string()) +
+             (mid_dw_feeds_pw(p, (int)i) ? " elided" : "") + "\n";
     if (p.seg.on) out += p.seg_text;
     if (!p.program.empty()) out += mid_barrier_line(p, false);
     if (BSX_DBG_ENV("BSX_PLAN_BLOCKS"))
@@ -2247,8 +2249,9 @@
         if (b.seg.fallback.find("hipRTC:") != std::string::npos) { snprintf(msg, cap, "%s", seg_msg.c_str()); return BSX_EMODEL; }
       }
     }
-    snprintf(msg, cap, "%s (%zu bytes of source, %zu bytes of code object, %ld B of scratch%s, cache %s)%s", b.mid.cached ? "cached" : "compiled", b.mid.source.size(),
-             b.mid.code.size(), b.scratch, b.opaque_tid ? ", lane indices re-derived per op" : "", rtc_cache_dir().c_str(), seg_msg.c_str());
+    snprintf(msg, cap, "%s (%zu bytes of source, %zu bytes of code object, %ld B of scratch%s%s, cache %s)%s", b.mid.cached ? "cached" : "compiled", b.mid.source.size(),
+             b.mid.code.size(), b.scratch, b.opaque_tid ? ", lane indices re-derived per op" : "", b.dwpw_declined.empty() ? "" : (", depthwise -> 1x1 pairs as two ops (" + b.dwpw_declined + ")").c_str(),
+             rtc_cache_dir().c_str(), seg_msg.c_str());
     return BSX_OK;
   } catch (...) { snprintf(msg, cap, "exception while reading the model"); return BSX_EMODEL; }
 }
@@ -2264,6 +2267,7 @@
     if (p.seg.on && std::find(p.seg_partials.begin(), p.seg_partials.end(), t) != p.seg_partials.end()) return nullptr;
     for (size_t i = 0; i < p.program.size() && i < p.program_out_tensor.size(); i++) {
       if (p.program_out_tensor[i] != t) continue;
+      if (program_op_in_registers(c, (int)i)) return "the specialised middle kernel computes it in registers inside the 1x1 convolution that reads it";
       if (p.program[i].out.space == kLocLds) return "the frame program keeps it in LDS";
       if (p.program[i].out.space != kLocGlobal) return "the frame program writes it to a buffer of its own";
       if (program_op_elided(c, (int)i)) return "the specialised middle kernel computes it chunk by chunk inside the depthwise that reads it";
diff --git a/backscrub_amd/csrc/gen_mid.cpp b/backscrub_amd/csrc/gen_mid.cpp
--- a/backscrub_amd/csrc/gen_mid.cpp
+++ b/backscrub_amd/csrc/gen_mid.cpp
@@ -76,7 +76,46 @@
   return true;
 }
 
-std::string generate_mid_source(const Plan& plan, std::string* why, bool act16, bool opaque_tid) {
+bool mid_dw_feeds_pw(const Plan& plan, int j) {
+  const std::vector<MicroOp>& P = plan.program;
+  const int n = (int)P.size();
+  auto disjoint = [](long a0, long a1, long b0, long b1) { return a1 <= b0 || b1 <= a0; };
+  if (BSX_DBG_ENV("BSX_RTC_NO_DWPW") || BSX_DBG_ENV("BSX_RTC_EXP_MFMA") || j < 0 || j + 1 >= n) return false;
+  const MicroOp& d = P[j];
+  const MicroOp& a = P[j + 1];
+  if (j >= (int)plan.program_out_tensor.size() || std::find(plan.program_dwpw_out.begin(), plan.program_dwpw_out.end(), plan.program_out_tensor[j]) == plan.program_dwpw_out.end()) return false;
+  if (!(d.kind == (int)StepKind::DwConv && dw_geom_ok(d) && d.sh == 1 && d.in0.space == kLocLds && (d.out.space == kLocGlobal || d.out.space == kLocLds) && (d.res.space == kLocNone || d.res.space == kLocLds) && d.stage_floats > 0 &&
+        (d.Cin % 16 == 0 || d.Cin % 16 == 8) && d.Cout == d.Cin)) return false;
+  if (!(a.kind == (int)StepKind::PwConv && a.mfma && !a.gemv && a.stage_floats > 0 && a.in0.space == d.out.space && a.in0.off == d.out.off && a.Cin == d.Cout && a.H * a.W == d.OH * d.OW &&
+        a.OH * a.OW == a.H * a.W && a.scale.space == kLocNone && a.in2.space == kLocNone && a.in1.space == kLocNone && a.cout_pad % 16 == 0 && a.n_cat == 0)) return false;
+  if (((long)a.H * a.W + 15) / 16 > plan.mid_lanes / 64) return false;
+  if (a.res.space == d.out.space && a.res.off == d.out.off) return false;
+  if (d.out.space == kLocGlobal) {
+    for (long e : plan.program_ext_offs) if (e == d.out.off) return false;
+    for (int q = j + 2; q < n; q++) {
+      for (const Loc* l : {&P[q].in0, &P[q].in1, &P[q].in2, &P[q].res, &P[q].scale}) if (l->space == kLocGlobal && l->off == d.out.off) return false;
+      for (int c = 0; c < P[q].n_cat; c++) if (P[q].cat[c].space == kLocGlobal && P[q].cat[c].off == d.out.off) return false;
+      if (P[q].out.space == kLocGlobal && P[q].out.off == d.out.off) break;
+    }
+  }
+  const long pix = (long)a.H * a.W;
+  std::vector<std::pair<long, long>> reads;
+  reads.push_back({d.in0.off, d.in0.off + (long)d.H * d.W * d.in0.stride});
+  reads.push_back({d.w_lds, d.w_lds + d.stage_floats});
+  reads.push_back({a.w_lds, a.w_lds + a.stage_floats});
+  if (d.res.space == kLocLds) reads.push_back({d.res.off, d.res.off + pix * d.res.stride});
+  if (!disjoint(d.w_lds, d.w_lds + d.stage_floats, a.w_lds, a.w_lds + a.stage_floats)) return false;
+  if (a.res.space == kLocLds) {
+    const long r0 = a.res.off, r1 = a.res.off + pix * a.res.stride;
+    if (!disjoint(r0, r1, reads[1].first, reads[1].second) || !disjoint(r0, r1, reads[2].first, reads[2].second)) return false;
+    if (a.out.space == kLocLds && !disjoint(r0, r1, a.out.off, a.out.off + pix * a.out.stride) && !(a.out.off == a.res.off && a.out.stride == a.res.stride)) return false;
+  }
+  if (a.out.space == kLocLds)
+    for (auto& r : reads) if (!disjoint(r.first, r.second, a.out.off, a.out.off + pix * a.out.stride)) return false;
+  return true;
+}
+
+std::string generate_mid_source(const Plan& plan, std::string* why, bool act16, bool opaque_tid, bool dwpw) {
   auto asp = [&](const Loc& l) { const int sp = sp_of(l); return (sp == 2 && act16) ? 3 : sp; };
   auto loc = [&](Out& o, const char* p, const Loc& l) { o.f("  static constexpr int %s_SP = %d, %s_OFF = %d, %s_ST = %d;\n", p, asp(l), p, l.off, p, l.stride); };
   auto fail = [&](const std::string& m) { if (why) *why = m; return std::string(); };
@@ -101,7 +140,12 @@
       if (m.fc_stage[1] > 0) dst.f("  stage<%d>(W + %lld, L + %d);\n", m.fc_stage[1], m.b3_off, m.fc_lds[1]);
     }
   };
-  stage_of(0, k);
+  auto dw_feeds_pw = [&](int j) { return dwpw && !fine && mid_dw_feeds_pw(plan, j); };
+  auto stage_for = [&](int i, Out& dst) {
+    stage_of(i, dst);
+    if (i + 1 < n && plan.program_dwpw_early && dw_feeds_pw(i)) stage_of(i + 1, dst);
+  };
+  stage_for(0, k);
   auto dw_chunked = [&](const MicroOp& d) { return mid_dw_chunked(d); };
   (void)dw_chunked;
   auto pw_feeds_dw = [&](int j) { return !fine && mid_pw_feeds_dw(plan, j); };
@@ -114,7 +158,8 @@
     k.f("  // ---- P%d %s\n", i, i < (int)plan.program_labels.size() ? comment_safe(plan.program_labels[i]).c_str() : "");
     if (fine) k.f("  f_b = __builtin_readcyclecounter();\n");
     const bool fed_by_prev = i > 0 && pw_feeds_dw(i - 1);
-    if (i + 1 < n && !fed_by_prev) stage_of(i + 1, k);
+    const bool fused_dw = dw_feeds_pw(i), fused_pw = i > 0 && dw_feeds_pw(i - 1);
+    if (i + 1 < n && !fed_by_prev && !(fused_dw && plan.program_dwpw_early)) stage_for(i + 1, k);
     auto fc_loads = [&](int j) {
       const MicroOp& q = P[j];
       auto fcl = [&](int which, int cin, int cout, int stage, int lds, long long w2, long long b) {
@@ -129,7 +174,7 @@
       if (j <= 0 || j >= n || P[j].kind != kMicroSe || P[j].fc_stage[0] > 0 || P[j].fc_stage[1] > 0) return false;
       if (BSX_DBG_ENV("BSX_RTC_NO_EARLY_FC")) return false;
       const MicroOp& pv = P[j - 1];
-      if (pv.kind == (int)StepKind::PwConv && pv.mfma && !pv.gemv) return true;
+      if (pv.kind == (int)StepKind::PwConv && pv.mfma && !pv.gemv) return !(j >= 2 && dw_feeds_pw(j - 2));
       if (pv.kind != (int)StepKind::DwConv || pv.in0.space != kLocLds) return false;
       const int K = pv.kh, S = pv.sh, V = K == 5 ? 2 : 4, TX = (S == 1 && !(pv.OW % 5 != 0 && pv.OW % 4 == 0)) ? 5 : 4, NIN = (TX - 1) * S + K;
       return K * (NIN + K) * V <= 144;
@@ -138,12 +183,17 @@
     if (m.kind == (int)StepKind::PwConv && m.mfma && !m.gemv) {
       if (m.Cin % 4 || m.Cout % 4 || m.cout_pad % 16 || m.stage_floats <= 0) return fail("pw: channel counts / unstaged weights");
       if (m.scale.space != kLocNone && m.scale.space != kLocLds) return fail("pw: scale vector outside LDS");
+      if (m.out.space == kLocLds && m.res.space == kLocLds) {
+        const long px = (long)m.OH * m.OW, o0 = m.out.off, o1 = o0 + px * m.out.stride, r0 = m.res.off, r1 = r0 + px * m.res.stride;
+        if (!(o1 <= r0 || r1 <= o0) && !(o0 == r0 && m.out.stride == m.res.stride)) return fail("pw: output overlaps its residual");
+      }
       o.f("struct Op%d {\n  static constexpr int P = %d, CIN = %d, COUT = %d, CPAD = %d, ACT = %d;\n", i, m.OH * m.OW, m.Cin, m.Cout, m.cout_pad, m.act);
       loc(o, "X", m.in0); loc(o, "Y", m.out); loc(o, "R", m.res); loc(o, "D", m.in2);
       o.f("  static constexpr int S_OFF = %d, W_LDS = %d, B_LDS = %d;\n", m.scale.space == kLocLds ? m.scale.off : -1, m.w_lds, m.w_lds + (int)(m.b_off - m.w_off));
       o.f("  static constexpr int N0 = 0, NCOLS = %d, YSUB = 0;\n", m.cout_pad);
       o.f("  static constexpr bool NFAST = %s;\n};\n", ((m.out.space == kLocGlobal && !BSX_DBG_ENV("BSX_RTC_NO_NFAST")) || (m.in0.space == kLocGlobal && m.cout_pad > 16 && !BSX_DBG_ENV("BSX_RTC_NO_NFAST_IN"))) ? "true" : "false");
       if (pw_feeds_dw(i)) k.f("  // (computed chunk by chunk inside P%d: the tensor between them is never written)\n", i + 1);
+      else if (fused_pw) k.f("  op_dw_pw<Op%d, Op%d>(L, A);      // depthwise P%d and this 1x1 as one body\n", i - 1, i, i - 1);
       else k.f("  op_pw<Op%d>(L, A);\n", i);
     } else if (m.kind == (int)StepKind::DwConv) {
       const bool ok = m.strip && m.dh == 1 && m.dw == 1 && m.kh == m.kw && (m.kh == 3 || m.kh == 5) && m.sh == m.sw && (m.sh == 1 || m.sh == 2) && m.Cin % 4 == 0;
@@ -176,11 +226,12 @@
             o.f("  static constexpr int S_OFF = %d, W_LDS = %d, B_LDS = %d;\n", a.scale.space == kLocLds ? a.scale.off : -1, a.w_lds, a.w_lds + (int)(a.b_off - a.w_off));
             o.f("  static constexpr int N0 = %d, NCOLS = %d, YSUB = %d;\n  static constexpr bool NFAST = true;\n};\n", c * CK, (CKc + 15) / 16 * 16, c * CK);
             k.f("  op_pw<Op%d_%d>(L, A);\n  __syncthreads();\n", i - 1, c);
-            if (c == nch - 1 && i + 1 < n) stage_of(i + 1, k);
+            if (c == nch - 1 && i + 1 < n) stage_for(i + 1, k);
           } else
             k.f("  load_chunk<%d, %d, %d, %d, %d, %d, %d, %d>(L, A);\n  __syncthreads();\n", asp(m.in0), m.in0.off, m.H * m.W, m.in0.stride, CKc, c * CK, m.ws_off, CK + 4);
         }
-        k.f("  op_dw<%s>(L, A, W);\n", name);
+        if (fused_dw) k.f("  // (runs inside P%d, which feeds its outputs to the matrix cores from registers: the tensor between them is never formed)\n", i + 1);
+        else k.f("  op_dw<%s>(L, A, W);\n", name);
       }
     } else if (m.kind == kMicroSe) {
       if (m.in1.space != kLocLds || (m.n_fc == 2 && m.in2.space != kLocLds) || m.Cin % 4 || m.C1 % 1) return fail("se: mean / hidden vectors outside LDS");
diff --git a/backscrub_amd/csrc/gen_mid.hpp b/backscrub_amd/csrc/gen_mid.hpp
--- a/backscrub_amd/csrc/gen_mid.hpp
+++ b/backscrub_amd/csrc/gen_mid.hpp
@@ -5,9 +5,10 @@
 
 namespace bsx {
 
-std::string generate_mid_source(const Plan& plan, std::string* why, bool act16 = false, bool opaque_tid = false);
+std::string generate_mid_source(const Plan& plan, std::string* why, bool act16 = false, bool opaque_tid = false, bool dwpw = true);
 
 bool mid_dw_chunked(const MicroOp& d);
 bool mid_pw_feeds_dw(const Plan& plan, int j);
+bool mid_dw_feeds_pw(const Plan& plan, int j);
 
 }
diff --git a/backscrub_amd/csrc/mid_prelude.hip b/backscrub_amd/csrc/mid_prelude.hip
--- a/backscrub_amd/csrc/mid_prelude.hip
+++ b/backscrub_amd/csrc/mid_prelude.hip
@@ -299,6 +299,109 @@
   }
 }
 
+template <class D, class T> __device__ __forceinline__ void op_dw_pw(lds_f* L, glb_f* A) {
+  constexpr int P = T::P, CIN = T::CIN, CPAD = T::CPAD, MT = (P + 15) / 16, NT = T::NCOLS / 16;
+  constexpr int NJ = CIN / 16, TAIL = CIN % 16, TM = TAIL / 4, K = D::K;
+  static_assert(CPAD % 16 == 0 && (TAIL == 0 || TAIL == 8), "op_dw_pw: channel counts");
+  static_assert(D::S == 1 && D::X_SP == SP_LDS && D::W_SP == SP_LDS && (D::R_SP == SP_NONE || D::R_SP == SP_LDS) && D::C == CIN && D::CW == CIN && D::OH * D::OW == P, "op_dw_pw: depthwise form");
+  static_assert(T::S_OFF < 0 && T::D_SP == SP_NONE && T::N0 == 0 && T::YSUB == 0, "op_dw_pw: 1x1 form");
+  const int lane = tid_now() & 63, li = lane & 15, g = lane >> 4, wave = wave_id();
+  const lds_f* wl = L + T::W_LDS;
+  const lds_f* bl = L + T::B_LDS;
+#pragma unroll
+  for (int it = 0; it < (MT + kWaves - 1) / kWaves; it++) {
+    const int tm = wave + it * kWaves;
+    if (tm >= MT) break;
+    const int m0 = tm << 4;
+    const int arow = (P % 16 == 0) ? m0 + li : min(m0 + li, P - 1);
+    const int oy = arow / D::OW, ox = arow - oy * D::OW;
+    f4v acc0[NT], acc1[NT];
+#pragma unroll
+    for (int tn = 0; tn < NT; tn++) { acc0[tn] = (f4v)(0.f); acc1[tn] = (f4v)(0.f); }
+    auto tap = [&](int fy, int fx, int* xo, int* wo) {
+      const int iy = oy - D::PT + fy, ix = ox - D::PL + fx;
+      const bool in = iy >= 0 && iy < D::H && ix >= 0 && ix < D::W;
+      *xo = in ? D::X_OFF + (iy * D::W + ix) * D::X_ST : kZeroOff;
+      *wo = D::W_OFF + (fy * K + fx) * D::CW;
+      return in;
+    };
+#pragma unroll
+    for (int j = 0; j < NJ; j++) {
+      const int ch = 16 * j + 4 * g;
+      f4v acc = (f4v)(0.f);
+#pragma unroll
+      for (int fy = 0; fy < K; fy++) {
+#pragma unroll
+        for (int fx = 0; fx < K; fx++) {
+          int xo, wo;
+          const bool in = tap(fy, fx, &xo, &wo);
+          acc = __builtin_elementwise_fma(*(const lds_v4*)(L + xo + (in ? ch : 0)), *(const lds_v4*)(L + wo + ch), acc);
+        }
+      }
+      __builtin_amdgcn_sched_barrier(0);
+      float b[NT][4];
+#pragma unroll
+      for (int tn = 0; tn < NT; tn++) {
+        const lds_f* bp = wl + (4 * g) * CPAD + (tn << 4) + li;
+        const lds_f* br = bp + (16 * j) * CPAD;
+        b[tn][0] = br[0]; b[tn][1] = br[CPAD]; b[tn][2] = br[2 * CPAD]; b[tn][3] = br[3 * CPAD];
+      }
+      f4v aj = act4<D::ACT>(acc + *(const lds_v4*)(L + D::B_OFF + ch));
+      if constexpr (D::R_SP != SP_NONE) aj += *(const lds_v4*)(L + D::R_OFF + arow * D::R_ST + ch);
+#pragma unroll
+      for (int tn = 0; tn < NT; tn++) {
+        f4v& c = (j & 1) ? acc1[tn] : acc0[tn];
+        c = __builtin_amdgcn_mfma_f32_16x16x4f32(b[tn][0], aj.x, c, 0, 0, 0);
+        c = __builtin_amdgcn_mfma_f32_16x16x4f32(b[tn][1], aj.y, c, 0, 0, 0);
+        c = __builtin_amdgcn_mfma_f32_16x16x4f32(b[tn][2], aj.z, c, 0, 0, 0);
+        c = __builtin_amdgcn_mfma_f32_16x16x4f32(b[tn][3], aj.w, c, 0, 0, 0);
+      }
+      __builtin_amdgcn_sched_barrier(0);
+    }
+    if constexpr (TM > 0) {
+      const int ch = 16 * NJ + 2 * g;
+      float tb[NT][2];
+#pragma unroll
+      for (int tn = 0; tn < NT; tn++) {
+        const int k0 = 16 * NJ + TM * g;
+#pragma unroll
+        for (int r = 0; r < TM; r++) tb[tn][r] = wl[(k0 + r) * CPAD + (tn << 4) + li];
+      }
+      f2v acc = (f2v)(0.f);
+#pragma unroll
+      for (int fy = 0; fy < K; fy++) {
+#pragma unroll
+        for (int fx = 0; fx < K; fx++) {
+          int xo, wo;
+          const bool in = tap(fy, fx, &xo, &wo);
+          acc = __builtin_elementwise_fma(*(const lds_v2*)(L + xo + (in ? ch : 0)), *(const lds_v2*)(L + wo + ch), acc);
+        }
+      }
+      acc = act2<D::ACT>(acc + *(const lds_v2*)(L + D::B_OFF + ch));
+      if constexpr (D::R_SP != SP_NONE) acc += *(const lds_v2*)(L + D::R_OFF + arow * D::R_ST + ch);
+      const float ta[2] = {acc.x, acc.y};
+#pragma unroll
+      for (int tn = 0; tn < NT; tn++) {
+#pragma unroll
+        for (int r = 0; r < TM; r++) acc1[tn] = __builtin_amdgcn_mfma_f32_16x16x4f32(tb[tn][r], ta[r], acc1[tn], 0, 0, 0);
+      }
+      __builtin_amdgcn_sched_barrier(0);
+    }
+#pragma unroll
+    for (int tn = 0; tn < NT; tn++) {
+      const int n0 = tn << 4;
+      const f4v acc = acc0[tn] + acc1[tn];
+      const int c0 = n0 + 4 * g, pix = m0 + li;
+      f4v v = acc;
+      if ((T::COUT % 16 == 0 || c0 < T::COUT) && (P % 16 == 0 || pix < P)) {
+        v = act4<T::ACT>(v + *(const lds_v4*)(bl + c0));
+        if constexpr (T::R_SP != SP_NONE) v += ld4<T::R_SP>(L + T::R_OFF, A + T::R_OFF, pix * T::R_ST + c0);
+        st4<T::Y_SP>(L + T::Y_OFF, A + T::Y_OFF, pix * T::Y_ST + c0 - T::YSUB, v);
+      }
+    }
+  }
+}
+
 template <int SP, int OFF, int ST, int ROWS, int C, int HW, int COFF, bool ACCUM, int MEAN_OFF>
 __device__ __forceinline__ void gap_part(lds_f* L, glb_f* A) {
   constexpr int C4 = C / 4;
diff --git a/backscrub_amd/csrc/plan.cpp b/backscrub_amd/csrc/plan.cpp
--- a/backscrub_amd/csrc/plan.cpp
+++ b/backscrub_amd/csrc/plan.cpp
@@ -97,8 +97,8 @@
   return s;
 }
 
-static void lower_frame_program(const Graph& g, Plan* plan, const std::vector<Step>& steps, const std::vector<int>& ext, const std::map<int, int>& part_n,
-                                const std::map<int, int>& part_hw, const int scratch, const unsigned policy = 0) {
+static void lower_frame_program_pass(const Graph& g, Plan* plan, const std::vector<Step>& steps, const std::vector<int>& ext, const std::map<int, int>& part_n,
+                                     const std::map<int, int>& part_hw, const int scratch, const unsigned policy, const std::vector<char>& dwpw_in, std::vector<char>* dwpw_out, const bool dwpw_early) {
   const bool long_to_hbm = (policy & 1u) != 0, elide_expand = (policy & 2u) != 0, small_top = (policy & 4u) != 0;
   const int kLdsTotal = plan->lds_total_floats, kLdsZero = plan->lds_zero_off();
   plan->program.clear();
@@ -108,6 +108,8 @@
   plan->program_blocks.clear();
   plan->program_check.clear();
   plan->program_ext_offs.clear();
+  plan->program_dwpw_out.clear();
+  plan->program_dwpw_early = dwpw_early;
   for (int t : ext) if (t >= 0 && plan->tensor_off[t] >= 0) plan->program_ext_offs.push_back(plan->tensor_off[t]);
   const int NS = (int)steps.size();
   const int NT = (int)g.tensors.size();
@@ -136,6 +138,22 @@
         for (int t : {a.in0, a.in2, a.in_scale}) if (t >= 0) last[t] = std::max(last[t], s + 1);
       }
     }
+  auto dwpw = [&](int s) { return s >= 0 && s < (int)dwpw_in.size() && dwpw_in[s] != 0; };
+  for (int s = 0; s + 1 < NS; s++) if (dwpw(s)) for (int t : {steps[s].in0, steps[s].residual}) if (t >= 0) last[t] = std::max(last[t], s + 1);
+  dwpw_out->assign(NS, 0);
+  std::map<int, int> in_place;
+  for (int s = 0; s + 1 < NS; s++) {
+    if (!dwpw(s)) continue;
+    const Step& d = steps[s];
+    const Step& a = steps[s + 1];
+    const int r = a.residual, o = a.out;
+    if (r < 0 || o < 0 || r == o || r == g.input || o == g.output || last[r] != s + 1 || r == d.in0 || r == d.residual || r == a.in0 || r == a.in2 || r == a.in_scale) continue;
+    if (std::find(ext.begin(), ext.end(), r) != ext.end() || std::find(ext.begin(), ext.end(), o) != ext.end()) continue;
+    const TensorInfo& tr = g.tensors[r];
+    const TensorInfo& to = g.tensors[o];
+    if (tr.dims[3] != to.dims[3] || tr.dims[1] * tr.dims[2] != to.dims[1] * to.dims[2] || tr.dims[1] * tr.dims[2] <= 1 || to.dims[3] % 4) continue;
+    in_place[o] = r;
+  }
   const bool no_lds = BSX_DBG_ENV("BSX_PROGRAM_NO_LDS") != nullptr;
   std::vector<Loc> loc(NT);
   struct Blk { int off, len, until; };
@@ -154,6 +172,9 @@
       const int pad = ((C / 4) % 2 == 0) ? 4 : 8, need = (P * (C + pad) + 3) / 4 * 4;
       if (reserved + need > kLdsTotal / 4) continue;
       reserved += need;
+      auto ipz = in_place.find(t);
+      if (ipz != in_place.end() && firstdef[ipz->second] >= 0) reserved_at[ipz->second] = kLdsZero - reserved;
+      else
       reserved_at[t] = kLdsZero - reserved;
     }
   }
@@ -217,6 +238,7 @@
   auto gemv_form = [&](const Step& st) { return st.kind == StepKind::PwConv && st.in2 < 0 && st.OH * st.OW <= 4 && st.OH * st.OW * st.Cout * 16 <= kLdsScratchFloats; };
   std::vector<int> stage(NS, 0), slot(NS, 0);
   std::vector<std::vector<int>> slots_from(NS);
+  int q_prev = 0;
   for (int s = 0; s < NS; s++) {
     const Step& st = steps[s];
     long nb = st.kind == StepKind::DwConv ? st.Cout : (st.kind == StepKind::TConv ? st.Cout : st.cout_pad);
@@ -243,6 +265,8 @@
       if (q > 0 && steps[q - 1].kind == StepKind::Gap) q--;
     }
     if (s > 2 && steps[s - 1].kind == StepKind::TConv && steps[s - 2].kind == StepKind::DwConv) q = std::min(q, s - 3);
+    if (dwpw_early && dwpw(s - 1) && stage[s - 1] > 0) q = std::min(q, q_prev);
+    q_prev = q;
     slots_from[q].push_back(s);
   }
   std::vector<MicroOp> prog;
@@ -280,7 +304,7 @@
         for (const Blk& b : live) { if (pos + need <= b.off) break; pos = std::max(pos, b.off + b.len); }
       }
       if (pos + need <= cap) {
-        const int until = elide[s2] ? s2 + 1 : s2;
+        const int until = (elide[s2] || dwpw(s2)) ? s2 + 1 : s2;
         slot[s2] = pos; live.push_back({pos, need, until}); high = std::max(high, pos + need);
         plan->program_blocks.push_back({pos, need, s, until, "weights of step " + std::to_string(s2)});
       }
@@ -302,7 +326,23 @@
         }
       }
     }
+    auto ip = in_place.find(st.out);
+    if (s > 0 && (*dwpw_out)[s - 1] && ip != in_place.end() && loc[st.out].space == kLocNone && loc[ip->second].space == kLocLds) {
+      const Loc lr = loc[ip->second];
+      const bool zone = reserved_at.find(ip->second) != reserved_at.end();
+      bool mine = zone;
+      for (Blk& b : live) if (!zone && b.off == lr.off && b.until == s) { b.until = last[st.out]; mine = true; }
+      if (mine) {
+        for (auto& pb : plan->program_blocks) if (pb.off == lr.off && pb.until == s && pb.what == "tensor " + std::to_string(ip->second)) { pb.until = last[st.out]; pb.what += ", then tensor " + std::to_string(st.out) + " in place"; }
+        loc[st.out] = lr;
+        loc[st.out].elems = (int)g.tensors[st.out].elems();
+        plan->program_lds_tensors++;
+      }
+    }
     place(st.out, s);
+    const bool fused_dw = dwpw(s) && s + 1 < NS && st.in0 >= 0 && loc[st.in0].space == kLocLds && (st.residual < 0 || loc[st.residual].space == kLocLds) && stage[s] > 0 && stage[s + 1] > 0 &&
+                          st.out >= 0 && (loc[st.out].space == kLocGlobal || loc[st.out].space == kLocLds);
+    if (fused_dw) { (*dwpw_out)[s] = 1; plan->program_dwpw_out.push_back(st.out); }
     MicroOp m;
     m.kind = (int)st.kind;
     m.H = st.H; m.W = st.W; m.Cin = st.Cin; m.OH = st.OH; m.OW = st.OW; m.Cout = st.Cout;
@@ -448,13 +488,47 @@
   if (plan->program_check != "ok") plan->program.clear();
 }
 
+static void lower_frame_program(const Graph& g, Plan* plan, const std::vector<Step>& steps, const std::vector<int>& ext, const std::map<int, int>& part_n,
+                                const std::map<int, int>& part_hw, const int scratch, const unsigned policy = 0, const bool dwpw_early = true) {
+  const int NS = (int)steps.size();
+  std::vector<char> cand(NS, 0), got;
+  const char* a16 = getenv("BSX_ACT16");
+  if (!BSX_DBG_ENV("BSX_RTC_NO_DWPW") && !BSX_DBG_ENV("BSX_NO_DW_STRIP") && !(a16 && atoi(a16) != 0)) {
+    std::vector<int> last_use(g.tensors.size(), -1);
+    for (int s = 0; s < NS; s++) {
+      for (int t : {steps[s].in0, steps[s].in1, steps[s].in2, steps[s].residual, steps[s].in_scale}) if (t >= 0) last_use[t] = s;
+      for (int t : steps[s].concat_in) last_use[t] = s;
+    }
+    for (int s = 0; s + 1 < NS; s++) {
+      const Step& d = steps[s];
+      const Step& a = steps[s + 1];
+      if (!(d.kind == StepKind::DwConv && d.kh == d.kw && (d.kh == 3 || d.kh == 5) && d.sh == 1 && d.sw == 1 && d.dh == 1 && d.dw == 1 && d.out >= 0 &&
+            (d.Cin % 16 == 0 || d.Cin % 16 == 8) && d.Cout == d.Cin)) continue;
+      if (!(a.kind == StepKind::PwConv && a.in0 == d.out && a.in1 < 0 && a.in2 < 0 && a.in_scale < 0 && a.residual != d.out && a.cout_pad % 16 == 0 && a.OH * a.OW > 4 &&
+            a.concat_in.empty())) continue;
+      if (last_use[d.out] != s + 1 || d.out == g.output || d.out == g.input || std::find(ext.begin(), ext.end(), d.out) != ext.end()) continue;
+      if (s + 2 < NS && steps[s + 2].kind == StepKind::DwConv && steps[s + 2].in0 == a.out && steps[s + 2].residual == a.out) continue;
+      if ((a.OH * a.OW + 15) / 16 > plan->mid_lanes / 64) continue;
+      cand[s] = 1;
+    }
+  }
+  for (int pass = 0; pass < 4; pass++) {
+    lower_frame_program_pass(g, plan, steps, ext, part_n, part_hw, scratch, policy, cand, &got, dwpw_early);
+    if (got == cand || plan->program.empty()) return;
+    cand = got;
+  }
+  cand.assign(NS, 0);
+  lower_frame_program_pass(g, plan, steps, ext, part_n, part_hw, scratch, policy, cand, &got, dwpw_early);
+}
+
 static long program_arena_bytes(const Plan& plan) {
   long b = 0;
   const int n = (int)plan.program.size();
   for (int i = 0; i < n; i++) {
     const MicroOp& m = plan.program[i];
-    const bool out_elided = mid_pw_feeds_dw(plan, i), in_elided = i > 0 && mid_pw_feeds_dw(plan, i - 1);
-    const long reps = out_elided ? (plan.program[i + 1].Cin + plan.program[i + 1].band_rows - 1) / plan.program[i + 1].band_rows : 1;
+    const bool out_elided = mid_pw_feeds_dw(plan, i) || mid_dw_feeds_pw(plan, i), in_elided = i > 0 && (mid_pw_feeds_dw(plan, i - 1) || mid_dw_feeds_pw(plan, i - 1));
+    const bool expand_elided = mid_pw_feeds_dw(plan, i);
+    const long reps = expand_elided ? (plan.program[i + 1].Cin + plan.program[i + 1].band_rows - 1) / plan.program[i + 1].band_rows : 1;
     for (const Loc* l : {&m.in0, &m.in1, &m.in2, &m.res, &m.out}) {
       if (l->space != kLocGlobal || (l == &m.out && out_elided) || (l == &m.in0 && in_elided)) continue;
       b += 4L * l->elems * (l == &m.out ? 1 : reps);
@@ -465,13 +539,20 @@
 }
 static void build_frame_program(const Graph& g, Plan* plan, const std::vector<Step>& steps, const std::vector<int>& ext = {},
                                 const std::map<int, int>& part_n = {}, const std::map<int, int>& part_hw = {}) {
-  auto lower = [&](unsigned policy) {
-    lower_frame_program(g, plan, steps, ext, part_n, part_hw, kLdsScratchFloats, policy);
+  auto lower_with = [&](unsigned policy, bool dwpw_early) {
+    lower_frame_program(g, plan, steps, ext, part_n, part_hw, kLdsScratchFloats, policy, dwpw_early);
     if (plan->program.empty() || BSX_DBG_ENV("BSX_PLAN_FULL_SCRATCH")) return;
     for (const MicroOp& m : plan->program)
       if ((m.kind == (int)StepKind::PwConv && m.gemv) || m.kind == kMicroTail || m.kind == (int)StepKind::Conv) return;
-    lower_frame_program(g, plan, steps, ext, part_n, part_hw, 64, policy);
-    if (plan->program.empty()) lower_frame_program(g, plan, steps, ext, part_n, part_hw, kLdsScratchFloats, policy);
+    lower_frame_program(g, plan, steps, ext, part_n, part_hw, 64, policy, dwpw_early);
+    if (plan->program.empty()) lower_frame_program(g, plan, steps, ext, part_n, part_hw, kLdsScratchFloats, policy, dwpw_early);
+  };
+  auto lower = [&](unsigned policy) {
+    lower_with(policy, true);
+    if (plan->program.empty() || plan->program_dwpw_out.empty()) return;
+    const long early = program_arena_bytes(*plan);
+    lower_with(policy, false);
+    if (plan->program.empty() || !(program_arena_bytes(*plan) < early)) lower_with(policy, true);
   };
   if (const char* force = BSX_DBG_ENV("BSX_PLAN_POLICY")) { plan->program_policy = (unsigned)atoi(force) & 7u; lower(plan->program_policy); plan->program_arena_bytes = program_arena_bytes(*plan); return; }
   unsigned best = 0;
diff --git a/backscrub_amd/csrc/plan.hpp b/backscrub_amd/csrc/plan.hpp
--- a/backscrub_amd/csrc/plan.hpp
+++ b/backscrub_amd/csrc/plan.hpp
@@ -114,6 +114,8 @@
   int program_lds_floats = 0;
   int program_scratch_floats = 0;
   int program_lds_tensors = 0, program_global_tensors = 0;
+  std::vector<int> program_dwpw_out;
+  bool program_dwpw_early = false;
   std::vector<long> program_ext_offs;
   struct LdsBlock { int off, len, from, until; std::string what; };
   std::vector<LdsBlock> program_blocks;
diff --git a/backscrub_amd/csrc/specialised.cpp b/backscrub_amd/csrc/specialised.cpp
--- a/backscrub_amd/csrc/specialised.cpp
+++ b/backscrub_amd/csrc/specialised.cpp
@@ -34,19 +34,35 @@
 void build_mid(const Plan& plan, bool act16, const std::string& arch, SpecialisedBuild* b) {
   int force = -1;
   if (const char* e = BSX_DBG_ENV("BSX_RTC_TID")) force = atoi(e) != 0;
+  bool dwpw = true;
   auto form = [&](bool opaque, SpecialisedCode* m, long* scratch) {
-    m->source = generate_mid_source(plan, &m->why, act16, opaque);
+    m->source = generate_mid_source(plan, &m->why, act16, opaque, dwpw);
     if (m->source.empty()) { m->fallback = "interpreted (" + m->why + ")"; return false; }
     if (!compile(m, arch, "interpreted", 400)) return false;
     *scratch = code_object_scratch_bytes(m->code, "bsx_mid");
     return true;
   };
-  if (!form(force == 1, &b->mid, &b->scratch)) return;
+  auto pick = [&](SpecialisedBuild* o) {
+    if (!form(force == 1, &o->mid, &o->scratch)) return false;
+    o->opaque_tid = force == 1;
+    if (force >= 0 || o->scratch <= 0) return true;
+    SpecialisedCode alt;
+    long alt_scratch = -1;
+    if (form(true, &alt, &alt_scratch) && alt_scratch >= 0 && alt_scratch < o->scratch) { o->mid = std::move(alt); o->scratch = alt_scratch; o->opaque_tid = true; }
+    return true;
+  };
+  if (!BSX_DBG_ENV("BSX_RTC_FINE")) for (int j = 0; j + 1 < (int)plan.program.size(); j++) if (mid_dw_feeds_pw(plan, j)) b->dwpw = true;
+  if (!b->dwpw) { pick(b); return; }
+  const bool switched = BSX_DBG_ENV("BSX_RTC_DWPW_DECLINE") != nullptr;
+  const bool built = form(force == 1, &b->mid, &b->scratch);
   b->opaque_tid = force == 1;
-  if (force >= 0 || b->scratch <= 0) return;
-  SpecialisedCode alt;
-  long alt_scratch = -1;
-  if (form(true, &alt, &alt_scratch) && alt_scratch >= 0 && alt_scratch < b->scratch) { b->mid = std::move(alt); b->scratch = alt_scratch; b->opaque_tid = true; }
+  if (built && b->scratch <= 0 && !switched) return;
+  dwpw = false;
+  SpecialisedBuild u;
+  if (pick(&u) && !u.mid.code.empty()) {
+    u.dwpw_declined = (built && b->scratch <= 0) ? "declined by the debug switch" : built ? "the fused form needs " + std::to_string(b->scratch) + " B of scratch" : "the fused form did not compile";
+    b->mid = std::move(u.mid); b->scratch = u.scratch; b->opaque_tid = u.opaque_tid; b->dwpw = false; b->dwpw_declined = u.dwpw_declined;
+  } else if (!built) b->dwpw = false;
 }
 
 void build_seg(const Plan& plan, KernelVariant v, const std::string& arch, SpecialisedCode* s) {
@@ -87,9 +103,11 @@
   static const char* const kMid[] = {"bsx_mid"};
   static const char* const kSeg[] = {"bsx_seg_head", "bsx_seg_k2", "bsx_seg_k3", "bsx_seg_tail", "bsx_seg_k3f"};
   k->mid_note = b.mid.fallback;
+  k->dwpw = b.dwpw && !b.mid.code.empty();
   if (!b.mid.code.empty()) {
     if (!load_module(b.mid.code, kMid, 1, &k->mid_mod, &k->mid)) k->mid_note = "interpreted (code object did not load)";
     else k->mid_note = std::string("specialised kernel (hipRTC") + (b.mid.cached ? ", from the cache" : ", compiled now") + (b.opaque_tid ? ", lane indices re-derived per op" : "") +
+                       (b.dwpw_declined.empty() ? std::string() : ", depthwise -> 1x1 pairs as two ops (" + b.dwpw_declined + ")") +
                        (b.scratch > 0 ? ", " + std::to_string(b.scratch) + " B of scratch" : "") + ")";
   }
   k->seg_note = b.seg.fallback;
diff --git a/backscrub_amd/csrc/specialised.hpp b/backscrub_amd/csrc/specialised.hpp
--- a/backscrub_amd/csrc/specialised.hpp
+++ b/backscrub_amd/csrc/specialised.hpp
@@ -25,6 +25,8 @@
 struct SpecialisedBuild {
   SpecialisedCode mid, seg;
   bool opaque_tid = false;
+  bool dwpw = false;
+  std::string dwpw_declined;
   bool seg_k3_frame = false;
   long scratch = -1;
 };
@@ -34,6 +36,7 @@
 struct SpecialisedKernels {
   hipModule_t mid_mod = nullptr, seg_mod = nullptr;
   hipFunction_t mid = nullptr;
+  bool dwpw = false;
   hipFunction_t seg[4] = {};
   hipFunction_t k3_frame = nullptr;
   std::string mid_note, seg_note;
```

After: 753,000 frames/s, median of 6. 1.02x the previous value.
